# Artemarius/cuda-gaussian-splatting

Hardware: AMD Instinct MI355X
Metric: fwd+bwd Mpixels/s @1080p, 1M Gaussians, SH3 (higher is better)
Workload: dtype f32

## Files before the change

cuda-gaussian-splatting_amd/_lib.py:

```python
from __future__ import annotations

import ctypes as C
import os

_HERE = os.path.dirname(os.path.abspath(__file__))
LIB_PATH = os.environ.get("CUGS_HIP_LIBRARY") or os.path.join(_HERE, "libcugs_hip.so")

PACKED_STRIDE = 12
GRAD_STRIDE = 16
TILE = 16


class Camera(C.Structure):
    _fields_ = [("view", C.c_float * 16), ("fx", C.c_float), ("fy", C.c_float), ("cx", C.c_float),
                ("cy", C.c_float), ("width", C.c_int32), ("height", C.c_int32),
                ("cam_center", C.c_float * 3), ("reserved", C.c_float)]


class AdamGroup(C.Structure):
    _fields_ = [("param", C.c_void_p), ("grad", C.c_void_p), ("m", C.c_void_p), ("v", C.c_void_p),
                ("n", C.c_int64), ("lr", C.c_float), ("reserved", C.c_float)]


class AdamFused(C.Structure):
    _fields_ = [("m", C.c_void_p * 5), ("v", C.c_void_p * 5), ("lr", C.c_float * 5), ("beta1", C.c_float),
                ("beta2", C.c_float), ("eps", C.c_float), ("bc1", C.c_float), ("bc2", C.c_float)]


class DensifyArray(C.Structure):
    _fields_ = [("src", C.c_void_p), ("dst", C.c_void_p), ("row_floats", C.c_int32), ("mode", C.c_int32)]


DENSIFY_COPY, DENSIFY_POSITIONS, DENSIFY_SCALES, DENSIFY_STATE = 0, 1, 2, 3


class McmcFused(C.Structure):
    _fields_ = [("lambda_opacity", C.c_float), ("lambda_scale", C.c_float), ("noise_lr", C.c_float),
                ("gate_k", C.c_float), ("gate_t", C.c_float), ("step", C.c_uint32), ("seed", C.c_uint64),
                ("noise", C.c_void_p)]


KNN_AUTO, KNN_EXHAUSTIVE, KNN_TREE = 0, 1, 2
MCMC_STREAM_NOISE, MCMC_STREAM_JITTER, MCMC_STREAM_SAMPLE = 0, 1, 2


class PoseGrad(C.Structure):
    _fields_ = [("dL_dview", C.c_void_p), ("rows", C.c_void_p), ("workspace", C.c_void_p),
                ("workspace_bytes", C.c_size_t)]


class BlendForwardOpts(C.Structure):
    _fields_ = [("zero_buf", C.c_void_p), ("zero_bytes", C.c_size_t), ("tile_order", C.c_void_p),
                ("depths", C.c_void_p), ("out_depth", C.c_void_p)]


class BlendBackwardOpts(C.Structure):
    _fields_ = [("prezeroed", C.c_int), ("abs_grad", C.c_int), ("tile_order", C.c_void_p), ("depths", C.c_void_p),
                ("dL_ddepth_map", C.c_void_p), ("dL_dalpha", C.c_void_p), ("dL_ddepths", C.c_void_p),
                ("dL_dmeans_2d_abs", C.c_void_p)]


class LossOpts(C.Structure):
    _fields_ = [("exposure", C.c_void_p), ("mask", C.c_void_p), ("dL_dexposure", C.c_void_p), ("corrected", C.c_void_p)]


class DepthLossOpts(C.Structure):
    _fields_ = [("weight", C.c_void_p), ("scale_shift", C.c_void_p), ("fit", C.c_int), ("inverse", C.c_int),
                ("min_alpha", C.c_float), ("expected", C.c_void_p)]


class NormalLossOpts(C.Structure):
    _fields_ = [("weight", C.c_void_p), ("normals_out", C.c_void_p), ("cos_weight", C.c_float), ("l1_weight", C.c_float),
                ("min_alpha", C.c_float)]


class BilagridDims(C.Structure):
    _fields_ = [("l", C.c_int32), ("gy", C.c_int32), ("gx", C.c_int32)]

_P = C.c_void_p
_I = C.c_int
_L = C.c_int64
_F = C.c_float
_U32 = C.c_uint32
_U64 = C.c_uint64

SIGNATURES = {
    "cugs_version": (C.c_char_p, []),
    "cugs_error_string": (C.c_char_p, [_I]),
    "cugs_project_forward": (_I, [_L, _I, _I, _P, _P, _P, _P, _P, C.POINTER(Camera), _F,
                                  _P, _P, _P, _P, _P, _P, _P, _P, _P, _P]),
    "cugs_project_forward_keyed": (_I, [_L, _I, _I, _P, _P, _P, _P, _P, C.POINTER(Camera), _F,
                                        _P, _P, _P, _P, _P, _P, _P, _P, _P, _P, C.c_size_t, _P]),
    "cugs_project_forward_geometry": (_I, [_L, _P, _P, _P, _P, C.POINTER(Camera), _F, _P, _P, _P, _P, _P, _P, _P, _P,
                                           C.c_size_t, _P]),
    "cugs_project_forward_colour": (_I, [_L, _I, _I, _P, _P, C.POINTER(Camera), _P, _P, _P, _P]),
    "cugs_evaluate_sh": (_I, [_I, _L, _I, _P, _P, _P, _P]),
    "cugs_evaluate_sh_backward": (_I, [_I, _L, _I, _P, _P, _P, _P, _P]),
    "cugs_pack_projected": (_I, [_L, _P, _P, _P, _P, _P, _P]),
    "cugs_sort_workspace_bytes": (C.c_size_t, [_L]),
    "cugs_sort_pair_workspace_bytes": (C.c_size_t, [_L]),
    "cugs_sort_count_pairs": (_I, [_L, _P, _P, _P, _P, _I, _I, _P, C.c_size_t, C.POINTER(C.c_int64), _P]),
    "cugs_sort_count_pairs_wide": (_I, [_L, _P, _P, _P, _P, _I, _I, _P, C.c_size_t, C.POINTER(C.c_int64), _P]),
    "cugs_sort_pairs_predicted_wide": (_I, [_L, _L, _P, _P, _P, _P, _I, _I, _P, C.c_size_t, _P, C.c_size_t, _P, _P, _P,
                                            C.POINTER(C.c_int64), _P]),
    "cugs_sort_pairs": (_I, [_L, _L, _P, _P, _P, _P, _I, _I, _P, C.c_size_t, _P, C.c_size_t, _P, _P, _P, _P]),
    "cugs_sort_pairs_predicted": (_I, [_L, _L, _P, _P, _P, _P, _I, _I, _P, C.c_size_t, _P, C.c_size_t, _P, _P, _P,
                                       C.POINTER(C.c_int64), _P]),
    "cugs_sort_pairs_predicted_keyed": (_I, [_L, _L, _P, _P, _P, _P, _I, _I, _P, C.c_size_t, _P, C.c_size_t, _P, _P, _P,
                                             C.POINTER(C.c_int64), _P]),
    "cugs_sort_pairs_predicted_keyed_ordered": (_I, [_L, _L, _P, _P, _P, _P, _I, _I, _P, C.c_size_t, _P, C.c_size_t, _P, _P, _P,
                                                     C.POINTER(C.c_int64), _P, _P]),
    "cugs_tile_order": (_I, [_I, _I, _P, _P, _P]),
    "cugs_rasterize_forward": (_I, [_I, _I, C.POINTER(C.c_float), _P, _P, _P, _P, _P, _P, _P,
                                    _P, _P, _P, _P]),
    "cugs_rasterize_forward_opts": (_I, [_I, _I, C.POINTER(C.c_float), _P, _P, _P, _P, _P, _P, _P,
                                         _P, _P, _P, C.POINTER(BlendForwardOpts), _P]),
    "cugs_blend_scores": (_I, [_I, _I, _P, _P, _P, _P, _P, _P, _P, _I, _P, _P]),
    "cugs_rasterize_backward": (_I, [_I, _I, C.POINTER(C.c_float), _P, _P, _P, _P, _P, _P, _P,
                                     _P, _P, _P, _L, _P, _P, _P, _P, _P, _P]),
    "cugs_rasterize_backward_opts": (_I, [_I, _I, C.POINTER(C.c_float), _P, _P, _P, _P, _P, _P, _P,
                                          _P, _P, _P, _L, _P, _P, _P, _P, _P, C.POINTER(BlendBackwardOpts), _P]),
    "cugs_project_backward": (_I, [_L, _I, _I, _P, _P, _P, _P, _P, _P, _P, C.POINTER(Camera), _F,
                                   _P, _P, _P, _P, _P, _P, _P, _P, _P, _P, _P, _P, _P]),
    "cugs_project_backward_adam": (_I, [_L, _I, _I, _P, _P, _P, _P, _P, _P, _P, C.POINTER(Camera), _F, _P,
                                        C.POINTER(AdamFused), _P, _P]),
    "cugs_sh_backward_views": (_I, [_I, _L, _I, _P, _I, _P, C.POINTER(C.c_float), _P, _P]),
    "cugs_gated_colour_grad": (_I, [_L, _P, _P, _P, _P]),
    "cugs_adam_bias_correction": (None, [_F, _F, _I, C.POINTER(C.c_float), C.POINTER(C.c_float)]),
    "cugs_fused_adam": (_I, [_P, _P, _P, _P, _L, _F, _F, _F, _F, _F, _F, _P]),
    "cugs_fused_adam_groups": (_I, [C.POINTER(AdamGroup), _I, _F, _F, _F, _F, _F, _P]),
    "cugs_fused_adam_groups_rows": (_I, [C.POINTER(AdamGroup), _I, C.POINTER(C.c_int32), _P, _L, _F, _F, _F, _F, _F, _P]),
    "cugs_loss_workspace_bytes": (C.c_size_t, [_I, _I]),
    "cugs_combined_loss": (_I, [_I, _I, _P, _P, _F, _I, _P, C.c_size_t, _P, _P, _P, _P]),
    "cugs_loss_opts_workspace_bytes": (C.c_size_t, [_I, _I]),
    "cugs_combined_loss_opts": (_I, [_I, _I, _P, _P, _F, _I, C.POINTER(LossOpts), _P, C.c_size_t, _P, _P, _P, _P]),
    "cugs_depth_loss_workspace_bytes": (C.c_size_t, [_I, _I]),
    "cugs_depth_loss": (_I, [_I, _I, _P, _P, _P, C.POINTER(DepthLossOpts), _P, C.c_size_t, _P, _P, _P, _P]),
    "cugs_normal_loss_workspace_bytes": (C.c_size_t, [_I, _I]),
    "cugs_normal_loss": (_I, [_I, _I, _F, _F, _F, _F, _P, _P, _P, C.POINTER(NormalLossOpts), _P, C.c_size_t, _P, _P, _P, _P]),
    "cugs_bilagrid_workspace_bytes": (C.c_size_t, [_I, _I, C.POINTER(BilagridDims)]),
    "cugs_bilagrid_slice": (_I, [_I, _I, C.POINTER(BilagridDims), _P, _P, _P, _P]),
    "cugs_bilagrid_slice_backward": (_I, [_I, _I, C.POINTER(BilagridDims), _P, _P, _P, _P, C.c_size_t, _P, _P, _P]),
    "cugs_bilagrid_tv": (_I, [C.POINTER(BilagridDims), _P, _F, _P, _P, _I, _P]),
    "cugs_eval_workspace_bytes": (C.c_size_t, [_I, _I]),
    "cugs_eval_metrics": (_I, [_I, _I, _P, _P, _P, _I, _P, C.c_size_t, _P, _P]),
    "cugs_densify_accumulate": (_I, [_L, _P, _P, _P, _P, _P, _P]),
    "cugs_densify_accumulate_strided": (_I, [_L, _P, _L, _P, _P, _P, _P, _P]),
    "cugs_densify_classify": (_I, [_L, _P, _P, _P, _P, _P, _F, _F, _F, _I, _F, _F, _P, _P, _P]),
    "cugs_densify_workspace_bytes": (C.c_size_t, [_L]),
    "cugs_densify_plan": (_I, [_L, _P, _P, C.c_size_t, C.POINTER(C.c_int64), _P]),
    "cugs_densify_apply": (_I, [_L, _L, _P, C.c_size_t, _P, _P, C.POINTER(DensifyArray), _I, _P]),
    "cugs_mcmc_random_bits": (_I, [_U64, _U32, _U32, _U64, _L, _P, _P]),
    "cugs_mcmc_regularization": (_I, [_L, _P, _P, _F, _F, _P, _P, _P, _P, _P, _P, C.c_size_t, _P]),
    "cugs_mcmc_inject_noise": (_I, [_L, _P, _P, _P, _F, _F, _F, _P, _U64, _U32, _P]),
    "cugs_mcmc_relocate_workspace_bytes": (C.c_size_t, [_L]),
    "cugs_mcmc_relocate": (_I, [_L, _I, _P, _P, _P, _P, _P, _F, _F, _F, _U64, _U32, C.POINTER(_P), C.POINTER(_P), _P,
                                C.c_size_t, _P, _P, _P]),
    "cugs_project_backward_adam_mcmc": (_I, [_L, _I, _I, _P, _P, _P, _P, _P, _P, _P, C.POINTER(Camera), _F, _P,
                                             C.POINTER(AdamFused), C.POINTER(McmcFused), _P, _P]),
    "cugs_pose_grad_workspace_bytes": (C.c_size_t, [_L]),
    "cugs_project_backward_pose": (_I, [_L, _I, _I, _P, _P, _P, _P, _P, _P, _P, C.POINTER(Camera), _F,
                                        _P, _P, _P, _P, _P, _P, _P, _P, _P, _P, _P, _P, C.POINTER(PoseGrad), _P]),
    "cugs_project_backward_adam_pose": (_I, [_L, _I, _I, _P, _P, _P, _P, _P, _P, _P, C.POINTER(Camera), _F, _P,
                                             C.POINTER(AdamFused), _P, C.POINTER(PoseGrad), _P]),
    "cugs_project_backward_adam_mcmc_pose": (_I, [_L, _I, _I, _P, _P, _P, _P, _P, _P, _P, C.POINTER(Camera), _F, _P,
                                                  C.POINTER(AdamFused), C.POINTER(McmcFused), _P, C.POINTER(PoseGrad),
                                                  _P]),
    "cugs_project_backward_adam_sparse": (_I, [_L, _I, _I, _P, _P, _P, _P, _P, _P, _P, C.POINTER(Camera), _F, _P,
                                               C.POINTER(AdamFused), _P, _P]),
    "cugs_project_backward_adam_sparse_pose": (_I, [_L, _I, _I, _P, _P, _P, _P, _P, _P, _P, C.POINTER(Camera), _F, _P,
                                                    C.POINTER(AdamFused), _P, C.POINTER(PoseGrad), _P]),
    "cugs_ply_vertex_floats": (_I, [_I, _I]),
    "cugs_ply_pack": (_I, [_L, _I, C.POINTER(_P), C.POINTER(_P), C.POINTER(_P), _P, _P]),
    "cugs_ply_unpack": (_I, [_L, _I, _I, _P, _P, C.POINTER(_P), C.POINTER(_P), C.POINTER(_P), _P]),
    "cugs_image_to_float": (_I, [_I, _I, _P, _I, _I, _P, _P]),
    "cugs_knn_workspace_bytes": (C.c_size_t, [_L, _I]),
    "cugs_knn_mean_distances": (_I, [_L, _I, _P, _P, _P, C.c_size_t, _I, _P]),
    "cugs_init_from_points": (_I, [_L, _I, _P, _P, _P, _P, _P, _P, _P, _P, _P]),
    "cugs_device_count": (_I, [C.POINTER(C.c_int)]),
}


def _load() -> C.CDLL:
    if not os.path.exists(LIB_PATH):
        raise ImportError(
            f"{LIB_PATH} not found: build it with `make -C {os.path.join(_HERE, 'csrc')}` "
            "(or `python -c 'import __graft_entry__ as g; g.build()'`). "
            "There is no fallback path: the HIP library is the implementation.")
    lib = C.CDLL(LIB_PATH)
    for name, (res, args) in SIGNATURES.items():
        try:
            fn = getattr(lib, name)
        except AttributeError as e:
            raise ImportError(f"{LIB_PATH} does not export {name}") from e
        fn.restype = res
        fn.argtypes = args
    return lib


lib = _load()


class CugsError(RuntimeError):
    """Non-zero return from the C ABI (the adapter's std::runtime_error, cuda_utils.cuh:12-20)."""


# ... 9 lines not shown
```

cuda-gaussian-splatting_amd/adapter/cugs_hip_torch.cpp:

```cpp
#include "cugs_hip_torch.hpp"

#include <c10/hip/HIPFunctions.h>
#include <c10/hip/HIPStream.h>
#include <hip/hip_runtime_api.h>

#include <algorithm>
#include <chrono>
#include <cmath>
#include <cstdio>
#include <cstdlib>
#include <map>
#include <stdexcept>
#include <string>
#include <tuple>
#include <vector>

namespace cugs_hip {
namespace {

void check(int code, const char* what) {
    if (code != 0)
        throw std::runtime_error(std::string("HIP error in ") + what + " - " + cugs_error_string(code));
}
void* stream_of(const torch::Tensor& t) {
// ... 106 lines not shown
        check((wide_depth ? cugs_sort_count_pairs_wide : cugs_sort_count_pairs)(
                  n, ptr<float>(m), ptr<float>(d), ptr<int32_t>(r), ptr<int32_t>(tiles), img_w, img_h, ws.data_ptr(),
                  ws.numel(), &total, st), "cugs_sort_count_pairs");
    o.total_pairs = static_cast<int>(total);
    o.gaussian_keys_sorted = torch::empty({total}, torch::TensorOptions().dtype(torch::kInt64).device(means_2d.device()));
    o.gaussian_values_sorted = torch::empty({total}, iopt(means_2d));
    if (num_tiles > 0) {
        auto wp = workspace(means_2d.device(), cugs_sort_pair_workspace_bytes(total), 1);
        check(cugs_sort_pairs(n, total, ptr<float>(m), ptr<float>(d), ptr<int32_t>(r), ptr<int32_t>(tiles), img_w, img_h,
                              ws.data_ptr(), ws.numel(), wp.data_ptr(), wp.numel(),
                              reinterpret_cast<uint64_t*>(ptr<int64_t>(o.gaussian_keys_sorted)),
                              ptr<int32_t>(o.gaussian_values_sorted), ptr<int32_t>(o.tile_ranges), st),
              "cugs_sort_pairs");
    }
    return o;
}
}

SortingOutput sort_gaussians(const torch::Tensor& means_2d, const torch::Tensor& depths, const torch::Tensor& radii,
                             const torch::Tensor& tiles_touched, int img_w, int img_h) {
    return sort_gaussians_impl(means_2d, depths, radii, tiles_touched, img_w, img_h, false);
}

ForwardOutput rasterize_forward(const torch::Tensor& means_2d, const torch::Tensor& cov_2d_inv, const torch::Tensor& rgb,
                                const torch::Tensor& opacities, const torch::Tensor& tile_ranges,
                                const torch::Tensor& gaussian_indices, int img_w, int img_h,
                                const float background[3], const torch::Tensor& packed, const torch::Tensor& zero_buf,
                                const torch::Tensor& tile_order, const torch::Tensor& depths) {
    TORCH_CHECK(means_2d.is_cuda(), "means_2d must be on CUDA");
    ForwardOutput o;
    o.color = torch::empty({img_h, img_w, 3}, fopt(means_2d));
    o.final_T = torch::empty({img_h, img_w}, fopt(means_2d));
    o.n_contrib = torch::empty({img_h, img_w}, iopt(means_2d));
    if (depths.defined()) {
        TORCH_CHECK(depths.is_cuda() && depths.device() == means_2d.device() && depths.dim() == 1 &&
                    depths.size(0) == means_2d.size(0), "depths must be [N] on the device of means_2d");
        o.depth_map = torch::empty({img_h, img_w}, fopt(means_2d));
    }
    if (img_w == 0 || img_h == 0) {
        if (zero_buf.defined()) zero_buf.zero_();
        return o;
    }
    auto m = means_2d.contiguous(), c = cov_2d_inv.contiguous(), r = rgb.contiguous(), op = opacities.contiguous();
    auto tr = tile_ranges.contiguous(), gi = gaussian_indices.contiguous();
    if (zero_buf.defined())
        TORCH_CHECK(zero_buf.is_contiguous() && zero_buf.scalar_type() == torch::kFloat32 && zero_buf.numel() % 4 == 0,
                    "zero_buf must be a contiguous float32 tensor of a multiple of four elements");
    if (tile_order.defined())
        TORCH_CHECK(tile_order.is_contiguous() && tile_order.scalar_type() == torch::kInt32 &&
                    tile_order.numel() == 4 * tr.size(0), "tile_order must be a contiguous [tiles, 4] int32 tensor");
    const auto z = depths.defined() ? f32c(depths) : depths;
    cugs_blend_forward_opts opts{};
    if (zero_buf.defined()) {
        opts.zero_buf = zero_buf.data_ptr();
        opts.zero_bytes = static_cast<size_t>(zero_buf.numel()) * sizeof(float);
    }
    opts.tile_order = order_ptr(tile_order);
    opts.depths = ptr<float>(z);
    opts.out_depth = ptr<float>(o.depth_map);
    check(cugs_rasterize_forward_opts(img_w, img_h, background, ptr<int32_t>(tr), ptr<int32_t>(gi), ptr<float>(m),
                                      ptr<float>(c), ptr<float>(r), ptr<float>(op), ptr<float>(packed), ptr<float>(o.color),
                                      ptr<float>(o.final_T), ptr<int32_t>(o.n_contrib), &opts, stream_of(means_2d)),
          "cugs_rasterize_forward_opts");
    return o;
}

torch::Tensor tile_order_of(const torch::Tensor& tile_ranges, int img_w, int img_h) {
    auto tr = tile_ranges.contiguous();
    auto order = torch::empty({tr.size(0), 4}, iopt(tile_ranges));
    if (tr.size(0) > 0)
        check(cugs_tile_order(img_w, img_h, ptr<int32_t>(tr), reinterpret_cast<uint32_t*>(order.data_ptr<int32_t>()),
                              stream_of(tile_ranges)), "cugs_tile_order");
    return order;
}

RasterizeBackwardOutput rasterize_backward(const torch::Tensor& dL_dcolor, const torch::Tensor& means_2d,
                                           const torch::Tensor& cov_2d_inv, const torch::Tensor& rgb,
                                           const torch::Tensor& opacities, const torch::Tensor& tile_ranges,
                                           const torch::Tensor& gaussian_indices, const torch::Tensor& final_T,
                                           const torch::Tensor& n_contrib, int img_w, int img_h,
                                           const float background[3], int n_gaussians, const torch::Tensor& packed,
                                           bool unpack, const torch::Tensor& zeroed_accum, const torch::Tensor& tile_order,
                                           const torch::Tensor& depths, const torch::Tensor& dL_ddepth_map,
                                           const torch::Tensor& dL_dalpha, bool want_abs_grad) {
    TORCH_CHECK(dL_dcolor.is_cuda(), "dL_dcolor must be on CUDA");
    const int64_t n = n_gaussians;
    RasterizeBackwardOutput o;
    const bool depth_route = depths.defined() || dL_ddepth_map.defined() || dL_dalpha.defined();
    if (depth_route) {
        TORCH_CHECK(depths.defined(), "the depth / alpha map gradients need the projection's depths");
        TORCH_CHECK(depths.is_cuda() && depths.device() == dL_dcolor.device() && depths.dim() == 1 && depths.size(0) == n,
                    "depths must be [N] on the device of dL_dcolor");
        for (const torch::Tensor* t : {&dL_ddepth_map, &dL_dalpha})
            if (t->defined())
                TORCH_CHECK(t->is_cuda() && t->device() == dL_dcolor.device() && t->dim() == 2 && t->size(0) == img_h &&
                            t->size(1) == img_w, "dL_ddepth_map / dL_dalpha must be [H, W] on the device of dL_dcolor");
    }
    const bool prezeroed = zeroed_accum.defined();
    if (prezeroed)
        TORCH_CHECK(zeroed_accum.is_contiguous() && zeroed_accum.dim() == 2 && zeroed_accum.size(0) == n &&
                    zeroed_accum.size(1) == CUGS_GRAD_STRIDE, "zeroed_accum must be a contiguous [N, 16] float32 tensor");
    o.grad_accum = prezeroed ? zeroed_accum : torch::empty({n, CUGS_GRAD_STRIDE}, fopt(dL_dcolor));
    if (unpack) {
        o.dL_drgb = torch::empty({n, 3}, fopt(dL_dcolor));
        o.dL_dopacity_act = torch::empty({n}, fopt(dL_dcolor));
        o.dL_dmeans_2d = torch::empty({n, 2}, fopt(dL_dcolor));
        o.dL_dcov_2d_inv = torch::empty({n, 3}, fopt(dL_dcolor));
        if (depth_route) o.dL_ddepths = torch::empty({n}, fopt(dL_dcolor));
    }
    if (want_abs_grad)
        o.dL_dmeans_2d_abs = unpack ? torch::empty({n, 2}, fopt(dL_dcolor)) : o.grad_accum.slice(1, 10, 12);
    if (n == 0) return o;
    auto g = dL_dcolor.contiguous(), m = means_2d.contiguous(), c = cov_2d_inv.contiguous(), r = rgb.contiguous();
    auto op = opacities.contiguous(), tr = tile_ranges.contiguous(), gi = gaussian_indices.contiguous();
    auto ft = final_T.contiguous(), nc = n_contrib.contiguous();
    if (tile_order.defined())
        TORCH_CHECK(tile_order.is_contiguous() && tile_order.scalar_type() == torch::kInt32 &&
                    tile_order.numel() == 4 * tr.size(0), "tile_order must be a contiguous [tiles, 4] int32 tensor");
    auto f32 = [](const torch::Tensor& t) { return t.defined() ? f32c(t) : t; };
    const auto z = f32(depths), dd = f32(dL_ddepth_map), da = f32(dL_dalpha);
    cugs_blend_backward_opts opts{};
    opts.prezeroed = prezeroed ? 1 : 0;
    opts.abs_grad = want_abs_grad ? 1 : 0;
    opts.tile_order = order_ptr(tile_order);
    opts.depths = ptr<float>(z);
    opts.dL_ddepth_map = ptr<float>(dd);
    opts.dL_dalpha = ptr<float>(da);
    opts.dL_ddepths = ptr<float>(o.dL_ddepths);
    opts.dL_dmeans_2d_abs = unpack ? ptr<float>(o.dL_dmeans_2d_abs) : nullptr;
    check(cugs_rasterize_backward_opts(img_w, img_h, background, ptr<int32_t>(tr), ptr<int32_t>(gi), ptr<float>(m),
                                       ptr<float>(c), ptr<float>(r), ptr<float>(op), ptr<float>(packed), ptr<float>(g),
                                       ptr<float>(ft), ptr<int32_t>(nc), n, ptr<float>(o.grad_accum),
                                       ptr<float>(o.dL_drgb), ptr<float>(o.dL_dopacity_act), ptr<float>(o.dL_dmeans_2d),
                                       ptr<float>(o.dL_dcov_2d_inv), &opts, stream_of(dL_dcolor)),
          "cugs_rasterize_backward_opts");
    return o;
}

namespace {
ProjectionBackwardOutput project_backward_impl(const torch::Tensor* accum, const torch::Tensor* colour_gate,
                                               torch::Tensor* d_means_out, const torch::Tensor& gm, const torch::Tensor& gc,
                                               const torch::Tensor& gr, const torch::Tensor& go,
                                               const torch::Tensor& positions, const torch::Tensor& rotations,
                                               const torch::Tensor& scales, const torch::Tensor& opacities,
                                               const torch::Tensor& sh_coeffs, const torch::Tensor& radii,
                                               const cugs_camera& camera, int degree, float scale_modifier,
                                               const cugs_pose_grad* pose = nullptr) {
    TORCH_CHECK(positions.is_cuda(), "positions must be on CUDA");
    const int64_t n = positions.size(0);
    ProjectionBackwardOutput o;
    o.dL_dpositions = torch::empty({n, 3}, fopt(positions));
    o.dL_drotations = torch::empty({n, 4}, fopt(positions));
    o.dL_dscales = torch::empty({n, 3}, fopt(positions));
    o.dL_dopacities = torch::empty({n, 1}, fopt(positions));
    auto sh = f32c(sh_coeffs);
    o.dL_dsh_coeffs = torch::empty_like(sh);
    if (n == 0) return o;
    auto pos = f32c(positions), rot = f32c(rotations), scl = f32c(scales), opa = f32c(opacities), rad = radii.contiguous();
    auto cm = gm.defined() ? gm.contiguous() : gm, cc = gc.defined() ? gc.contiguous() : gc;
    auto cr = gr.defined() ? gr.contiguous() : gr, co = go.defined() ? go.contiguous() : go;
    if (pose) {
        check(cugs_project_backward_pose(n, static_cast<int>(sh.size(2)), degree, ptr<float>(pos), ptr<float>(rot),
                                         ptr<float>(scl), ptr<float>(opa), ptr<float>(sh), ptr<int32_t>(rad),
                                         colour_gate ? ptr<uint8_t>(*colour_gate) : nullptr, &camera, scale_modifier,
                                         accum ? ptr<float>(*accum) : nullptr, ptr<float>(cm), ptr<float>(cc),
                                         ptr<float>(cr), ptr<float>(co), ptr<float>(o.dL_dpositions),
                                         ptr<float>(o.dL_drotations), ptr<float>(o.dL_dscales),
                                         ptr<float>(o.dL_dopacities), ptr<float>(o.dL_dsh_coeffs),
                                         d_means_out ? ptr<float>(*d_means_out) : nullptr,
                                         nullptr, pose, stream_of(positions)),
              "cugs_project_backward_pose");
        return o;
    }
    check(cugs_project_backward(n, static_cast<int>(sh.size(2)), degree, ptr<float>(pos), ptr<float>(rot), ptr<float>(scl),
                                ptr<float>(opa), ptr<float>(sh), ptr<int32_t>(rad),
                                colour_gate ? ptr<uint8_t>(*colour_gate) : nullptr, &camera, scale_modifier,
                                accum ? ptr<float>(*accum) : nullptr, ptr<float>(cm), ptr<float>(cc), ptr<float>(cr),
                                ptr<float>(co), ptr<float>(o.dL_dpositions), ptr<float>(o.dL_drotations),
                                ptr<float>(o.dL_dscales), ptr<float>(o.dL_dopacities), ptr<float>(o.dL_dsh_coeffs),
                                d_means_out ? ptr<float>(*d_means_out) : nullptr, nullptr,
                                stream_of(positions)),
          "cugs_project_backward");
    return o;
}
}

ProjectionBackwardOutput project_backward(const torch::Tensor& dL_dmeans_2d, const torch::Tensor& dL_dcov_2d_inv,
                                          const torch::Tensor& dL_drgb, const torch::Tensor& dL_dopacity_act,
                                          const torch::Tensor& positions, const torch::Tensor& rotations,
                                          const torch::Tensor& scales, const torch::Tensor& opacities,
                                          const torch::Tensor& sh_coeffs, const torch::Tensor& radii,
                                          const cugs_camera& camera, int active_sh_degree, float scale_modifier) {
    return project_backward_impl(nullptr, nullptr, nullptr, dL_dmeans_2d, dL_dcov_2d_inv, dL_drgb, dL_dopacity_act,
                                 positions, rotations, scales, opacities, sh_coeffs, radii, camera, active_sh_degree,
                                 scale_modifier);
}

torch::Tensor evaluate_sh_cuda(int degree, const torch::Tensor& sh_coeffs, const torch::Tensor& directions) {
    TORCH_CHECK(degree >= 0 && degree <= 3, "SH degree must be 0..3, got ", degree);
    TORCH_CHECK(sh_coeffs.is_cuda(), "sh_coeffs must be on CUDA device");
    TORCH_CHECK(directions.is_cuda(), "directions must be on CUDA device");
    TORCH_CHECK(sh_coeffs.dim() == 3 && sh_coeffs.size(1) == 3, "sh_coeffs must be [N, 3, C]");
    TORCH_CHECK(directions.dim() == 2 && directions.size(1) == 3, "directions must be [N, 3]");
    TORCH_CHECK(sh_coeffs.size(0) == directions.size(0), "Batch size mismatch");
    TORCH_CHECK(sh_coeffs.size(2) >= (degree + 1) * (degree + 1), "Need at least ", (degree + 1) * (degree + 1),
                " coefficients for degree ", degree);
    auto c = f32c(sh_coeffs), d = f32c(directions);
    auto out = torch::empty({c.size(0), 3}, fopt(c));
    if (c.size(0) == 0) return out;
    check(cugs_evaluate_sh(degree, c.size(0), static_cast<int>(c.size(2)), ptr<float>(c), ptr<float>(d), ptr<float>(out),
                           stream_of(c)), "cugs_evaluate_sh");
    return out;
}

torch::Tensor evaluate_sh_backward_cuda(int degree, const torch::Tensor& sh_coeffs, const torch::Tensor& directions,
                                        const torch::Tensor& dL_dcolor) {
    TORCH_CHECK(degree >= 0 && degree <= 3, "SH degree must be 0..3, got ", degree);
    TORCH_CHECK(sh_coeffs.is_cuda() && directions.is_cuda() && dL_dcolor.is_cuda(), "inputs must be on CUDA device");
    TORCH_CHECK(sh_coeffs.dim() == 3 && sh_coeffs.size(1) == 3, "sh_coeffs must be [N, 3, C]");
    TORCH_CHECK(directions.dim() == 2 && directions.size(1) == 3, "directions must be [N, 3]");
    TORCH_CHECK(dL_dcolor.dim() == 2 && dL_dcolor.size(1) == 3, "dL_dcolor must be [N, 3]");
    auto c = f32c(sh_coeffs), d = f32c(directions), g = f32c(dL_dcolor);
    auto out = torch::empty_like(c);
    if (c.size(0) == 0) return out;
    check(cugs_evaluate_sh_backward(degree, c.size(0), static_cast<int>(c.size(2)), ptr<float>(c), ptr<float>(d),
                                    ptr<float>(g), ptr<float>(out), stream_of(c)), "cugs_evaluate_sh_backward");
    return out;
}

static int max_sh_degree(const torch::Tensor& sh) {
    return sh.defined() ? static_cast<int>(std::sqrt(static_cast<float>(sh.size(2)))) - 1 : 0;
}

RenderOutput render(const ModelTensors& model, const cugs_camera& camera, const RenderSettings& settings,
                    bool for_backward, bool want_depth_map) {
    TORCH_CHECK(model.positions.defined() && model.positions.is_cuda(), "GaussianModel must be on CUDA device");
    const int64_t n = model.positions.size(0);
    const int w = camera.width, h = camera.height;
    RenderOutput o;
    if (n == 0) {
        o.color = torch::empty({h, w, 3}, fopt(model.positions));
        for (int ch = 0; ch < 3; ++ch) o.color.select(2, ch).fill_(settings.background[ch]);
        o.final_T = torch::ones({h, w}, fopt(model.positions));
        o.n_contrib = torch::zeros({h, w}, iopt(model.positions));
        o.means_2d = torch::empty({0, 2}, fopt(model.positions)); o.depths = torch::empty({0}, fopt(model.positions));
        o.cov_2d_inv = torch::empty({0, 3}, fopt(model.positions)); o.radii = torch::empty({0}, iopt(model.positions));
        o.rgb = torch::empty({0, 3}, fopt(model.positions)); o.opacities_act = torch::empty({0}, fopt(model.positions));
        o.gaussian_indices = torch::empty({0}, iopt(model.positions)); o.tile_ranges = torch::empty({0, 2}, iopt(model.positions));
        if (want_depth_map) o.depth_map = torch::zeros({h, w}, fopt(model.positions));
        return o;
    }
    const int degree = std::min(settings.active_sh_degree, max_sh_degree(model.sh_coeffs));
    SortState& state = sort_state(model.positions.device());
    const int num_tiles = ((w + CUGS_TILE - 1) / CUGS_TILE) * ((h + CUGS_TILE - 1) / CUGS_TILE);
    const bool predicted = state.last_pairs >= 0 && num_tiles > 0;
    const bool wide = state.wide_left > 0;
    if (wide) --state.wide_left;
    const bool keyed = predicted && !wide;
    auto proj = project_impl(model.positions, model.rotations, model.scales, model.opacities, model.sh_coeffs, camera,
                             degree, settings.scale_modifier, keyed);
    torch::Tensor accum = for_backward ? torch::empty({n, CUGS_GRAD_STRIDE}, fopt(model.positions)) : torch::Tensor();
    auto blend = [&](const SortingOutput& s) {
        return rasterize_forward(proj.means_2d, proj.cov_2d_inv, proj.rgb, proj.opacities_act, s.tile_ranges,
                                 s.gaussian_values_sorted, w, h, settings.background, proj.packed, accum, s.tile_order,
                                 want_depth_map ? proj.depths : torch::Tensor());
// ... 29 lines not shown
            check(cugs_sort_pairs_predicted_keyed(
                      n, cap, ptr<float>(proj.means_2d), ptr<float>(proj.depths), ptr<int32_t>(proj.radii), ptr<int32_t>(tiles), w, h,
                      ws.data_ptr(), ws.numel(), wp.data_ptr(), wp.numel(), nullptr, ptr<int32_t>(srt.gaussian_values_sorted),
                      ptr<int32_t>(srt.tile_ranges), total.data_ptr<int64_t>(), st), "cugs_sort_pairs_predicted_keyed");
        } else {
            srt.tile_order = torch::empty({num_tiles, 4}, iopt(proj.means_2d));
            check(cugs_sort_pairs_predicted_keyed_ordered(
                      n, cap, ptr<float>(proj.means_2d), ptr<float>(proj.depths), ptr<int32_t>(proj.radii), ptr<int32_t>(tiles), w, h,
                      ws.data_ptr(), ws.numel(), wp.data_ptr(), wp.numel(), nullptr, ptr<int32_t>(srt.gaussian_values_sorted),
                      ptr<int32_t>(srt.tile_ranges), total.data_ptr<int64_t>(),
                      reinterpret_cast<uint32_t*>(srt.tile_order.data_ptr<int32_t>()), st), "cugs_sort_pairs_predicted_keyed_ordered");
        }
        hipEvent_t ev;
        TORCH_CHECK(hipEventCreateWithFlags(&ev, hipEventDisableTiming) == hipSuccess, "hipEventCreate failed");
        TORCH_CHECK(hipEventRecord(ev, static_cast<hipStream_t>(st)) == hipSuccess, "hipEventRecord failed");
        fwd = blend(srt);
        const bool ok = hipEventSynchronize(ev) == hipSuccess;
        (void)hipEventDestroy(ev);
        TORCH_CHECK(ok, "hipEventSynchronize failed");
        const int64_t p = total.data_ptr<int64_t>()[0];
        TORCH_CHECK(p >= -1 && p <= 2147483647ll, "pair count exceeds the reference's int indexing");
        if (p >= 0 && p <= cap) {
            srt.total_pairs = static_cast<int>(p);
            srt.gaussian_values_sorted = srt.gaussian_values_sorted.slice(0, 0, p);
        } else {
            if (p == -1) state.wide_left = kWideDepthHold;
            srt = sort_gaussians_impl(proj.means_2d, proj.depths, proj.radii, proj.tiles_touched, w, h,
                                      p == -1 || state.wide_left > 0);
            if (ordered) srt.tile_order = tile_order_of(srt.tile_ranges, w, h);
            fwd = blend(srt);
        }
    }
    state.last_pairs = std::max<int64_t>(srt.total_pairs, prev - prev / 32);
    o.color = fwd.color; o.final_T = fwd.final_T; o.n_contrib = fwd.n_contrib; o.depth_map = fwd.depth_map;
    o.means_2d = proj.means_2d; o.depths = proj.depths; o.cov_2d_inv = proj.cov_2d_inv; o.radii = proj.radii;
    o.rgb = proj.rgb; o.opacities_act = proj.opacities_act;
    o.gaussian_indices = srt.gaussian_values_sorted; o.tile_ranges = srt.tile_ranges; o.packed = proj.packed;
    o.tile_order = srt.tile_order;
    o.colour_gate = proj.colour_gate;
    o.zeroed_accum = accum;
    if (accum.defined()) o.accum_used = std::make_shared<std::atomic<bool>>(false);
    return o;
}

BackwardOutput render_backward(const torch::Tensor& dL_dcolor, const RenderOutput& ro, const ModelTensors& model,
                               const cugs_camera& camera, const RenderSettings& settings, FusedAdam* fused,
                               const MCMCController* mcmc, int step, const torch::Tensor& dL_ddepth_map,
                               const torch::Tensor& dL_dalpha, bool want_camera_grad, bool want_abs_grad,
                               bool sparse_adam) {
    TORCH_CHECK(!mcmc || fused, "the fused MCMC route needs the FusedAdam (otherwise: compute_regularization, step, "
                "inject_noise)");
    TORCH_CHECK(!sparse_adam || fused, "sparse_adam needs the FusedAdam (otherwise: render_backward, apply_gradients, "
                "step(radii))");
    TORCH_CHECK(!sparse_adam || !mcmc, "sparse_adam cannot be combined with the fused MCMC route: its regulariser and "
                "noise act on every Gaussian");
    TORCH_CHECK(dL_dcolor.is_cuda(), "dL_dcolor must be on CUDA device");
    TORCH_CHECK(dL_dcolor.dim() == 3 && dL_dcolor.size(2) == 3, "dL_dcolor must be [H, W, 3]");
    TORCH_CHECK(!dL_ddepth_map.defined() || ro.depth_map.defined(),
                "dL_ddepth_map needs a render with the depth map (render(..., want_depth_map = true))");
    const bool depth_grads = dL_ddepth_map.defined() || dL_dalpha.defined();
    const int64_t n = model.positions.size(0);
    BackwardOutput o;
    if (n == 0) {
        o.dL_dpositions = torch::zeros({0, 3}, fopt(dL_dcolor)); o.dL_drotations = torch::zeros({0, 4}, fopt(dL_dcolor));
        o.dL_dscales = torch::zeros({0, 3}, fopt(dL_dcolor)); o.dL_dopacities = torch::zeros({0, 1}, fopt(dL_dcolor));
        o.dL_dsh_coeffs = torch::zeros_like(model.sh_coeffs); o.dL_dmeans_2d = torch::zeros({0, 2}, fopt(dL_dcolor));
        if (want_camera_grad) o.dL_dviewmat = torch::zeros({4, 4}, fopt(dL_dcolor));
        if (want_abs_grad) o.dL_dmeans_2d_abs = torch::zeros({0, 2}, fopt(dL_dcolor));
        return o;
    }
    const int degree = std::min(settings.active_sh_degree, max_sh_degree(model.sh_coeffs));
    torch::Tensor packed = ro.packed;
    if (!packed.defined() || packed.size(0) != n) {
        packed = torch::empty({n, CUGS_PACKED_STRIDE}, fopt(dL_dcolor));
        auto m = ro.means_2d.contiguous(), c = ro.cov_2d_inv.contiguous(), r = ro.rgb.contiguous(),
             op = ro.opacities_act.contiguous();
        check(cugs_pack_projected(n, ptr<float>(m), ptr<float>(c), ptr<float>(r), ptr<float>(op), ptr<float>(packed),
                                  stream_of(dL_dcolor)), "cugs_pack_projected");
    }
    torch::Tensor zeroed = ro.zeroed_accum;
    ro.zeroed_accum = torch::Tensor();
    if (zeroed.defined() && ro.accum_used && ro.accum_used->exchange(true)) zeroed = torch::Tensor();
    if (zeroed.defined() && (zeroed.dim() != 2 || zeroed.size(0) != n)) zeroed = torch::Tensor();
    auto rb = rasterize_backward(dL_dcolor, ro.means_2d, ro.cov_2d_inv, ro.rgb, ro.opacities_act, ro.tile_ranges,
                                 ro.gaussian_indices, ro.final_T, ro.n_contrib, camera.width, camera.height,
                                 settings.background, static_cast<int>(n), packed, false, zeroed, ro.tile_order,
                                 depth_grads ? ro.depths : torch::Tensor(), dL_ddepth_map, dL_dalpha, want_abs_grad);
    o.dL_dmeans_2d_abs = rb.dL_dmeans_2d_abs;
    o.dL_dmeans_2d = torch::empty({n, 2}, fopt(dL_dcolor));
    cugs_pose_grad pose{};
    torch::Tensor pose_ws;
    if (want_camera_grad) {
        o.dL_dviewmat = torch::empty({4, 4}, fopt(dL_dcolor));
        const size_t bytes = cugs_pose_grad_workspace_bytes(n);
        pose_ws = torch::empty({static_cast<int64_t>(bytes)}, dL_dcolor.options().dtype(torch::kUInt8));
        pose = cugs_pose_grad{ptr<float>(o.dL_dviewmat), nullptr, pose_ws.data_ptr(), bytes};
    }
    if (fused) {
        const auto& pr = fused->params();
        TORCH_CHECK(pr[0].data_ptr() == model.positions.data_ptr() && pr[1].data_ptr() == model.sh_coeffs.data_ptr(),
                    "the fused optimizer step needs the FusedAdam that was built on this model");
        TORCH_CHECK(ro.colour_gate.defined() && ro.colour_gate.size(0) == n,
                    "the fused optimizer step needs the colour_gate of cugs_hip::render");
        const cugs_adam_fused adam = fused->begin_fused_step();
        auto radii = ro.radii.contiguous(), gate = ro.colour_gate.contiguous();
        if (mcmc) {
            const cugs_mcmc_fused mc = mcmc->fused_args(step);
            if (want_camera_grad) {
                check(cugs_project_backward_adam_mcmc_pose(n, static_cast<int>(model.sh_coeffs.size(2)), degree,
                                                           ptr<float>(model.positions), ptr<float>(model.rotations),
                                                           ptr<float>(model.scales), ptr<float>(model.opacities),
                                                           ptr<float>(model.sh_coeffs), ptr<int32_t>(radii),
                                                           ptr<uint8_t>(gate), &camera, settings.scale_modifier,
                                                           ptr<float>(rb.grad_accum), &adam, &mc,
                                                           ptr<float>(o.dL_dmeans_2d), &pose, stream_of(dL_dcolor)),
                      "cugs_project_backward_adam_mcmc_pose");
                return o;
            }
            check(cugs_project_backward_adam_mcmc(n, static_cast<int>(model.sh_coeffs.size(2)), degree,
                                                  ptr<float>(model.positions), ptr<float>(model.rotations),
                                                  ptr<float>(model.scales), ptr<float>(model.opacities),
                                                  ptr<float>(model.sh_coeffs), ptr<int32_t>(radii), ptr<uint8_t>(gate),
                                                  &camera, settings.scale_modifier, ptr<float>(rb.grad_accum), &adam, &mc,
                                                  ptr<float>(o.dL_dmeans_2d), stream_of(dL_dcolor)),
                  "cugs_project_backward_adam_mcmc");
            return o;
        }
        if (sparse_adam) {
            if (want_camera_grad) {
                check(cugs_project_backward_adam_sparse_pose(n, static_cast<int>(model.sh_coeffs.size(2)), degree,
                                                             ptr<float>(model.positions), ptr<float>(model.rotations),
                                                             ptr<float>(model.scales), ptr<float>(model.opacities),
                                                             ptr<float>(model.sh_coeffs), ptr<int32_t>(radii),
                                                             ptr<uint8_t>(gate), &camera, settings.scale_modifier,
                                                             ptr<float>(rb.grad_accum), &adam, ptr<float>(o.dL_dmeans_2d),
                                                             &pose, stream_of(dL_dcolor)),
                      "cugs_project_backward_adam_sparse_pose");
                return o;
            }
            check(cugs_project_backward_adam_sparse(n, static_cast<int>(model.sh_coeffs.size(2)), degree,
                                                    ptr<float>(model.positions), ptr<float>(model.rotations),
                                                    ptr<float>(model.scales), ptr<float>(model.opacities),
                                                    ptr<float>(model.sh_coeffs), ptr<int32_t>(radii), ptr<uint8_t>(gate),
                                                    &camera, settings.scale_modifier, ptr<float>(rb.grad_accum), &adam,
                                                    ptr<float>(o.dL_dmeans_2d), stream_of(dL_dcolor)),
                  "cugs_project_backward_adam_sparse");
            return o;
        }
        if (want_camera_grad) {
            check(cugs_project_backward_adam_pose(n, static_cast<int>(model.sh_coeffs.size(2)), degree,
                                                  ptr<float>(model.positions), ptr<float>(model.rotations),
                                                  ptr<float>(model.scales), ptr<float>(model.opacities),
                                                  ptr<float>(model.sh_coeffs), ptr<int32_t>(radii), ptr<uint8_t>(gate),
                                                  &camera, settings.scale_modifier, ptr<float>(rb.grad_accum), &adam,
                                                  ptr<float>(o.dL_dmeans_2d), &pose, stream_of(dL_dcolor)),
                  "cugs_project_backward_adam_pose");
            return o;
        }
        check(cugs_project_backward_adam(n, static_cast<int>(model.sh_coeffs.size(2)), degree, ptr<float>(model.positions),
                                         ptr<float>(model.rotations), ptr<float>(model.scales), ptr<float>(model.opacities),
                                         ptr<float>(model.sh_coeffs), ptr<int32_t>(radii), ptr<uint8_t>(gate), &camera,
                                         settings.scale_modifier, ptr<float>(rb.grad_accum), &adam,
                                         ptr<float>(o.dL_dmeans_2d), stream_of(dL_dcolor)),
              "cugs_project_backward_adam");
        return o;
    }
    const bool have_gate = ro.colour_gate.defined() && ro.colour_gate.dim() == 1 && ro.colour_gate.size(0) == n;
    auto pb = project_backward_impl(&rb.grad_accum, have_gate ? &ro.colour_gate : nullptr, &o.dL_dmeans_2d, {}, {}, {}, {}, model.positions,
                                    model.rotations, model.scales, model.opacities, model.sh_coeffs, ro.radii, camera, degree,
                                    settings.scale_modifier, want_camera_grad ? &pose : nullptr);
    o.dL_dpositions = pb.dL_dpositions; o.dL_drotations = pb.dL_drotations; o.dL_dscales = pb.dL_dscales;
    o.dL_dopacities = pb.dL_dopacities; o.dL_dsh_coeffs = pb.dL_dsh_coeffs;
    return o;
}

namespace {
void validate_pair(const torch::Tensor& rendered, const torch::Tensor& target) {
    for (const torch::Tensor* img : {&rendered, &target}) {
        TORCH_CHECK(img->dim() == 3, "image must be 3-dimensional [H, W, 3], got ", img->dim(), " dims");
        TORCH_CHECK(img->size(2) == 3, "image must have 3 channels, got ", img->size(2));
        TORCH_CHECK(img->dtype() == torch::kFloat32, "image must be float32, got ", img->dtype());
        TORCH_CHECK(img->is_cuda(), "image must be on a CUDA device");
    }
    TORCH_CHECK(rendered.sizes() == target.sizes(), "rendered and target must have the same shape, got ",
                rendered.sizes(), " vs ", target.sizes());
}
torch::Tensor run_loss(const torch::Tensor& rendered, const torch::Tensor& target, float lambda_, int window_size,
                       torch::Tensor* ssim_map, torch::Tensor* grad) {
    validate_pair(rendered, target);
    TORCH_CHECK(window_size % 2 == 1, "window_size must be odd, got ", window_size);
    TORCH_CHECK(window_size >= 3, "window_size must be >= 3, got ", window_size);
    const int h = static_cast<int>(rendered.size(0)), w = static_cast<int>(rendered.size(1));
    auto r = rendered.contiguous(), t = target.contiguous();
    auto out = torch::empty({4}, fopt(rendered));
    if (ssim_map) *ssim_map = torch::empty({h, w}, fopt(rendered));
    if (grad) *grad = torch::empty({h, w, 3}, fopt(rendered));
    auto ws = workspace(rendered.device(), cugs_loss_workspace_bytes(w, h), 2);
    check(cugs_combined_loss(w, h, ptr<float>(r), ptr<float>(t), lambda_, window_size, ws.data_ptr(), ws.numel(),
                             ptr<float>(out), ssim_map ? ptr<float>(*ssim_map) : nullptr,
                             grad ? ptr<float>(*grad) : nullptr, stream_of(rendered)), "cugs_combined_loss");
    return out;
}
}

LossAndGrad combined_loss_and_grad(const torch::Tensor& rendered, const torch::Tensor& target, float lambda_, bool want_grad) {
    LossAndGrad o;
    auto out = run_loss(rendered, target, lambda_, 11, nullptr, want_grad ? &o.dL_dcolor : nullptr);
    o.loss = out[0]; o.l1 = out[1]; o.ssim_mean = out[2];
    return o;
}
torch::Tensor combined_loss(const torch::Tensor& rendered, const torch::Tensor& target, float lambda_) {
    return run_loss(rendered, target, lambda_, 11, nullptr, nullptr)[0];
}
torch::Tensor ssim(const torch::Tensor& rendered, const torch::Tensor& target, int window_size) {
    torch::Tensor map;
    run_loss(rendered, target, 0.2f, window_size, &map, nullptr);
    return map;
}

ExposureLoss combined_loss_exposure(const torch::Tensor& rendered, const torch::Tensor& target, float lambda_,
                                    const torch::Tensor& exposure, const torch::Tensor& mask, bool want_grad,
                                    bool want_corrected, int window_size) {
    validate_pair(rendered, target);
    TORCH_CHECK(window_size % 2 == 1, "window_size must be odd, got ", window_size);
    TORCH_CHECK(window_size >= 3, "window_size must be >= 3, got ", window_size);
    const int h = static_cast<int>(rendered.size(0)), w = static_cast<int>(rendered.size(1));
    if (exposure.defined()) {
        TORCH_CHECK(exposure.dim() == 2 && exposure.size(0) == 3 && exposure.size(1) == 4, "exposure must be [3, 4], got ", exposure.sizes());
        TORCH_CHECK(exposure.dtype() == torch::kFloat32, "exposure must be float32, got ", exposure.dtype());
        TORCH_CHECK(exposure.is_cuda() && exposure.device() == rendered.device(), "exposure must be on the images' CUDA device");
        TORCH_CHECK(exposure.is_contiguous(), "exposure must be contiguous");
    }
    torch::Tensor m;
    if (mask.defined()) {
        TORCH_CHECK(mask.dim() == 2 && mask.size(0) == h && mask.size(1) == w, "mask must be [H, W], got ", mask.sizes());
        TORCH_CHECK(mask.dtype() == torch::kFloat32, "mask must be float32, got ", mask.dtype());
        TORCH_CHECK(mask.is_cuda() && mask.device() == rendered.device(), "mask must be on the images' CUDA device");
        m = mask.contiguous();
    }
    auto r = rendered.contiguous(), t = target.contiguous();
    auto out = torch::empty({4}, fopt(rendered));
    ExposureLoss o;
    if (want_grad) o.dL_dcolor = torch::empty({h, w, 3}, fopt(rendered));
    if (want_grad && exposure.defined()) o.dL_dexposure = torch::empty({3, 4}, fopt(rendered));
    if (want_corrected) o.corrected = torch::empty({h, w, 3}, fopt(rendered));
    cugs_loss_opts opts{};
    opts.exposure = exposure.defined() ? exposure.data_ptr<float>() : nullptr;
    opts.mask = m.defined() ? m.data_ptr<float>() : nullptr;
    opts.dL_dexposure = o.dL_dexposure.defined() ? o.dL_dexposure.data_ptr<float>() : nullptr;
    opts.corrected = o.corrected.defined() ? o.corrected.data_ptr<float>() : nullptr;
    auto ws = workspace(rendered.device(), cugs_loss_opts_workspace_bytes(w, h), 2);
    check(cugs_combined_loss_opts(w, h, ptr<float>(r), ptr<float>(t), lambda_, window_size, &opts, ws.data_ptr(), ws.numel(),
                                  ptr<float>(out), nullptr, want_grad ? o.dL_dcolor.data_ptr<float>() : nullptr,
// ... 864 lines not shown
```

cuda-gaussian-splatting_amd/adapter/cugs_hip_torch.hpp:

```cpp
#pragma once

#include <torch/torch.h>

#include <atomic>
#include <memory>

#include <array>
#include <string>
#include <vector>

#include "../../include/cugs_hip.h"
#include "eval_results.hpp"

namespace cugs_hip {

struct ProjectionOutput {
    torch::Tensor means_2d, depths, cov_2d_inv, radii, tiles_touched, rgb, opacities_act;
    torch::Tensor packed;
    torch::Tensor colour_gate;
};
struct SortingOutput {
    torch::Tensor gaussian_keys_sorted, gaussian_values_sorted, tile_ranges;
    int total_pairs = 0;
    torch::Tensor tile_order;
};
struct ForwardOutput {
    torch::Tensor color, final_T, n_contrib;
    torch::Tensor depth_map;
};
struct RasterizeBackwardOutput {
    torch::Tensor dL_drgb, dL_dopacity_act, dL_dmeans_2d, dL_dcov_2d_inv;
    torch::Tensor grad_accum;
    torch::Tensor dL_ddepths;
    torch::Tensor dL_dmeans_2d_abs;
};
struct ProjectionBackwardOutput { torch::Tensor dL_dpositions, dL_drotations, dL_dscales, dL_dopacities, dL_dsh_coeffs; };

struct ModelTensors {
    torch::Tensor positions, sh_coeffs, opacities, rotations, scales;
};
struct RenderSettings { float background[3] = {0.f, 0.f, 0.f}; int active_sh_degree = 3; float scale_modifier = 1.f; };
struct RenderOutput {
    torch::Tensor color, final_T, n_contrib, means_2d, depths, cov_2d_inv, radii, rgb, opacities_act,
        gaussian_indices, tile_ranges;
    torch::Tensor packed;
    torch::Tensor colour_gate;
    mutable torch::Tensor zeroed_accum;
    std::shared_ptr<std::atomic<bool>> accum_used;
    torch::Tensor tile_order;
    torch::Tensor depth_map;
};
struct BackwardOutput {
    torch::Tensor dL_dpositions, dL_drotations, dL_dscales, dL_dopacities, dL_dsh_coeffs, dL_dmeans_2d;
    torch::Tensor dL_dviewmat;
    torch::Tensor dL_dmeans_2d_abs;
};

ProjectionOutput project_gaussians(const torch::Tensor& positions, const torch::Tensor& rotations,
                                   const torch::Tensor& scales, const torch::Tensor& opacities,
                                   const torch::Tensor& sh_coeffs, const cugs_camera& camera,
                                   int active_sh_degree, float scale_modifier = 1.0f);
SortingOutput sort_gaussians(const torch::Tensor& means_2d, const torch::Tensor& depths, const torch::Tensor& radii,
                             const torch::Tensor& tiles_touched, int img_w, int img_h);
ForwardOutput rasterize_forward(const torch::Tensor& means_2d, const torch::Tensor& cov_2d_inv,
                                const torch::Tensor& rgb, const torch::Tensor& opacities,
                                const torch::Tensor& tile_ranges, const torch::Tensor& gaussian_indices,
                                int img_w, int img_h, const float background[3],
                                const torch::Tensor& packed = {}, const torch::Tensor& zero_buf = {},
                                const torch::Tensor& tile_order = {}, const torch::Tensor& depths = {});
torch::Tensor tile_order_of(const torch::Tensor& tile_ranges, int img_w, int img_h);
RasterizeBackwardOutput rasterize_backward(const torch::Tensor& dL_dcolor, const torch::Tensor& means_2d,
                                           const torch::Tensor& cov_2d_inv, const torch::Tensor& rgb,
                                           const torch::Tensor& opacities, const torch::Tensor& tile_ranges,
                                           const torch::Tensor& gaussian_indices, const torch::Tensor& final_T,
                                           const torch::Tensor& n_contrib, int img_w, int img_h,
                                           const float background[3], int n_gaussians,
                                           const torch::Tensor& packed = {}, bool unpack = true,
                                           const torch::Tensor& zeroed_accum = {}, const torch::Tensor& tile_order = {},
                                           const torch::Tensor& depths = {}, const torch::Tensor& dL_ddepth_map = {},
                                           const torch::Tensor& dL_dalpha = {}, bool want_abs_grad = false);
ProjectionBackwardOutput project_backward(const torch::Tensor& dL_dmeans_2d, const torch::Tensor& dL_dcov_2d_inv,
                                          const torch::Tensor& dL_drgb, const torch::Tensor& dL_dopacity_act,
                                          const torch::Tensor& positions, const torch::Tensor& rotations,
                                          const torch::Tensor& scales, const torch::Tensor& opacities,
                                          const torch::Tensor& sh_coeffs, const torch::Tensor& radii,
                                          const cugs_camera& camera, int active_sh_degree,
                                          float scale_modifier = 1.0f);
torch::Tensor evaluate_sh_cuda(int degree, const torch::Tensor& sh_coeffs, const torch::Tensor& directions);
torch::Tensor evaluate_sh_backward_cuda(int degree, const torch::Tensor& sh_coeffs, const torch::Tensor& directions,
                                        const torch::Tensor& dL_dcolor);

RenderOutput render(const ModelTensors& model, const cugs_camera& camera, const RenderSettings& settings,
                    bool for_backward = true, bool want_depth_map = false);
class FusedAdam;
class MCMCController;
BackwardOutput render_backward(const torch::Tensor& dL_dcolor, const RenderOutput& render_out,
                               const ModelTensors& model, const cugs_camera& camera, const RenderSettings& settings,
                               FusedAdam* fused = nullptr, const MCMCController* mcmc = nullptr, int step = 0,
                               const torch::Tensor& dL_ddepth_map = {}, const torch::Tensor& dL_dalpha = {},
                               bool want_camera_grad = false, bool want_abs_grad = false, bool sparse_adam = false);

struct LossAndGrad { torch::Tensor loss, l1, ssim_mean, dL_dcolor; };
LossAndGrad combined_loss_and_grad(const torch::Tensor& rendered, const torch::Tensor& target, float lambda_ = 0.2f,
                                   bool want_grad = true);
torch::Tensor combined_loss(const torch::Tensor& rendered, const torch::Tensor& target, float lambda_ = 0.2f);
torch::Tensor ssim(const torch::Tensor& rendered, const torch::Tensor& target, int window_size = 11);

struct ExposureLoss { torch::Tensor loss, dL_dcolor, dL_dexposure, l1, ssim_mean, corrected; };
ExposureLoss combined_loss_exposure(const torch::Tensor& rendered, const torch::Tensor& target, float lambda_ = 0.2f,
                                    const torch::Tensor& exposure = {}, const torch::Tensor& mask = {},
                                    bool want_grad = true, bool want_corrected = false, int window_size = 11);

struct DepthLoss { torch::Tensor loss, dL_ddepth_map, dL_dalpha, scale_shift, valid_weight, valid_count, fit_ok, expected; };
DepthLoss depth_loss(const torch::Tensor& depth_map, const torch::Tensor& alpha, const torch::Tensor& target,
                     const torch::Tensor& weight = {}, bool inverse = false, const torch::Tensor& align = {},
                     bool fit = false, float min_alpha = 1e-3f, bool want_grad = true, bool want_expected = false);

struct NormalLoss { torch::Tensor loss, dL_ddepth_map, dL_dalpha, valid_weight, valid_count, normals; };
NormalLoss normal_loss(const torch::Tensor& depth_map, const torch::Tensor& alpha, float fx, float fy, float cx, float cy,
                       const torch::Tensor& target = {}, const torch::Tensor& weight = {}, float cos_weight = 1.0f,
                       float l1_weight = 0.0f, float min_alpha = 1e-3f, bool want_grad = true, bool want_normals = false);
torch::Tensor depth_to_normals(const torch::Tensor& depth_map, const torch::Tensor& alpha, float fx, float fy, float cx,
                               float cy, float min_alpha = 1e-3f);

struct BilagridGrad { torch::Tensor dL_drendered, dL_dgrid; };
struct BilagridTV { torch::Tensor tv, dL_dgrid; };
torch::Tensor bilagrid_slice(const torch::Tensor& grid, const torch::Tensor& rendered);
BilagridGrad bilagrid_slice_backward(const torch::Tensor& grid, const torch::Tensor& rendered,
                                     const torch::Tensor& dL_dcorrected, bool want_grid_grad = true,
                                     bool want_image_grad = true);
BilagridTV bilagrid_tv(const torch::Tensor& grid, float weight = 1.0f, const torch::Tensor& dL_dgrid = {});

struct AdamHyper { float beta1 = 0.9f, beta2 = 0.999f, eps = 1e-15f; };
class FusedAdam {
public:
    FusedAdam(std::array<torch::Tensor, 5> params, std::array<float, 5> lrs, AdamHyper h = {});
    void apply_gradients(const BackwardOutput& grads);
    void zero_grad();
    void set_lr(int group, float lr) { lrs_[group] = lr; }
    float get_lr(int group) const { return lrs_[group]; }
    void step();
    void step(const torch::Tensor& visible);
    cugs_adam_fused begin_fused_step();
    const std::array<torch::Tensor, 5>& params() const { return params_; }
    const std::array<torch::Tensor, 5>& exp_avg() const { return m_; }
    const std::array<torch::Tensor, 5>& exp_avg_sq() const { return v_; }
private:
    friend class DensificationController;
    friend class MCMCController;
    friend int64_t prune_gaussians(ModelTensors&, const torch::Tensor&, FusedAdam*);
    friend bool write_gaussian_ply(const std::string&, const ModelTensors&, const FusedAdam*);
    friend ModelTensors read_gaussian_ply(const std::string&, const torch::Device&, FusedAdam*);
    void step_groups(const torch::Tensor* rows);
    std::array<torch::Tensor, 5> params_, m_, v_, grads_;
    std::array<float, 5> lrs_;
    AdamHyper h_;
    int step_count_ = 0;
};

struct DensificationConfig {
    int densify_from = 500, densify_until = 15000, densify_every = 100, opacity_reset_every = 3000;
    float grad_threshold = 0.0002f, opacity_threshold = 0.005f, percent_dense = 0.01f;
    int max_screen_size = 20, max_gaussians = 0;
// ... 87 lines not shown
```

cuda-gaussian-splatting_amd/csrc/project_backward.hip:

```cpp
#include "project_backward_kernels.h"

namespace {

template <int C>
int launch_shv(int64_t n, int degree, const float* pos, const float* gated, const ViewCenters& vc, float* out,
               bool aligned, hipStream_t st) {
    if (aligned)
        hipLaunchKernelGGL((k_sh_backward_views<C, true>), dim3(grid_for(n)), dim3(CUGS_BLOCK), 0, st, n, degree, pos, gated, vc, out);
    else
        hipLaunchKernelGGL((k_sh_backward_views<C, false>), dim3(grid_for(n)), dim3(CUGS_BLOCK), 0, st, n, degree, pos, gated, vc, out);
    CUGS_LAUNCH_CHECK();
    return 0;
}


template <int C>
int launch_pb(int64_t n, int degree, const CamArgs& cam, const PBPtrs& p, bool aligned, hipStream_t st,
              const AdamFusedArgs* adam = nullptr) {
    const AdamFusedArgs none{};
    if (adam) {
        if constexpr (C == 16) {
            if (aligned && p.colour_gate) {
                hipLaunchKernelGGL((k_project_backward<C, true, true, true>), dim3(grid_for(n)), dim3(CUGS_BLOCK), 0, st, n, degree, cam, p, *adam, McmcFusedArgs{}, PoseArgs{});
                CUGS_LAUNCH_CHECK();
                return 0;
            }
        }
        if (aligned)
            hipLaunchKernelGGL((k_project_backward<C, true, true>), dim3(grid_for(n)), dim3(CUGS_BLOCK), 0, st, n, degree, cam, p, *adam, McmcFusedArgs{}, PoseArgs{});
        else
            hipLaunchKernelGGL((k_project_backward<C, false, true>), dim3(grid_for(n)), dim3(CUGS_BLOCK), 0, st, n, degree, cam, p, *adam, McmcFusedArgs{}, PoseArgs{});
    } else if (aligned) {
        if constexpr (C == 16) {
            if (p.colour_gate) {
                hipLaunchKernelGGL((k_project_backward<C, true, false, true>), dim3(grid_for(n)), dim3(CUGS_BLOCK), 0, st, n, degree, cam, p, none, McmcFusedArgs{}, PoseArgs{});
                CUGS_LAUNCH_CHECK();
                return 0;
            }
        }
        hipLaunchKernelGGL((k_project_backward<C, true, false>), dim3(grid_for(n)), dim3(CUGS_BLOCK), 0, st, n, degree, cam, p, none, McmcFusedArgs{}, PoseArgs{});
    } else {
        hipLaunchKernelGGL((k_project_backward<C, false, false>), dim3(grid_for(n)), dim3(CUGS_BLOCK), 0, st, n, degree, cam, p, none, McmcFusedArgs{}, PoseArgs{});
    }
    CUGS_LAUNCH_CHECK();
    return 0;
}


template <int C>
int launch_shb(int64_t n, int degree, const float* sh, const float* dirs, const float* g, float* out,
               bool aligned, hipStream_t st) {
    if (aligned)
        hipLaunchKernelGGL((k_sh_backward<C, true>), dim3(grid_for(n)), dim3(CUGS_BLOCK), 0, st, n, degree, sh, dirs, g, out);
    else
        hipLaunchKernelGGL((k_sh_backward<C, false>), dim3(grid_for(n)), dim3(CUGS_BLOCK), 0, st, n, degree, sh, dirs, g, out);
    CUGS_LAUNCH_CHECK();
    return 0;
}


}

extern "C" int cugs_project_backward(int64_t n, int num_coeffs, int active_degree, const float* positions,
                                     const float* rotations, const float* scales, const float* opacities,
                                     const float* sh_coeffs, const int32_t* radii, const uint8_t* colour_gate,
                                     const cugs_camera* camera_host, float scale_modifier,
                                     const float* grad_accum, const float* dL_dmeans_2d,
                                     const float* dL_dcov_2d_inv, const float* dL_drgb,
                                     const float* dL_dopacity_act, float* dL_dpositions, float* dL_drotations,
                                     float* dL_dscales, float* dL_dopacities, float* dL_dsh_coeffs,
                                     float* dL_dmeans_2d_out, float* dL_drgb_gated_out, void* stream) {
    CamArgs cam;
    PBPtrs p;
    bool aligned;
    const int r = prepare_plain(n, num_coeffs, active_degree, positions, rotations, scales, opacities, sh_coeffs, radii,
                                colour_gate, camera_host, scale_modifier, grad_accum, dL_dmeans_2d, dL_dcov_2d_inv, dL_drgb,
                                dL_dopacity_act, dL_dpositions, dL_drotations, dL_dscales, dL_dopacities, dL_dsh_coeffs,
                                dL_dmeans_2d_out, dL_drgb_gated_out, cam, p, aligned);
    if (r != 0) return r == 1 ? 0 : r;
    hipStream_t st = static_cast<hipStream_t>(stream);
    switch (num_coeffs) {
        case 1: return launch_pb<1>(n, active_degree, cam, p, aligned, st);
        case 4: return launch_pb<4>(n, active_degree, cam, p, aligned, st);
        case 9: return launch_pb<9>(n, active_degree, cam, p, aligned, st);
        default: return launch_pb<16>(n, active_degree, cam, p, aligned, st);
    }
}


extern "C" int cugs_project_backward_adam(int64_t n, int num_coeffs, int active_degree, float* positions,
                                          float* rotations, float* scales, float* opacities, float* sh_coeffs,
                                          const int32_t* radii, const uint8_t* colour_gate,
                                          const cugs_camera* camera_host, float scale_modifier,
                                          const float* grad_accum, const cugs_adam_fused* adam_host,
                                          float* dL_dmeans_2d_out, void* stream) {
    CamArgs cam;
    PBPtrs p;
    AdamFusedArgs a;
    bool aligned;
    const int r = prepare_adam(n, num_coeffs, active_degree, positions, rotations, scales, opacities, sh_coeffs, radii,
                               colour_gate, camera_host, scale_modifier, grad_accum, adam_host, dL_dmeans_2d_out, cam, p,
                               a, aligned);
    if (r != 0) return r == 1 ? 0 : r;
    hipStream_t st = static_cast<hipStream_t>(stream);
    switch (num_coeffs) {
        case 1: return launch_pb<1>(n, active_degree, cam, p, aligned, st, &a);
        case 4: return launch_pb<4>(n, active_degree, cam, p, aligned, st, &a);
        case 9: return launch_pb<9>(n, active_degree, cam, p, aligned, st, &a);
        default: return launch_pb<16>(n, active_degree, cam, p, aligned, st, &a);
    }
}

extern "C" int cugs_evaluate_sh_backward(int degree, int64_t n, int num_coeffs, const float* sh_coeffs,
                                         const float* directions, const float* dL_dcolor, float* dL_dsh,
                                         void* stream) {
    if (degree < 0 || degree > 3 || n < 0) return CUGS_EINVAL;
    if ((degree + 1) * (degree + 1) > num_coeffs) return CUGS_EINVAL;
    if (n == 0) return 0;
    if (!sh_coeffs || !directions || !dL_dcolor || !dL_dsh) return CUGS_EINVAL;
    hipStream_t st = static_cast<hipStream_t>(stream);
    const bool aligned = cugs_aligned16(sh_coeffs) && cugs_aligned16(dL_dsh);
    switch (num_coeffs) {
        case 1: return launch_shb<1>(n, degree, sh_coeffs, directions, dL_dcolor, dL_dsh, aligned, st);
        case 4: return launch_shb<4>(n, degree, sh_coeffs, directions, dL_dcolor, dL_dsh, aligned, st);
        case 9: return launch_shb<9>(n, degree, sh_coeffs, directions, dL_dcolor, dL_dsh, aligned, st);
        case 16: return launch_shb<16>(n, degree, sh_coeffs, directions, dL_dcolor, dL_dsh, aligned, st);
        default:
            hipLaunchKernelGGL(k_sh_backward_generic, dim3(grid_for(n)), dim3(CUGS_BLOCK), 0, st, n, degree,
                               num_coeffs, sh_coeffs, directions, dL_dcolor, dL_dsh);
            CUGS_LAUNCH_CHECK();
            return 0;
    }
}

extern "C" int cugs_sh_backward_views(int degree, int64_t n, int num_coeffs, const float* positions,
                                      int num_views, const float* gated_rgb_views,
                                      const float* cam_centers_host, float* dL_dsh, void* stream) {
    if (degree < 0 || degree > 3 || n < 0 || num_views < 1 || num_views > MAX_VIEWS) return CUGS_EINVAL;
    if ((degree + 1) * (degree + 1) > num_coeffs) return CUGS_EINVAL;
    if (num_coeffs != 1 && num_coeffs != 4 && num_coeffs != 9 && num_coeffs != 16) return CUGS_EINVAL;
    if (n == 0) return 0;
    if (!positions || !gated_rgb_views || !cam_centers_host || !dL_dsh) return CUGS_EINVAL;
    ViewCenters vc;
    vc.count = num_views;
    for (int v = 0; v < MAX_VIEWS; ++v)
        for (int k = 0; k < 3; ++k) vc.c[v][k] = v < num_views ? cam_centers_host[v * 3 + k] : 0.0f;
    hipStream_t st = static_cast<hipStream_t>(stream);
    const bool aligned = cugs_aligned16(dL_dsh);
    switch (num_coeffs) {
        case 1: return launch_shv<1>(n, degree, positions, gated_rgb_views, vc, dL_dsh, aligned, st);
        case 4: return launch_shv<4>(n, degree, positions, gated_rgb_views, vc, dL_dsh, aligned, st);
        case 9: return launch_shv<9>(n, degree, positions, gated_rgb_views, vc, dL_dsh, aligned, st);
        default: return launch_shv<16>(n, degree, positions, gated_rgb_views, vc, dL_dsh, aligned, st);
    }
}

extern "C" int cugs_gated_colour_grad(int64_t n, const float* grad_accum, const uint8_t* colour_gate,
                                      float* dL_drgb_gated_out, void* stream) {
    if (n < 0) return CUGS_EINVAL;
    if (n == 0) return 0;
    if (!grad_accum || !colour_gate || !dL_drgb_gated_out) return CUGS_EINVAL;
    if (!cugs_aligned16(grad_accum)) return CUGS_EALIGN;
    hipLaunchKernelGGL(k_gated_colour_grad, dim3(grid_for(n)), dim3(CUGS_BLOCK), 0, static_cast<hipStream_t>(stream), n,
                       grad_accum, colour_gate, dL_drgb_gated_out);
    CUGS_LAUNCH_CHECK();
    return 0;
}
```

cuda-gaussian-splatting_amd/csrc/project_backward_kernels.h:

```cpp
#pragma once
#include "cugs_raster_common.h"
#include "cugs_mcmc.h"

namespace {

template <int C>
struct ShTile {
    static constexpr int ROW = 3 * C;
    static constexpr int LROW = (ROW % 2 == 0) ? ROW + 1 : ROW;
};

template <int C, bool ALIGNED>
__device__ __forceinline__ void load_sh_rows(const float* __restrict__ sh, int64_t base, int count, float* s_sh) {
    constexpr int ROW = ShTile<C>::ROW, LROW = ShTile<C>::LROW;
    const float* src = sh + base * ROW;
    const int total = count * ROW;
    const int tid = threadIdx.x;
    if (ALIGNED && count == CUGS_BLOCK) {
        constexpr int TOTAL4 = CUGS_BLOCK * ROW / 4, PER = (TOTAL4 + CUGS_BLOCK - 1) / CUGS_BLOCK;
        const float4* src4 = reinterpret_cast<const float4*>(src);
        float4 v[PER];
#pragma unroll
        for (int i = 0; i < PER; ++i) {
            const int e4 = tid + i * CUGS_BLOCK;
            v[i] = (e4 < TOTAL4) ? src4[e4] : make_float4(0.f, 0.f, 0.f, 0.f);
        }
#pragma unroll
        for (int i = 0; i < PER; ++i) {
            const int e4 = tid + i * CUGS_BLOCK;
            if (e4 < TOTAL4) {
                int e = e4 * 4;
                int row = e / ROW, col = e - row * ROW;
                const float vals[4] = {v[i].x, v[i].y, v[i].z, v[i].w};
#pragma unroll
                for (int k = 0; k < 4; ++k) {
                    s_sh[row * LROW + col] = vals[k];
                    if (++col == ROW) { col = 0; ++row; }
                }
            }
        }
    } else if (ALIGNED) {
        const int total4 = total >> 2;
        const float4* src4 = reinterpret_cast<const float4*>(src);
        for (int e4 = threadIdx.x; e4 < total4; e4 += CUGS_BLOCK) {
            const float4 v = src4[e4];
            int e = e4 * 4, row = e / ROW, col = e - row * ROW;
            const float vals[4] = {v.x, v.y, v.z, v.w};
#pragma unroll
            for (int k = 0; k < 4; ++k) {
                s_sh[row * LROW + col] = vals[k];
                if (++col == ROW) { col = 0; ++row; }
            }
        }
        for (int e = (total4 << 2) + threadIdx.x; e < total; e += CUGS_BLOCK) {
            int row = e / ROW, col = e - row * ROW;
            s_sh[row * LROW + col] = src[e];
        }
    } else {
        for (int e = threadIdx.x; e < total; e += CUGS_BLOCK) {
            int row = e / ROW, col = e - row * ROW;
            s_sh[row * LROW + col] = src[e];
        }
    }
}

constexpr int SH_FACTOR_ROW = 20;
__device__ __forceinline__ void store_sh_rows_from_factors(float* __restrict__ dst_base, int64_t base, int count, int num_active,
                                                           const float* s_fac) {
    constexpr int C = 16, ROW4 = 3 * C / 4;
    float4* dst4 = reinterpret_cast<float4*>(dst_base + base * (3 * C));
    const int total4 = count * ROW4;
#pragma unroll
    for (int i = 0; i < ROW4; ++i) {
        const int e4 = (int)threadIdx.x + i * CUGS_BLOCK;
        if (e4 < total4) {
            const int r = e4 / ROW4, j = e4 - r * ROW4, ch = j >> 2, k = (j & 3) * 4;
            const float4 y = *reinterpret_cast<const float4*>(s_fac + r * SH_FACTOR_ROW + k);
            const float g = s_fac[r * SH_FACTOR_ROW + 16 + ch];
            cugs_stnt(dst4 + e4, make_float4(k + 0 < num_active ? g * y.x : 0.0f, k + 1 < num_active ? g * y.y : 0.0f,
                                             k + 2 < num_active ? g * y.z : 0.0f, k + 3 < num_active ? g * y.w : 0.0f));
        }
    }
}

template <int C, bool ALIGNED>
__device__ __forceinline__ void store_sh_rows(float* __restrict__ dst_base, int64_t base, int count,
                                              const float* s_sh) {
    constexpr int ROW = ShTile<C>::ROW, LROW = ShTile<C>::LROW;
    float* dst = dst_base + base * ROW;
    const int total = count * ROW;
    if (ALIGNED) {
        const int total4 = total >> 2;
        float4* dst4 = reinterpret_cast<float4*>(dst);
        for (int e4 = threadIdx.x; e4 < total4; e4 += CUGS_BLOCK) {
            int e = e4 * 4, row = e / ROW, col = e - row * ROW;
            float vals[4];
#pragma unroll
            for (int k = 0; k < 4; ++k) {
                vals[k] = s_sh[row * LROW + col];
                if (++col == ROW) { col = 0; ++row; }
            }
            cugs_stnt(dst4 + e4, make_float4(vals[0], vals[1], vals[2], vals[3]));
        }
        for (int e = (total4 << 2) + threadIdx.x; e < total; e += CUGS_BLOCK) {
            int row = e / ROW, col = e - row * ROW;
            dst[e] = s_sh[row * LROW + col];
        }
    } else {
        for (int e = threadIdx.x; e < total; e += CUGS_BLOCK) {
            int row = e / ROW, col = e - row * ROW;
            dst[e] = s_sh[row * LROW + col];
        }
    }
}

struct AdamFusedArgs {
    float* m[5]; float* v[5];
    float lr[5];
    float beta1, beta2, eps, bc1, bc2;
};
__device__ __forceinline__ void adam_update(float& p, float g, float& m, float& v, float lr, const AdamFusedArgs& h) {
    const float mi = h.beta1 * m + (1.0f - h.beta1) * g;
    m = mi;
    const float vi = h.beta2 * v + (1.0f - h.beta2) * g * g;
    v = vi;
    const float m_hat = mi * h.bc1;
    const float v_hat = vi * h.bc2;
    p -= lr * m_hat / (sqrtf(v_hat) + h.eps);
}
template <int C, bool ALIGNED, bool SPARSE = false>
__device__ __forceinline__ void adam_sh_rows(float* __restrict__ param, float* __restrict__ mom, float* __restrict__ var,
                                             int64_t base, int count, const float* s_sh, float lr, const AdamFusedArgs& h,
                                             const float* s_vis = nullptr) {
    constexpr int ROW = ShTile<C>::ROW, LROW = ShTile<C>::LROW;
    float* P = param + base * ROW; float* M = mom + base * ROW; float* V = var + base * ROW;
    const int total = count * ROW;
    int done = 0;
    if constexpr (SPARSE) {
        if (ALIGNED) {
            const int total4 = total >> 2;
            for (int e4 = threadIdx.x; e4 < total4; e4 += CUGS_BLOCK) {
                int e = e4 * 4, row = e / ROW, col = e - row * ROW;
                float g[4];
                bool vis[4];
#pragma unroll
                for (int k = 0; k < 4; ++k) {
                    g[k] = s_sh[row * LROW + col];
                    vis[k] = s_vis[row] != 0.0f;
                    if (++col == ROW) { col = 0; ++row; }
                }
                if (!(vis[0] || vis[1] || vis[2] || vis[3])) continue;
                float4 pp = cugs_ldnt(reinterpret_cast<float4*>(P) + e4), mm = cugs_ldnt(reinterpret_cast<float4*>(M) + e4),
                       vv = cugs_ldnt(reinterpret_cast<float4*>(V) + e4);
                if (vis[0]) adam_update(pp.x, g[0], mm.x, vv.x, lr, h);
                if (vis[1]) adam_update(pp.y, g[1], mm.y, vv.y, lr, h);
                if (vis[2]) adam_update(pp.z, g[2], mm.z, vv.z, lr, h);
                if (vis[3]) adam_update(pp.w, g[3], mm.w, vv.w, lr, h);
                cugs_stnt(reinterpret_cast<float4*>(P) + e4, pp); cugs_stnt(reinterpret_cast<float4*>(M) + e4, mm);
                cugs_stnt(reinterpret_cast<float4*>(V) + e4, vv);
            }
            done = total4 << 2;
        }
        for (int e = done + threadIdx.x; e < total; e += CUGS_BLOCK) {
// ... 90 lines not shown
    }
}

__device__ __forceinline__ int active_count(int degree) { return (degree + 1) * (degree + 1); }


__device__ __forceinline__ Sym2 grad_cov_from_inv(const Sym2& inv, const Sym2& g_inv) {
    const float a = inv.a, b = inv.b, c = inv.c;
    const float da = g_inv.a, db = g_inv.b * 0.5f, dc = g_inv.c;
    const float t00 = a * da + b * db, t01 = a * db + b * dc;
    const float t10 = b * da + c * db, t11 = b * db + c * dc;
    return Sym2{-(t00 * a + t01 * b), -(t00 * b + t01 * c), -(t10 * b + t11 * c)};
}

__device__ __forceinline__ Sym3 grad_cov3d(const M23& T, const Sym2& g) {
    const float e0 = T.r0x * g.a + T.r1x * g.b, e1 = T.r0x * g.b + T.r1x * g.c;
    const float e2 = T.r0y * g.a + T.r1y * g.b, e3 = T.r0y * g.b + T.r1y * g.c;
    const float e4 = T.r0z * g.a + T.r1z * g.b, e5 = T.r0z * g.b + T.r1z * g.c;
    Sym3 d;
    d.xx = e0 * T.r0x + e1 * T.r1x;
    d.xy = e0 * T.r0y + e1 * T.r1y;
    d.xz = e0 * T.r0z + e1 * T.r1z;
    d.yy = e2 * T.r0y + e3 * T.r1y;
    d.yz = e2 * T.r0z + e3 * T.r1z;
    d.zz = e4 * T.r0z + e5 * T.r1z;
    return d;
}

__device__ __forceinline__ M3 grad_M(const Sym3& d, const M3& M) {
    M3 o;
    o.m00 = 2.0f * (d.xx * M.m00 + d.xy * M.m10 + d.xz * M.m20);
    o.m01 = 2.0f * (d.xx * M.m01 + d.xy * M.m11 + d.xz * M.m21);
    o.m02 = 2.0f * (d.xx * M.m02 + d.xy * M.m12 + d.xz * M.m22);
    o.m10 = 2.0f * (d.xy * M.m00 + d.yy * M.m10 + d.yz * M.m20);
    o.m11 = 2.0f * (d.xy * M.m01 + d.yy * M.m11 + d.yz * M.m21);
    o.m12 = 2.0f * (d.xy * M.m02 + d.yy * M.m12 + d.yz * M.m22);
    o.m20 = 2.0f * (d.xz * M.m00 + d.yz * M.m10 + d.zz * M.m20);
    o.m21 = 2.0f * (d.xz * M.m01 + d.yz * M.m11 + d.zz * M.m21);
    o.m22 = 2.0f * (d.xz * M.m02 + d.yz * M.m12 + d.zz * M.m22);
    return o;
}

__device__ __forceinline__ float4 grad_quat(const QuatRot& q, const M3& g) {
    const float w = q.w, x = q.x, y = q.y, z = q.z;
    const float dw = 2.0f * (-z * g.m01 + y * g.m02 + z * g.m10 - x * g.m12 + -y * g.m20 + x * g.m21);
    const float dx = 2.0f * (y * g.m01 + z * g.m02 + y * g.m10 - 2.0f * x * g.m11 - w * g.m12 +
                             z * g.m20 + w * g.m21 - 2.0f * x * g.m22);
    const float dy = 2.0f * (-2.0f * y * g.m00 + x * g.m01 + w * g.m02 + x * g.m10 + z * g.m12 +
                             -w * g.m20 + z * g.m21 - 2.0f * y * g.m22);
    const float dz = 2.0f * (-2.0f * z * g.m00 - w * g.m01 + x * g.m02 + w * g.m10 -
                             2.0f * z * g.m11 + y * g.m12 + x * g.m20 + y * g.m21);
    const float dot = dw * w + dx * x + dy * y + dz * z;
    return make_float4(q.inv_norm * (dw - w * dot), q.inv_norm * (dx - x * dot),
                       q.inv_norm * (dy - y * dot), q.inv_norm * (dz - z * dot));
}

__device__ __forceinline__ void add_grad_t_from_cov(const Sym2& g, const Sym3& S, const M3& W, V3 t,
                                                    float fx, float fy, const Jac& J, const M23& T, V3& dt,
                                                    float (&K)[6]) {
    const M23 TS = times_sym3(T, S);
    const float k0 = 2.0f * (g.a * TS.r0x + g.b * TS.r1x), k1 = 2.0f * (g.a * TS.r0y + g.b * TS.r1y);
    const float k2 = 2.0f * (g.a * TS.r0z + g.b * TS.r1z), k3 = 2.0f * (g.b * TS.r0x + g.c * TS.r1x);
    const float k4 = 2.0f * (g.b * TS.r0y + g.c * TS.r1y), k5 = 2.0f * (g.b * TS.r0z + g.c * TS.r1z);
    K[0] = k0; K[1] = k1; K[2] = k2; K[3] = k3; K[4] = k4; K[5] = k5;
    const float j0 = k0 * W.m00 + k1 * W.m01 + k2 * W.m02;
    const float j2 = k0 * W.m20 + k1 * W.m21 + k2 * W.m22;
    const float j4 = k3 * W.m10 + k4 * W.m11 + k5 * W.m12;
    const float j5 = k3 * W.m20 + k4 * W.m21 + k5 * W.m22;
    const float tz_inv3 = J.tz_inv2 * J.tz_inv;
    dt.x += j2 * (-fx * J.tz_inv2);
    dt.y += j5 * (-fy * J.tz_inv2);
    dt.z += j0 * (-fx * J.tz_inv2) + j2 * (2.0f * fx * t.x * tz_inv3) + j4 * (-fy * J.tz_inv2) +
            j5 * (2.0f * fy * t.y * tz_inv3);
}

struct PBPtrs {
    const float* positions; const float* rotations; const float* scales; const float* opacities;
    const float* sh; const int32_t* radii; const uint8_t* colour_gate;
    const float* grad_accum;
    const float* g_means; const float* g_cov; const float* g_rgb; const float* g_opa;
    float* d_pos; float* d_rot; float* d_scl; float* d_opa; float* d_sh; float* d_means_out;
    float* d_rgb_gated_out;
    float* w_pos; float* w_rot; float* w_scl; float* w_opa; float* w_sh;
};

struct PoseArgs {
    float* partial;
    float* rows;
};
constexpr int POSE_TERMS = 12;

__device__ __forceinline__ void pose_block_partial(const float (&v)[POSE_TERMS], float* s_red, float* __restrict__ out) {
    const int lane = (int)threadIdx.x & (CUGS_WAVE - 1), wave = (int)threadIdx.x / CUGS_WAVE;
    float r = reduce12r16(v, lane);
    r += __shfl_xor(r, 16);
    r += __shfl_xor(r, 32);
    __syncthreads();
    const int slot = reduce12r16_slot(lane);
    if (lane < 16 && slot >= 0) s_red[wave * POSE_TERMS + slot] = r;
    __syncthreads();
    if (threadIdx.x < POSE_TERMS) {
        float acc = s_red[threadIdx.x];
#pragma unroll
        for (int w = 1; w < CUGS_BLOCK / CUGS_WAVE; ++w) acc += s_red[w * POSE_TERMS + threadIdx.x];
        out[threadIdx.x] = acc;
    }
}

template <int C, bool ALIGNED, bool ADAM, bool FACTORS = false, bool MCMC = false, bool POSE = false, bool SPARSE = false>
__global__ __launch_bounds__(CUGS_BLOCK) void k_project_backward(int64_t n, int degree, CamArgs cam, PBPtrs p,
                                                                AdamFusedArgs adam, McmcFusedArgs mc, PoseArgs pose) {
    static_assert(!MCMC || ADAM, "the MCMC route is the fused optimizer step's");
    static_assert(!FACTORS || (C == 16 && ALIGNED), "factor tile: degree-3 storage, 16-byte rows");
    static_assert(!SPARSE || (ADAM && !MCMC), "the sparse route is the fused optimizer step's, and not MCMC's");
    constexpr int LROW = FACTORS ? SH_FACTOR_ROW : ShTile<C>::LROW;
    constexpr int VIS_WORDS = (SPARSE && !FACTORS) ? CUGS_BLOCK : 0;
    __shared__ __attribute__((aligned(16))) float s_sh[CUGS_BLOCK * LROW + VIS_WORDS];
    const int64_t base = (int64_t)blockIdx.x * CUGS_BLOCK;
    const int count = (int)min((int64_t)CUGS_BLOCK, n - base);
    const int64_t idx = base + threadIdx.x;
    const bool live = idx < n;
    const int num_active = active_count(degree);
    auto ldp = [](const float* q_) { return ADAM ? *q_ : cugs_ldnt(q_); };

    const bool gate_from_sh = !FACTORS && (p.colour_gate == nullptr);
    if (gate_from_sh) {
        load_sh_rows<C, ALIGNED>(p.sh, base, count, s_sh);
        __syncthreads();
    }

    float Y[16] = {0.0f, 0.0f, 0.0f, 0.0f, 0.0f, 0.0f, 0.0f, 0.0f, 0.0f, 0.0f, 0.0f, 0.0f, 0.0f, 0.0f, 0.0f, 0.0f};
    float gated[3] = {0.0f, 0.0f, 0.0f};
    V3 pos{0.0f, 0.0f, 0.0f};
    float g_mx = 0.0f, g_my = 0.0f, g_opa = 0.0f;
    Sym2 g_inv{0.0f, 0.0f, 0.0f};
    GradMoments mom{0.0f, 0.0f, 0.0f, 0.0f, 0.0f};
    float g_z = 0.0f;
    const bool from_rows = (p.grad_accum != nullptr);
    float in_scl[3] = {0.0f, 0.0f, 0.0f}, in_opa = 0.0f;
    float4 in_q = make_float4(0.0f, 0.0f, 0.0f, 0.0f);
    int in_radius = 0;
    if (FACTORS && live) {
        in_radius = p.radii[idx];
        if (!SPARSE || in_radius > 0) {
            in_scl[0] = ldp(p.scales + idx * 3 + 0); in_scl[1] = ldp(p.scales + idx * 3 + 1); in_scl[2] = ldp(p.scales + idx * 3 + 2);
            in_q = ADAM ? reinterpret_cast<const float4*>(p.rotations)[idx] : cugs_ldnt(reinterpret_cast<const float4*>(p.rotations) + idx);
            in_opa = ldp(p.opacities + idx);
        }
    }
    if constexpr (SPARSE && !FACTORS) {
        if (live) in_radius = p.radii[idx];
    }
    const bool work = SPARSE ? (live && in_radius > 0) : live;
    if (work) {
        pos = V3{ldp(p.positions + idx * 3 + 0), ldp(p.positions + idx * 3 + 1), ldp(p.positions + idx * 3 + 2)};
        float g_rgb[3];
        if (from_rows) {
            const float4* row = reinterpret_cast<const float4*>(p.grad_accum + idx * CUGS_GRAD_STRIDE);
            const float4 r0 = row[0], r1 = row[1];
            g_rgb[0] = r0.x; g_rgb[1] = r0.y; g_rgb[2] = r0.z; g_opa = r0.w;
            const float2 r2 = *reinterpret_cast<const float2*>(p.grad_accum + idx * CUGS_GRAD_STRIDE + 8);
            mom = GradMoments{r1.x, r1.y, r1.z, r1.w, r2.x};
            g_z = r2.y;
        } else {
            g_rgb[0] = p.g_rgb[idx * 3 + 0]; g_rgb[1] = p.g_rgb[idx * 3 + 1]; g_rgb[2] = p.g_rgb[idx * 3 + 2];
            g_opa = p.g_opa[idx];
            g_mx = p.g_means[idx * 2 + 0]; g_my = p.g_means[idx * 2 + 1];
            g_inv = Sym2{p.g_cov[idx * 3 + 0], p.g_cov[idx * 3 + 1], p.g_cov[idx * 3 + 2]};
        }
        sh_basis(degree, view_direction(pos, cam), Y);
#pragma unroll
        for (int ch = 0; ch < 3; ++ch) {
            bool open;
            if (gate_from_sh) open = raw_colour_backward(s_sh + threadIdx.x * LROW + ch * C, Y, num_active) > 0.0f;
            else open = ((p.colour_gate[idx] >> ch) & 1u) != 0u;
            gated[ch] = g_rgb[ch] * (open ? 1.0f : 0.0f);
            if (p.d_rgb_gated_out) p.d_rgb_gated_out[idx * 3 + ch] = gated[ch];
        }
    }
    if (gate_from_sh) __syncthreads();

    if (FACTORS) {
        if (ADAM || p.d_sh) {
            if (work) {
                float4* row = reinterpret_cast<float4*>(s_sh + threadIdx.x * SH_FACTOR_ROW);
                row[0] = make_float4(Y[0], Y[1], Y[2], Y[3]);
                row[1] = make_float4(Y[4], Y[5], Y[6], Y[7]);
                row[2] = make_float4(Y[8], Y[9], Y[10], Y[11]);
                row[3] = make_float4(Y[12], Y[13], Y[14], Y[15]);
                row[4] = make_float4(gated[0], gated[1], gated[2], SPARSE ? 1.0f : 0.0f);
            } else if constexpr (SPARSE) {
                if (live) reinterpret_cast<float4*>(s_sh + threadIdx.x * SH_FACTOR_ROW)[4] = make_float4(0.0f, 0.0f, 0.0f, 0.0f);
            }
            __syncthreads();
            if (ADAM) adam_sh_rows_from_factors<SPARSE>(p.w_sh, adam.m[1], adam.v[1], base, count, num_active, s_sh, adam.lr[1], adam);
            else store_sh_rows_from_factors(p.d_sh, base, count, num_active, s_sh);
        }
    } else if (ADAM || p.d_sh) {
        if constexpr (SPARSE) {
            if (live) s_sh[CUGS_BLOCK * LROW + threadIdx.x] = work ? 1.0f : 0.0f;
        }
        if (work) {
            float* row = s_sh + threadIdx.x * LROW;
#pragma unroll
            for (int ch = 0; ch < 3; ++ch)
#pragma unroll
                for (int k = 0; k < C; ++k) row[ch * C + k] = (k < num_active) ? gated[ch] * Y[k] : 0.0f;
        }
        __syncthreads();
        if (ADAM) adam_sh_rows<C, ALIGNED, SPARSE>(p.w_sh, adam.m[1], adam.v[1], base, count, s_sh, adam.lr[1], adam,
                                                   s_sh + CUGS_BLOCK * LROW);
        else store_sh_rows<C, ALIGNED>(p.d_sh, base, count, s_sh);
    }
    if (!POSE && !live) return;
    float pg[POSE_TERMS];
#pragma unroll
    for (int k = 0; k < POSE_TERMS; ++k) pg[k] = 0.0f;

    if (work) {
        V3 d_pos{0.0f, 0.0f, 0.0f}, d_log{0.0f, 0.0f, 0.0f};
        float4 d_q = make_float4(0.0f, 0.0f, 0.0f, 0.0f);
        float d_logit = 0.0f;
        if (((FACTORS || SPARSE) ? in_radius : p.radii[idx]) > 0) {
            const M3 W = view_rotation(cam);
            const V3 t = to_camera(cam, W, pos);
            if (!FACTORS) {
                in_scl[0] = ldp(p.scales + idx * 3 + 0); in_scl[1] = ldp(p.scales + idx * 3 + 1); in_scl[2] = ldp(p.scales + idx * 3 + 2);
            }
            const V3 s{cugs_expf(in_scl[0] + cam.log_mod), cugs_expf(in_scl[1] + cam.log_mod), cugs_expf(in_scl[2] + cam.log_mod)};
            const float4 q = FACTORS ? in_q
                           : ALIGNED ? (ADAM ? reinterpret_cast<const float4*>(p.rotations)[idx]
                                             : cugs_ldnt(reinterpret_cast<const float4*>(p.rotations) + idx))
                                     : make_float4(p.rotations[idx * 4 + 0], p.rotations[idx * 4 + 1],
                                                   p.rotations[idx * 4 + 2], p.rotations[idx * 4 + 3]);
            const QuatRot qr = rotation_of(q.x, q.y, q.z, q.w);
            const M3 M = scale_columns(qr.R, s);
            const Sym3 S = gram(M);
            const Jac J = jacobian(t, cam.fx, cam.fy);
            const Sym2 cov = screen_covariance(project_matrix_full(J, W), S);
            Sym2 inv;
            if (invert_sym2(cov, inv) > 0.0f) {
                if (from_rows) {
                    const Grad2D g2 = grads_from_moments(mom, inv.a, inv.b, inv.c);
                    g_mx = g2.mx; g_my = g2.my;
                    g_inv = Sym2{g2.a, g2.b, g2.c};
                }
                const M23 T = project_matrix_sparse(J, W);
                const Sym2 g_cov = grad_cov_from_inv(inv, g_inv);
                const Sym3 g_S = grad_cov3d(T, g_cov);
                const M3 g_M = grad_M(g_S, M);
                const M3 g_R{g_M.m00 * s.x, g_M.m01 * s.y, g_M.m02 * s.z, g_M.m10 * s.x, g_M.m11 * s.y,
                             g_M.m12 * s.z, g_M.m20 * s.x, g_M.m21 * s.y, g_M.m22 * s.z};
                const M3& R = qr.R;
                d_log.x = (g_M.m00 * R.m00 + g_M.m10 * R.m10 + g_M.m20 * R.m20) * s.x;
                d_log.y = (g_M.m01 * R.m01 + g_M.m11 * R.m11 + g_M.m21 * R.m21) * s.y;
                d_log.z = (g_M.m02 * R.m02 + g_M.m12 * R.m12 + g_M.m22 * R.m22) * s.z;
                d_q = grad_quat(qr, g_R);

                V3 dt{0.0f, 0.0f, 0.0f};
                dt.x += g_mx * cam.fx * J.tz_inv;
                dt.y += g_my * cam.fy * J.tz_inv;
                dt.z += g_mx * (-cam.fx * t.x * J.tz_inv2) + g_my * (-cam.fy * t.y * J.tz_inv2);
                float K[6];
                add_grad_t_from_cov(g_cov, S, W, t, cam.fx, cam.fy, J, T, dt, K);
                dt.z = (g_z != 0.0f) ? dt.z + g_z : dt.z;
                if (POSE) {
                    pg[0] = dt.x * pos.x + J.j00 * K[0]; pg[1] = dt.x * pos.y + J.j00 * K[1]; pg[2] = dt.x * pos.z + J.j00 * K[2];
                    pg[3] = dt.y * pos.x + J.j11 * K[3]; pg[4] = dt.y * pos.y + J.j11 * K[4]; pg[5] = dt.y * pos.z + J.j11 * K[5];
                    pg[6] = dt.z * pos.x + (J.j02 * K[0] + J.j12 * K[3]);
                    pg[7] = dt.z * pos.y + (J.j02 * K[1] + J.j12 * K[4]);
                    pg[8] = dt.z * pos.z + (J.j02 * K[2] + J.j12 * K[5]);
                    pg[9] = dt.x; pg[10] = dt.y; pg[11] = dt.z;
                }
                d_pos.x = W.m00 * dt.x + W.m10 * dt.y + W.m20 * dt.z;
                d_pos.y = W.m01 * dt.x + W.m11 * dt.y + W.m21 * dt.z;
                d_pos.z = W.m02 * dt.x + W.m12 * dt.y + W.m22 * dt.z;

                const float sig = cugs_sigmoidf(FACTORS ? in_opa : ldp(p.opacities + idx));
                d_logit = g_opa * sig * (1.0f - sig);
// ... 270 lines not shown
```

cuda-gaussian-splatting_amd/csrc/raster_backward.hip:

```cpp
#include "cugs_raster_common.h"

#include <cstdlib>

#ifdef CUGS_DEV
bool cugs_dev_backward_stats();
#endif

namespace {

#define CUGS_BWD_HITS 4
static_assert(CUGS_BWD_HITS == CUGS_HIT_GROUP, "a hit group is one flush");
#ifndef CUGS_BWD_ABS_WAVES
#define CUGS_BWD_ABS_WAVES 7
#endif
#ifndef CUGS_BWD_HSTRIDE
#define CUGS_BWD_HSTRIDE 64
#endif

template <bool PACKED, bool WIDE, bool STATS, bool DEPTH = false, bool ABS = false>
__global__ __launch_bounds__(CUGS_BLOCK) __attribute__((amdgpu_waves_per_eu(ABS ? CUGS_BWD_ABS_WAVES : (DEPTH ? 7 : 8))))
void k_raster_backward(RasterGeom geo, RasterSrc src,
                                                                const float* __restrict__ dL_dcolor,
                                                                const float* __restrict__ final_T,
                                                                const int32_t* __restrict__ n_contrib,
                                                                float* __restrict__ grad_accum, int64_t stats_row,
                                                                const float* __restrict__ depths,
                                                                const float* __restrict__ dL_ddepth_map,
                                                                const float* __restrict__ dL_dalpha) {
    __shared__ float4 s_rec[CUGS_BLOCK * CUGS_REC_F4];
    __shared__ float2 s_contrib[4][CUGS_BWD_HITS][CUGS_BWD_HSTRIDE];

#ifdef CUGS_DEV
    const bool no_atomics = stats_row == -2;
#else
    constexpr bool no_atomics = false;
#endif
    unsigned tile;
    int range_start, range_end;
    if (src.tile_order) {
        const uint4 rec = src.tile_order[blockIdx.x];
        tile = rec.x; range_start = (int)rec.y; range_end = (int)rec.z;
    } else {
        tile = cugs_blend_tile(blockIdx.x, (unsigned)geo.ntx, (unsigned)(geo.ntiles / geo.ntx));
        range_start = src.tile_ranges[tile * 2 + 0];
        range_end = src.tile_ranges[tile * 2 + 1];
    }
    const int tile_x = (int)(tile % (unsigned)geo.ntx), tile_y = (int)(tile / (unsigned)geo.ntx);
    const int tid = threadIdx.x, wave = tid >> 6, lane = tid & 63;
    const int quad_x = tile_x * CUGS_TILE + (wave & 1) * 8, quad_y = tile_y * CUGS_TILE + (wave >> 1) * 8;
    const int px = quad_x + (lane & 7), py = quad_y + (lane >> 3);
    const bool inside = (px < geo.width) && (py < geo.height);
    const float pxf = (float)px + 0.5f, pyf = (float)py + 0.5f;
    const float qx0 = (float)quad_x + 0.5f, qy0 = (float)quad_y + 0.5f;

    const int num_in_range = range_end - range_start;
    const int num_batches = (num_in_range + CUGS_BLOCK - 1) / CUGS_BLOCK;

    const int pix = py * geo.width + px;
    float T = inside ? final_T[pix] : 0.0f;
    const int max_contrib = inside ? n_contrib[pix] : 0;
    float dC0 = 0.0f, dC1 = 0.0f, dC2 = 0.0f;
    if (inside) {
        dC0 = dL_dcolor[pix * 3 + 0];
        dC1 = dL_dcolor[pix * 3 + 1];
        dC2 = dL_dcolor[pix * 3 + 2];
    }
    float dDp = 0.0f;
    if (DEPTH && inside && dL_ddepth_map) dDp = dL_ddepth_map[pix];
    const int h2 = lane >> 4, g2i = lane & 15;
    const int gx0 = quad_x + (g2i & 1) * 4, gy = quad_y + (g2i >> 1);
    const float px2 = (float)gx0 + 0.5f, py2 = (float)gy + 0.5f;
    const bool side = (lane & 8) != 0;
    float eA[4], eB[4], e2[4], eZ[4];
#pragma unroll
    for (int i = 0; i < 4; ++i) {
        float r = 0.0f, gg = 0.0f, bb = 0.0f, zz = 0.0f;
        if (gx0 + i < geo.width && gy < geo.height) {
            const int pq = gy * geo.width + gx0 + i, q = pq * 3;
            r = dL_dcolor[q + 0]; gg = dL_dcolor[q + 1]; bb = dL_dcolor[q + 2];
            if (DEPTH && dL_ddepth_map) zz = dL_ddepth_map[pq];
        }
        eA[i] = side ? gg : r; eB[i] = side ? r : gg; e2[i] = bb; eZ[i] = zz;
    }
    const int slot2 = ABS ? reduce12ar16_slot(lane, DEPTH) : DEPTH ? reduce10r16_slot(lane) : reduce9r16_slot(lane);
    const unsigned slot_off = (unsigned)(slot2 < 0 ? 0 : slot2) * 4u;
    unsigned long long hitrecs = 0ull;

    float D = fmaf(dC2, T * geo.bg2, fmaf(dC1, T * geo.bg1, dC0 * (T * geo.bg0)));
    if (DEPTH && inside && dL_dalpha) D = fmaf(-T, dL_dalpha[pix], D);
    float rem = (inside && max_contrib > 0) ? (float)max_contrib : -1.0f;
    bool wave_done = (__ballot(rem >= 0.0f) == 0ull);
    int pending = 0;
    unsigned st_steps = 0, st_contrib = 0, st_lanes = 0, st_batches = 0, st_tested = 0, st_open = 0;

    auto flush = [&](int cnt) {
        const int rec = (int)((hitrecs >> (16 * h2)) & 0xFFFFull);
        const float4* c4 = reinterpret_cast<const float4*>(&s_contrib[wave][h2][g2i * 4]);
        const float4 p01 = c4[0], p23 = c4[1];
        float4 head;
        if (ABS) {
            head = s_rec[rec];
        } else {
            const float2 m = *reinterpret_cast<const float2*>(&s_rec[rec]);
            head = make_float4(m.x, m.y, 0.0f, 0.0f);
        }
        const float2 mean = make_float2(head.x, head.y);
        const float4 tail = s_rec[rec + 1];
        const float dy = py2 - mean.y;
        const float dx0 = px2 - mean.x, dx1 = dx0 + 1.0f, dx2 = dx0 + 2.0f, dx3 = dx0 + 3.0f;
        float t = p01.y * dx0;
        float A = p01.y, M1 = t, Mxx = t * dx0;
        float RA = p01.x * eA[0], RB = p01.x * eB[0], R2 = p01.x * e2[0];
        t = p01.w * dx1; A += p01.w; M1 += t; Mxx = fmaf(t, dx1, Mxx);
        RA = fmaf(p01.z, eA[1], RA); RB = fmaf(p01.z, eB[1], RB); R2 = fmaf(p01.z, e2[1], R2);
        t = p23.y * dx2; A += p23.y; M1 += t; Mxx = fmaf(t, dx2, Mxx);
        RA = fmaf(p23.x, eA[2], RA); RB = fmaf(p23.x, eB[2], RB); R2 = fmaf(p23.x, e2[2], R2);
        t = p23.w * dx3; A += p23.w; M1 += t; Mxx = fmaf(t, dx3, Mxx);
        RA = fmaf(p23.z, eA[3], RA); RB = fmaf(p23.z, eB[3], RB); R2 = fmaf(p23.z, e2[3], R2);
        const float oA = tail.y * A;
        M1 *= tail.y; Mxx *= tail.y;
        const float M1y = dy * oA, Myy = dy * M1y, Mxy = dy * M1;
        float total;
        if (ABS) {
            const float bdy = head.w * dy, cdy = tail.x * dy;
            float SX = fabsf(p01.y) * fabsf(fmaf(head.z, dx0, bdy));
            float SY = fabsf(p01.y) * fabsf(fmaf(head.w, dx0, cdy));
            SX = fmaf(fabsf(p01.w), fabsf(fmaf(head.z, dx1, bdy)), SX);
            SY = fmaf(fabsf(p01.w), fabsf(fmaf(head.w, dx1, cdy)), SY);
            SX = fmaf(fabsf(p23.y), fabsf(fmaf(head.z, dx2, bdy)), SX);
            SY = fmaf(fabsf(p23.y), fabsf(fmaf(head.w, dx2, cdy)), SY);
            SX = fmaf(fabsf(p23.w), fabsf(fmaf(head.z, dx3, bdy)), SX);
// ... 22 lines not shown
                atomicAdd(reinterpret_cast<float*>(reinterpret_cast<char*>(grad_accum) + off), total);
            }
        }
    };

    auto step = [&](const int rec, const int slot) __attribute__((always_inline)) {
        if (STATS) ++st_steps;
        const float4 g0 = s_rec[rec], g1 = s_rec[rec + 1], col = s_rec[rec + 2];
        const float o = g1.y;

        PixelEval e;
        const float alpha = pixel_alpha_raw(pxf, pyf, g0.x, g0.y, g0.z, g0.w, g1.x, o, 1.0f, e);
        const float passf = passes_alpha_min(alpha);
        const float k = sat_mul(passf, rem);
        rem -= passf;
        const float al = alpha * k;
        const float gk = k * below_alpha_cap(alpha);

        const float rcp = __builtin_amdgcn_rcpf(1.0f - al);
        T *= rcp;
        const float weight = al * T;
        float G = fmaf(dC2, col.w, fmaf(dC1, col.z, dC0 * col.x));
        if (DEPTH) G = fmaf(dDp, col.y, G);
        const float gate = fmaf(T, G, -(rcp * D)) * gk;
        D = fmaf(weight, G, D);
        if (STATS) {
            const unsigned long long lm = __ballot(k != 0.0f);
            if (lm) { ++st_contrib; st_lanes += __popcll(lm); st_open += __popcll(__ballot(rem >= 0.0f)); }
        }
        s_contrib[wave][slot][lane] = make_float2(weight, gate * e.e);
    };

    for (int batch = num_batches - 1; batch >= 0; --batch) {
        if (lane == 0) s_contrib[wave][0][0].x = wave_done ? 1.0f : 0.0f;
        __syncthreads();
        if (s_contrib[0][0][0].x * s_contrib[1][0][0].x * s_contrib[2][0][0].x * s_contrib[3][0][0].x != 0.0f) break;

        stage_record<PACKED, DEPTH>(src, range_start + batch * CUGS_BLOCK + tid, range_end, s_rec, depths);
        __syncthreads();

        if (STATS && !wave_done) ++st_batches;
        if (!wave_done) {
            const int batch_count = min(CUGS_BLOCK, num_in_range - batch * CUGS_BLOCK);
            const int nsub = (batch_count + CUGS_WAVE - 1) / CUGS_WAVE;
            for (int sub = nsub - 1; sub >= 0 && !wave_done; --sub) {
                const int j = sub * CUGS_WAVE + lane;
                const ActiveRect ar = active_rect(__ballot(rem >= 0.0f), qx0, qy0);
                bool hit = false;
                if (j < batch_count)
                    hit = may_touch_quad(s_rec[j * CUGS_REC_F4 + 0], s_rec[j * CUGS_REC_F4 + 1], ar.x0, ar.y0, ar.wx,
                                         ar.wy);
                unsigned long long mask = __ballot(hit);
                if (STATS) st_tested += min(CUGS_WAVE, batch_count - sub * CUGS_WAVE);
                const unsigned rec_sub = (unsigned)(sub * CUGS_WAVE * CUGS_REC_F4);
                while (pending + __popcll(mask) >= CUGS_BWD_HITS) {
                    if (pending == 0) {
                        hitrecs = cugs_pop_hits4_desc(mask, rec_sub);
                    } else {
                        do hitrecs = cugs_set_hit(hitrecs, pending, rec_sub + cugs_pop_hit_desc(mask) * CUGS_REC_F4);
                        while (++pending < CUGS_BWD_HITS);
                        pending = 0;
                    }
                    step(cugs_hit(hitrecs, 0), 0);
                    step(cugs_hit(hitrecs, 1), 1);
                    step(cugs_hit(hitrecs, 2), 2);
                    step(cugs_hit(hitrecs, 3), 3);
                    const bool closed = (__ballot(rem >= 0.0f) == 0ull);
                    flush(CUGS_BWD_HITS);
                    if (closed) { wave_done = true; mask = 0ull; break; }
                }
                while (mask != 0ull) {
                    hitrecs = cugs_set_hit(hitrecs, pending, rec_sub + cugs_pop_hit_desc(mask) * CUGS_REC_F4);
                    ++pending;
                }
            }
            if (pending) {
                for (int p = 0; p < pending; ++p) step(cugs_hit(hitrecs, p), p);
                if (__ballot(rem >= 0.0f) == 0ull) wave_done = true;
                flush(pending);
                pending = 0;
            }
        }
    }
    if (STATS && lane == 0) {
        float* st = grad_accum + (int64_t)stats_row * CUGS_GRAD_STRIDE;
        atomicAdd(&st[0], (float)st_steps); atomicAdd(&st[1], (float)st_contrib); atomicAdd(&st[2], (float)st_lanes);
        atomicAdd(&st[3], (float)st_batches); atomicAdd(&st[4], (float)st_tested); atomicAdd(&st[5], (float)num_batches);
        atomicAdd(&st[7], (float)st_open);
    }
}

template <bool PACKED, bool DEPTH = false, bool ABS = false>
__global__ __launch_bounds__(CUGS_BLOCK) void k_unpack_grads(int64_t n, const float* __restrict__ acc,
                                                             const float* __restrict__ packed,
                                                             const float* __restrict__ cov_2d_inv,
                                                             float* __restrict__ dL_drgb,
                                                             float* __restrict__ dL_dopa,
                                                             float* __restrict__ dL_dmeans,
                                                             float* __restrict__ dL_dcov,
                                                             float* __restrict__ dL_ddepths,
                                                             float* __restrict__ dL_dmeans_abs) {
    const int64_t i = (int64_t)blockIdx.x * CUGS_BLOCK + threadIdx.x;
    if (i >= n) return;
    const float4* row = reinterpret_cast<const float4*>(acc + i * CUGS_GRAD_STRIDE);
    const float4 r0 = row[0], r1 = row[1];
    float r2;
    if (ABS) {
        const float4 w = row[2];
        r2 = w.x;
        if (DEPTH) dL_ddepths[i] = w.y;
        *reinterpret_cast<float2*>(dL_dmeans_abs + i * 2) = make_float2(w.z, w.w);
    } else if (DEPTH) {
        const float2 w89 = *reinterpret_cast<const float2*>(acc + i * CUGS_GRAD_STRIDE + 8);
        r2 = w89.x;
        dL_ddepths[i] = w89.y;
    } else {
        r2 = acc[i * CUGS_GRAD_STRIDE + 8];
    }
    float a, b, c;
    if (PACKED) {
        const float4* rec = reinterpret_cast<const float4*>(packed + i * CUGS_PACKED_STRIDE);
        const float4 p0 = rec[0];
        a = p0.z; b = p0.w; c = rec[1].x;
    } else {
        a = cov_2d_inv[i * 3 + 0]; b = cov_2d_inv[i * 3 + 1]; c = cov_2d_inv[i * 3 + 2];
    }
    dL_drgb[i * 3 + 0] = r0.x; dL_drgb[i * 3 + 1] = r0.y; dL_drgb[i * 3 + 2] = r0.z;
    dL_dopa[i] = r0.w;
    const GradMoments m{r1.x, r1.y, r1.z, r1.w, r2};
    const Grad2D g = grads_from_moments(m, a, b, c);
    dL_dmeans[i * 2 + 0] = g.mx; dL_dmeans[i * 2 + 1] = g.my;
    dL_dcov[i * 3 + 0] = g.a; dL_dcov[i * 3 + 1] = g.b; dL_dcov[i * 3 + 2] = g.c;
}

}

extern "C" int cugs_rasterize_backward_opts(int width, int height, const float background_host[3],
                                            const int32_t* tile_ranges, const int32_t* gaussian_indices,
                                            const float* means_2d, const float* cov_2d_inv, const float* rgb,
                                            const float* opacities_act, const float* packed,
                                            const float* dL_dcolor, const float* final_T,
                                            const int32_t* n_contrib, int64_t n, float* grad_accum,
                                            float* dL_drgb, float* dL_dopacity_act, float* dL_dmeans_2d,
                                            float* dL_dcov_2d_inv, const cugs_blend_backward_opts* opts, void* stream) {
    const cugs_blend_backward_opts o = opts ? *opts : cugs_blend_backward_opts{};
    const bool depth_map = o.depths || o.dL_ddepth_map || o.dL_dalpha;
    const bool abs_grad = o.abs_grad != 0;
    if (width < 0 || height < 0 || n < 0 || !background_host) return CUGS_EINVAL;
    if (n == 0) return 0;
    if (!grad_accum) return CUGS_EINVAL;
    if ((reinterpret_cast<uintptr_t>(grad_accum) & 63u) != 0) return CUGS_EALIGN;
    const int n_soa = (dL_drgb != nullptr) + (dL_dopacity_act != nullptr) + (dL_dmeans_2d != nullptr) +
                      (dL_dcov_2d_inv != nullptr);
    if (n_soa != 0 && n_soa != 4) return CUGS_EINVAL;
    if (depth_map && (n_soa == 4) != (o.dL_ddepths != nullptr)) return CUGS_EINVAL;
    if (!depth_map && o.dL_ddepths) return CUGS_EINVAL;
    if (abs_grad && (n_soa == 4) != (o.dL_dmeans_2d_abs != nullptr)) return CUGS_EINVAL;
    if (n_soa == 4 && !packed && !cov_2d_inv) return CUGS_EINVAL;
    if (packed && !cugs_aligned16(packed)) return CUGS_EALIGN;
    if (o.tile_order && !cugs_aligned16(o.tile_order)) return CUGS_EALIGN;
    hipStream_t st = static_cast<hipStream_t>(stream);
    int64_t rows = n;
#ifdef CUGS_DEV
    const bool stats = cugs_dev_backward_stats();
    if (stats) rows = n + 1;
#endif
    if (!o.prezeroed || rows != n)
        CUGS_RETURN_IF_HIP(hipMemsetAsync(grad_accum, 0, sizeof(float) * CUGS_GRAD_STRIDE * (size_t)rows, st));

    const int ntx = (width + CUGS_TILE - 1) / CUGS_TILE, nty = (height + CUGS_TILE - 1) / CUGS_TILE;
    if (ntx > 0 && nty > 0 && gaussian_indices) {
        if (!tile_ranges || !dL_dcolor || !final_T || !n_contrib) return CUGS_EINVAL;
        if (!packed && (!means_2d || !cov_2d_inv || !rgb || !opacities_act)) return CUGS_EINVAL;
        if (depth_map && !o.depths) return CUGS_EINVAL;
        if ((int64_t)width * height > 2147483647ll / 3) return CUGS_EOVERFLOW;
        RasterGeom geo{width, height, ntx, ntx * nty, background_host[0], background_host[1], background_host[2]};
        RasterSrc src{tile_ranges, gaussian_indices, packed, means_2d, cov_2d_inv, rgb, opacities_act, reinterpret_cast<const uint4*>(o.tile_order)};
        const bool wide = rows > (int64_t(1) << 26);
        int64_t stats_arg = n;
#ifdef CUGS_DEV
        if (const char* e = std::getenv("CUGS_BWD_NO_ATOMICS")) if (e[0] == '1') stats_arg = -2;
#endif
        const auto launch = [&](auto* kernel) {
            hipLaunchKernelGGL(kernel, dim3(geo.ntiles), dim3(CUGS_BLOCK), 0, st, geo, src, dL_dcolor, final_T, n_contrib,
                               grad_accum, stats_arg, o.depths, o.dL_ddepth_map, o.dL_dalpha);
        };
#ifdef CUGS_DEV
        if (stats && !depth_map && !abs_grad)
            cugs_with_bool(packed != nullptr, [&](auto P) { launch(k_raster_backward<P(), true, true>); });
        else
#endif
        cugs_with_bool(packed != nullptr, [&](auto P) { cugs_with_bool(wide, [&](auto W) {
            cugs_with_bool(depth_map, [&](auto D) { cugs_with_bool(abs_grad, [&](auto A) {
                launch(k_raster_backward<P(), W(), false, D(), A()>);
            }); });
        }); });
        CUGS_LAUNCH_CHECK();
    }
    if (n_soa == 4) {
        const dim3 grid((unsigned)((n + CUGS_BLOCK - 1) / CUGS_BLOCK));
        cugs_with_bool(packed != nullptr, [&](auto P) { cugs_with_bool(depth_map, [&](auto D) {
            cugs_with_bool(abs_grad, [&](auto A) {
                hipLaunchKernelGGL((k_unpack_grads<P(), D(), A()>), grid, dim3(CUGS_BLOCK), 0, st, n, grad_accum, packed,
                                   cov_2d_inv, dL_drgb, dL_dopacity_act, dL_dmeans_2d, dL_dcov_2d_inv, o.dL_ddepths,
                                   o.dL_dmeans_2d_abs);
            });
        }); });
        CUGS_LAUNCH_CHECK();
    }
    return 0;
}

extern "C" int cugs_rasterize_backward(int width, int height, const float background_host[3],
                                       const int32_t* tile_ranges, const int32_t* gaussian_indices,
                                       const float* means_2d, const float* cov_2d_inv, const float* rgb,
                                       const float* opacities_act, const float* packed,
                                       const float* dL_dcolor, const float* final_T,
                                       const int32_t* n_contrib, int64_t n, float* grad_accum,
                                       float* dL_drgb, float* dL_dopacity_act, float* dL_dmeans_2d,
                                       float* dL_dcov_2d_inv, void* stream) {
    return cugs_rasterize_backward_opts(width, height, background_host, tile_ranges, gaussian_indices, means_2d, cov_2d_inv,
                                        rgb, opacities_act, packed, dL_dcolor, final_T, n_contrib, n, grad_accum, dL_drgb,
                                        dL_dopacity_act, dL_dmeans_2d, dL_dcov_2d_inv, nullptr, stream);
}

#ifdef CUGS_DEV
namespace {
__global__ void k_dbg_reduce9(const float* __restrict__ in, float* __restrict__ out, int* __restrict__ slots) {
    const int l = threadIdx.x;
    const bool side = (l & 8) != 0;
    const float v0 = in[0 * 64 + l], v1 = in[1 * 64 + l];
    out[l] = reduce9t(side ? v1 : v0, side ? v0 : v1, in[2 * 64 + l], in[3 * 64 + l], in[4 * 64 + l], in[5 * 64 + l],
                      in[6 * 64 + l], in[8 * 64 + l], in[7 * 64 + l]);
    slots[l] = reduce9t_slot(l);
}
__global__ void k_dbg_reduce9r16(const float* __restrict__ in, float* __restrict__ out, int* __restrict__ slots) {
    const int l = threadIdx.x;
    const bool side = (l & 8) != 0;
    const float v0 = in[0 * 64 + l], v1 = in[1 * 64 + l];
    out[l] = reduce9r16(side ? v1 : v0, side ? v0 : v1, in[2 * 64 + l], in[3 * 64 + l], in[4 * 64 + l], in[5 * 64 + l],
                        in[6 * 64 + l], in[8 * 64 + l], in[7 * 64 + l], l);
    slots[l] = reduce9r16_slot(l);
}
__global__ void k_dbg_reduce10r16(const float* __restrict__ in, float* __restrict__ out, int* __restrict__ slots) {
    const int l = threadIdx.x;
    const bool side = (l & 8) != 0;
    const float v0 = in[0 * 64 + l], v1 = in[1 * 64 + l];
    out[l] = reduce10r16(side ? v1 : v0, side ? v0 : v1, in[2 * 64 + l], in[3 * 64 + l], in[4 * 64 + l], in[5 * 64 + l],
                         in[6 * 64 + l], in[8 * 64 + l], in[7 * 64 + l], in[9 * 64 + l], l);
    slots[l] = reduce10r16_slot(l);
}
__global__ void k_dbg_reduce12ar16(const float* __restrict__ in, float* __restrict__ out, int* __restrict__ slots,
                                   int* __restrict__ slots_nodepth) {
    const int l = threadIdx.x;
    const bool side = (l & 8) != 0;
    const float v0 = in[0 * 64 + l], v1 = in[1 * 64 + l];
    out[l] = reduce12ar16(side ? v1 : v0, side ? v0 : v1, in[2 * 64 + l], in[3 * 64 + l], in[4 * 64 + l], in[5 * 64 + l],
                          in[6 * 64 + l], in[8 * 64 + l], in[7 * 64 + l], in[9 * 64 + l], in[10 * 64 + l], in[11 * 64 + l],
                          l);
    slots[l] = reduce12ar16_slot(l, true);
    slots_nodepth[l] = reduce12ar16_slot(l, false);
}
__global__ void k_dbg_rcp(const float* __restrict__ in, float* __restrict__ out, int n) {
    const int i = blockIdx.x * blockDim.x + threadIdx.x;
    if (i < n) out[i] = __builtin_amdgcn_rcpf(in[i]);
}
__global__ void k_dbg_blend_exp(const float* __restrict__ q, float* __restrict__ out, int n) {
    const int i = blockIdx.x * blockDim.x + threadIdx.x;
// ... 73 lines not shown
```

cuda-gaussian-splatting_amd/rasterizer.py:

```python
from __future__ import annotations

import ctypes as C
from typing import Dict, Optional, Sequence

import torch

from . import _lib
from ._lib import lib, check
from .types import (BackwardOutput, CameraInfo, ForwardOutput, GaussianModel, ProjectionBackwardOutput,
                    ProjectionOutput, RasterizeBackwardOutput, RenderOutput, RenderSettings,
                    SortingOutput, K_TILE_SIZE)


def _torch_check(cond: bool, msg: str) -> None:
    if not cond:
        raise RuntimeError(msg)


def _ptr(t: Optional[torch.Tensor]) -> C.c_void_p:
    return C.c_void_p(0 if t is None or t.numel() == 0 else t.data_ptr())


def _stream(device: torch.device) -> C.c_void_p:
    return C.c_void_p(torch.cuda.current_stream(device).cuda_stream)


def _f32c(t: torch.Tensor) -> torch.Tensor:
    return t.contiguous().to(torch.float32)


_workspaces: Dict[tuple, torch.Tensor] = {}
SORT_CONTROL_BYTES = 256


def _skey(device: torch.device) -> tuple:
    return (device, int(torch.cuda.current_stream(device).cuda_stream))


_pinned = {}


class _PinnedSlot:

    def __init__(self, tensor, pool):
        self.tensor, self._pool = tensor, pool

    def release(self):
        if self._pool is not None:
            pool, self._pool = self._pool, None
            pool.append(self.tensor)

    def __del__(self):
        try:
            self.release()
        except Exception:
            pass


def _pinned_total(device: torch.device) -> "_PinnedSlot":
    pool = _pinned.setdefault(device, [])
    return _PinnedSlot(pool.pop() if pool else torch.zeros(1, dtype=torch.int64).pin_memory(), pool)


def _workspace(device: torch.device, nbytes: int, kind: str = "n") -> torch.Tensor:
    key = (_skey(device), kind)
    ws = _workspaces.get(key)
    if ws is None or ws.numel() < nbytes:
        ws = torch.empty(int(nbytes * 1.25) + 4096, dtype=torch.uint8, device=device)
        ws[:SORT_CONTROL_BYTES].zero_()
        _workspaces[key] = ws
    return ws


_side_streams = {}


def _side_stream(device: torch.device) -> torch.cuda.Stream:
    key = _skey(device)
    st = _side_streams.get(key)
    if st is None:
        try:
            least, _greatest = torch.cuda.Stream.priority_range()
        except Exception:
            least = 0
        st = torch.cuda.Stream(device=device, priority=least)
        _side_streams[key] = st
    return st


def project_gaussians(positions: torch.Tensor, rotations: torch.Tensor, scales: torch.Tensor,
                      opacities: torch.Tensor, sh_coeffs: torch.Tensor, camera: CameraInfo,
                      active_sh_degree: int, scale_modifier: float = 1.0,
                      want_colour_gate: bool = True, key_sort: bool = False,
                      colour_on_side_stream: bool = False) -> ProjectionOutput:
    _torch_check(positions.is_cuda, "positions must be on CUDA")
    _torch_check(positions.dim() == 2 and positions.shape[1] == 3, "positions must be [N, 3]")
    n = int(positions.shape[0])
    dev = positions.device
    f = dict(dtype=torch.float32, device=dev)
    i = dict(dtype=torch.int32, device=dev)
    means_2d = torch.empty((n, 2), **f)
    depths = torch.empty((n,), **f)
    cov_2d_inv = torch.empty((n, 3), **f)
    radii = torch.empty((n,), **i)
    tiles_touched = torch.empty((n,), **i)
    opacities_act = torch.empty((n,), **f)
    rgb = torch.empty((n, 3), **f)
    packed = torch.empty((n, _lib.PACKED_STRIDE), **f)
    colour_gate = torch.empty((n,), dtype=torch.uint8, device=dev) if want_colour_gate else None
    if n == 0:
        return ProjectionOutput(means_2d, depths, cov_2d_inv, radii, tiles_touched, rgb, opacities_act, packed,
                                colour_gate)
    _torch_check(sh_coeffs.dim() == 3 and sh_coeffs.shape[1] == 3 and sh_coeffs.shape[0] == n,
                 "sh_coeffs must be [N, 3, C]")
    num_coeffs = int(sh_coeffs.shape[2])
    _torch_check(0 <= active_sh_degree <= 3, f"SH degree must be 0..3, got {active_sh_degree}")
    _torch_check((active_sh_degree + 1) ** 2 <= num_coeffs,
                 f"Need at least {(active_sh_degree + 1) ** 2} coefficients for degree {active_sh_degree}")
    pos_c, rot_c, scl_c, opa_c, sh_c = map(_f32c, (positions, rotations, scales, opacities, sh_coeffs))
    cam = camera.to_abi()
    outs = (_ptr(means_2d), _ptr(depths), _ptr(cov_2d_inv), _ptr(radii), _ptr(tiles_touched), _ptr(opacities_act),
            _ptr(rgb), _ptr(packed), _ptr(colour_gate))
    if colour_on_side_stream:
        ws = _workspace(dev, lib.cugs_sort_workspace_bytes(n), "n") if key_sort else None
        main = torch.cuda.current_stream(dev)
        side = _side_stream(dev)
        start = torch.cuda.Event()
        start.record(main)
        check(lib.cugs_project_forward_geometry(n, _ptr(pos_c), _ptr(rot_c), _ptr(scl_c), _ptr(opa_c), C.byref(cam),
                                                float(scale_modifier), _ptr(means_2d), _ptr(depths), _ptr(cov_2d_inv),
                                                _ptr(radii), _ptr(tiles_touched), _ptr(opacities_act), _ptr(packed),
                                                _ptr(ws), ws.numel() if ws is not None else 0, _stream(dev)),
              "cugs_project_forward_geometry")
        side.wait_event(start)
        check(lib.cugs_project_forward_colour(n, num_coeffs, int(active_sh_degree), _ptr(pos_c), _ptr(sh_c), C.byref(cam),
                                              _ptr(rgb), _ptr(packed), _ptr(colour_gate),
                                              C.c_void_p(side.cuda_stream)), "cugs_project_forward_colour")
        done = torch.cuda.Event()
        done.record(side)
        return ProjectionOutput(means_2d, depths, cov_2d_inv, radii, tiles_touched, rgb, opacities_act, packed,
                                colour_gate, sort_workspace=ws, colour_ready=done)
    if key_sort:
        ws = _workspace(dev, lib.cugs_sort_workspace_bytes(n), "n")
        check(lib.cugs_project_forward_keyed(n, num_coeffs, int(active_sh_degree), _ptr(pos_c), _ptr(rot_c),
                                             _ptr(scl_c), _ptr(opa_c), _ptr(sh_c), C.byref(cam), float(scale_modifier),
                                             *outs, _ptr(ws), ws.numel(), _stream(dev)), "cugs_project_forward_keyed")
        return ProjectionOutput(means_2d, depths, cov_2d_inv, radii, tiles_touched, rgb, opacities_act, packed,
                                colour_gate, sort_workspace=ws)
    check(lib.cugs_project_forward(n, num_coeffs, int(active_sh_degree), _ptr(pos_c), _ptr(rot_c), _ptr(scl_c),
                                   _ptr(opa_c), _ptr(sh_c), C.byref(cam), float(scale_modifier),
                                   *outs, _stream(dev)), "cugs_project_forward")
    return ProjectionOutput(means_2d, depths, cov_2d_inv, radii, tiles_touched, rgb, opacities_act, packed,
                            colour_gate)


def evaluate_sh_cuda(degree: int, sh_coeffs: torch.Tensor, directions: torch.Tensor) -> torch.Tensor:
    _torch_check(0 <= degree <= 3, f"SH degree must be 0..3, got {degree}")
    _torch_check(sh_coeffs.is_cuda, "sh_coeffs must be on CUDA device")
    _torch_check(directions.is_cuda, "directions must be on CUDA device")
    _torch_check(sh_coeffs.dim() == 3 and sh_coeffs.shape[1] == 3, "sh_coeffs must be [N, 3, C]")
    _torch_check(directions.dim() == 2 and directions.shape[1] == 3, "directions must be [N, 3]")
    _torch_check(sh_coeffs.shape[0] == directions.shape[0], "Batch size mismatch")
    num_coeffs = int(sh_coeffs.shape[2])
    _torch_check(num_coeffs >= (degree + 1) ** 2,
                 f"Need at least {(degree + 1) ** 2} coefficients for degree {degree}")
    n = int(sh_coeffs.shape[0])
    coeffs, dirs = _f32c(sh_coeffs), _f32c(directions)
    out = torch.empty((n, 3), dtype=torch.float32, device=sh_coeffs.device)
    if n == 0:
        return out
    check(lib.cugs_evaluate_sh(int(degree), n, num_coeffs, _ptr(coeffs), _ptr(dirs), _ptr(out),
                               _stream(out.device)), "cugs_evaluate_sh")
    return out


def evaluate_sh_backward_cuda(degree: int, sh_coeffs: torch.Tensor, directions: torch.Tensor,
                              dL_dcolor: torch.Tensor) -> torch.Tensor:
    _torch_check(0 <= degree <= 3, f"SH degree must be 0..3, got {degree}")
    _torch_check(sh_coeffs.is_cuda, "sh_coeffs must be on CUDA device")
    _torch_check(directions.is_cuda, "directions must be on CUDA device")
    _torch_check(dL_dcolor.is_cuda, "dL_dcolor must be on CUDA device")
    _torch_check(sh_coeffs.dim() == 3 and sh_coeffs.shape[1] == 3, "sh_coeffs must be [N, 3, C]")
    _torch_check(directions.dim() == 2 and directions.shape[1] == 3, "directions must be [N, 3]")
    _torch_check(dL_dcolor.dim() == 2 and dL_dcolor.shape[1] == 3, "dL_dcolor must be [N, 3]")
    n, num_coeffs = int(sh_coeffs.shape[0]), int(sh_coeffs.shape[2])
    _torch_check(num_coeffs >= (degree + 1) ** 2, "not enough SH coefficients for the degree")
    coeffs, dirs, g = _f32c(sh_coeffs), _f32c(directions), _f32c(dL_dcolor)
    out = torch.empty_like(coeffs)
    if n == 0:
        return out
    check(lib.cugs_evaluate_sh_backward(int(degree), n, num_coeffs, _ptr(coeffs), _ptr(dirs), _ptr(g),
                                        _ptr(out), _stream(out.device)), "cugs_evaluate_sh_backward")
    return out


TILE_ORDER = True
TILE_ORDER_MIN_PAIRS = 2_000_000


def wants_tile_order(dev) -> bool:
    return bool(TILE_ORDER) and _last_pairs.get(_skey(dev), 0) >= TILE_ORDER_MIN_PAIRS

# ... 110 lines not shown
        out = sort_gaussians(means_2d, depths, radii, tiles_touched, img_w, img_h, want_keys, wide_depth=wide,
                             want_tile_order=want_tile_order)
        _last_pairs[key] = out.total_pairs
        return out
    cap = _capacity_for(dev, last)
    i32 = dict(dtype=torch.int32, device=dev)
    tile_ranges = torch.empty((ntx * nty, 2), **i32)
    keys = torch.empty((cap if want_keys else 0,), dtype=torch.int64, device=dev)
    vals = torch.empty((cap,), **i32)
    tiles_c = tiles_touched.contiguous().to(torch.int32)
    means_c, depths_c, radii_c = means_2d.contiguous(), depths.contiguous(), radii.contiguous()
    ws = keyed_workspace if keyed_workspace is not None else _workspace(dev, lib.cugs_sort_workspace_bytes(n), "n")
    wp = _workspace(dev, lib.cugs_sort_pair_workspace_bytes(cap), "p")
    slot = _pinned_total(dev)
    total = slot.tensor
    entry = lib.cugs_sort_pairs_predicted_keyed if keyed_workspace is not None else lib.cugs_sort_pairs_predicted
    if wide:
        entry = lib.cugs_sort_pairs_predicted_wide
    common = (n, cap, _ptr(means_c), _ptr(depths_c), _ptr(radii_c), _ptr(tiles_c), int(img_w), int(img_h), _ptr(ws),
              ws.numel(), _ptr(wp), wp.numel(), _ptr(keys) if want_keys else C.c_void_p(0), _ptr(vals),
              _ptr(tile_ranges), C.cast(total.data_ptr(), C.POINTER(C.c_int64)))
    tile_order = None
    if want_tile_order and keyed_workspace is not None and not wide:
        tile_order = torch.empty((ntx * nty, 4), **i32)
        check(lib.cugs_sort_pairs_predicted_keyed_ordered(*common, _ptr(tile_order), _stream(dev)),
              "cugs_sort_pairs_predicted_keyed_ordered")
    else:
        check(entry(*common, _stream(dev)), "cugs_sort_pairs_predicted")
        if want_tile_order:
            tile_order = tile_order_of(tile_ranges, img_w, img_h)
    ev = torch.cuda.Event()
    ev.record()
    return PendingSort((means_c, depths_c, radii_c, tiles_c, img_w, img_h, want_keys), keys, vals, tile_ranges, cap, slot, ev,
                       key, tile_order=tile_order)


def rasterize_forward(means_2d: torch.Tensor, cov_2d_inv: torch.Tensor, rgb: torch.Tensor,
                      opacities: torch.Tensor, tile_ranges: torch.Tensor, gaussian_indices: torch.Tensor,
                      img_w: int, img_h: int, background: Sequence[float],
                      packed: Optional[torch.Tensor] = None, zero_buf: Optional[torch.Tensor] = None,
                      tile_order: Optional[torch.Tensor] = None,
                      depths: Optional[torch.Tensor] = None) -> ForwardOutput:
    _torch_check(means_2d.is_cuda, "means_2d must be on CUDA")
    dev = means_2d.device
    color = torch.empty((img_h, img_w, 3), dtype=torch.float32, device=dev)
    final_T = torch.empty((img_h, img_w), dtype=torch.float32, device=dev)
    n_contrib = torch.empty((img_h, img_w), dtype=torch.int32, device=dev)
    depth_map = None
    if depths is not None:
        _torch_check(depths.is_cuda and depths.device == dev, "depths must be on the device of means_2d")
        _torch_check(depths.dim() == 1 and depths.shape[0] == means_2d.shape[0], "depths must be [N]")
        depth_map = torch.empty((img_h, img_w), dtype=torch.float32, device=dev)
    if img_w == 0 or img_h == 0:
        if zero_buf is not None:
            zero_buf.zero_()
        return ForwardOutput(color, final_T, n_contrib, depth_map)
    bg = (C.c_float * 3)(*[float(b) for b in background])
    if zero_buf is not None:
        _torch_check(zero_buf.is_contiguous() and zero_buf.dtype == torch.float32 and zero_buf.numel() % 4 == 0,
                     "zero_buf must be a contiguous float32 tensor of a multiple of four elements")
    if tile_order is not None:
        _torch_check(tile_order.is_contiguous() and tile_order.dtype == torch.int32 and
                     tile_order.numel() == 4 * tile_ranges.shape[0], "tile_order must be a contiguous [tiles, 4] int32 tensor")
    z = None if depths is None else _f32c(depths)
    opts = _lib.BlendForwardOpts(_ptr(zero_buf), zero_buf.numel() * 4 if zero_buf is not None else 0, _ptr(tile_order),
                                 _ptr(z), _ptr(depth_map))
    check(lib.cugs_rasterize_forward_opts(int(img_w), int(img_h), bg, _ptr(tile_ranges.contiguous()),
                                          _ptr(gaussian_indices.contiguous()), _ptr(means_2d.contiguous()),
                                          _ptr(cov_2d_inv.contiguous()), _ptr(rgb.contiguous()),
                                          _ptr(opacities.contiguous()), _ptr(packed), _ptr(color), _ptr(final_T),
                                          _ptr(n_contrib), C.byref(opts), _stream(dev)), "cugs_rasterize_forward_opts")
    return ForwardOutput(color, final_T, n_contrib, depth_map)


def rasterize_backward(dL_dcolor: torch.Tensor, means_2d: torch.Tensor, cov_2d_inv: torch.Tensor,
                       rgb: torch.Tensor, opacities: torch.Tensor, tile_ranges: torch.Tensor,
                       gaussian_indices: torch.Tensor, final_T: torch.Tensor, n_contrib: torch.Tensor,
                       img_w: int, img_h: int, background: Sequence[float], n_gaussians: int,
                       packed: Optional[torch.Tensor] = None, unpack: bool = True,
                       zeroed_accum: Optional[torch.Tensor] = None,
                       tile_order: Optional[torch.Tensor] = None, depths: Optional[torch.Tensor] = None,
                       dL_ddepth_map: Optional[torch.Tensor] = None,
                       dL_dalpha: Optional[torch.Tensor] = None,
                       want_abs_grad: bool = False) -> RasterizeBackwardOutput:
    _torch_check(dL_dcolor.is_cuda, "dL_dcolor must be on CUDA")
    dev = dL_dcolor.device
    n = int(n_gaussians)
    f = dict(dtype=torch.float32, device=dev)
    depth_route = depths is not None or dL_ddepth_map is not None or dL_dalpha is not None
    if depth_route:
        _torch_check(depths is not None, "the depth / alpha map gradients need the projection's depths")
        _torch_check(depths.is_cuda and depths.device == dev and depths.dim() == 1 and depths.shape[0] == n,
                     "depths must be [N] on the device of dL_dcolor")
        for name, g in (("dL_ddepth_map", dL_ddepth_map), ("dL_dalpha", dL_dalpha)):
            if g is not None:
                _torch_check(g.is_cuda and g.device == dev, f"{name} must be on the device of dL_dcolor")
                _torch_check(tuple(g.shape) == (int(img_h), int(img_w)), f"{name} must be [H, W] = [{img_h}, {img_w}]")
    if zeroed_accum is not None:
        _torch_check(tuple(zeroed_accum.shape) == (n, _lib.GRAD_STRIDE) and zeroed_accum.is_contiguous(),
                     "zeroed_accum must be a contiguous [N, 16] float32 tensor")
    accum = zeroed_accum if zeroed_accum is not None else torch.empty((n, _lib.GRAD_STRIDE), **f)
    if unpack:
        d_rgb, d_opa = torch.empty((n, 3), **f), torch.empty((n,), **f)
        d_means, d_cov = torch.empty((n, 2), **f), torch.empty((n, 3), **f)
    else:
        d_rgb = d_opa = d_means = d_cov = None
    d_z = torch.empty((n,), **f) if unpack and depth_route else None
    d_abs = None
    if want_abs_grad:
        d_abs = torch.empty((n, 2), **f) if unpack else accum[:, 10:12]
    if n > 0 and tile_order is not None:
        _torch_check(tile_order.is_contiguous() and tile_order.dtype == torch.int32 and
                     tile_order.numel() == 4 * tile_ranges.shape[0], "tile_order must be a contiguous [tiles, 4] int32 tensor")
    if n > 0:
        bg = (C.c_float * 3)(*[float(b) for b in background])
        z, g_depth, g_alpha = (None if t is None else _f32c(t) for t in (depths, dL_ddepth_map, dL_dalpha))
        opts = _lib.BlendBackwardOpts(1 if zeroed_accum is not None else 0, 1 if want_abs_grad else 0, _ptr(tile_order),
                                      _ptr(z), _ptr(g_depth), _ptr(g_alpha), _ptr(d_z),
                                      _ptr(d_abs) if unpack else None)
        check(lib.cugs_rasterize_backward_opts(int(img_w), int(img_h), bg, _ptr(tile_ranges.contiguous()),
                                               _ptr(gaussian_indices.contiguous()), _ptr(means_2d.contiguous()),
                                               _ptr(cov_2d_inv.contiguous()), _ptr(rgb.contiguous()),
                                               _ptr(opacities.contiguous()), _ptr(packed),
                                               _ptr(dL_dcolor.contiguous()), _ptr(final_T.contiguous()),
                                               _ptr(n_contrib.contiguous()), n, _ptr(accum), _ptr(d_rgb), _ptr(d_opa),
                                               _ptr(d_means), _ptr(d_cov), C.byref(opts), _stream(dev)),
              "cugs_rasterize_backward_opts")
    return RasterizeBackwardOutput(d_rgb, d_opa, d_means, d_cov, accum, dL_ddepths=d_z, dL_dmeans_2d_abs=d_abs)


def project_backward(dL_dmeans_2d: Optional[torch.Tensor], dL_dcov_2d_inv: Optional[torch.Tensor],
                     dL_drgb: Optional[torch.Tensor], dL_dopacity_act: Optional[torch.Tensor],
                     positions: torch.Tensor, rotations: torch.Tensor, scales: torch.Tensor,
                     opacities: torch.Tensor, sh_coeffs: torch.Tensor, radii: torch.Tensor,
                     camera: CameraInfo, active_sh_degree: int, scale_modifier: float = 1.0,
                     grad_accum: Optional[torch.Tensor] = None, colour_gate: Optional[torch.Tensor] = None,
                     dL_dmeans_2d_out: Optional[torch.Tensor] = None,
                     dL_drgb_gated_out: Optional[torch.Tensor] = None,
                     skip_sh_grad: bool = False,
                     geom_flat: Optional[torch.Tensor] = None, want_camera_grad: bool = False,
                     dL_dview_rows: Optional[torch.Tensor] = None) -> ProjectionBackwardOutput:
    _torch_check(positions.is_cuda, "positions must be on CUDA")
    n = int(positions.shape[0])
    dev = positions.device
    f = dict(dtype=torch.float32, device=dev)
    _torch_check(dL_dview_rows is None or want_camera_grad, "dL_dview_rows needs want_camera_grad=True")
    _check_pose_rows(dL_dview_rows, n, dev)
    d_view = torch.empty((4, 4), **f) if want_camera_grad else None
    if geom_flat is not None:
        d_rot, d_pos, d_scl, d_opa = geometry_views(geom_flat, n)
    else:
        d_pos, d_rot = torch.empty((n, 3), **f), torch.empty((n, 4), **f)
        d_scl, d_opa = torch.empty((n, 3), **f), torch.empty((n, 1), **f)
    sh_c = _f32c(sh_coeffs)
    d_sh = None if skip_sh_grad else torch.empty_like(sh_c)
    if n == 0:
        if d_view is not None:
            d_view.zero_()
        return ProjectionBackwardOutput(d_pos, d_rot, d_scl, d_opa, d_sh, dL_dviewmat=d_view)
    pos_c, rot_c, scl_c, opa_c = map(_f32c, (positions, rotations, scales, opacities))
    cam = camera.to_abi()
    cont = lambda t: None if t is None else t.contiguous()
    args = (n, int(sh_c.shape[2]), int(active_sh_degree), _ptr(pos_c), _ptr(rot_c), _ptr(scl_c), _ptr(opa_c), _ptr(sh_c),
            _ptr(radii.contiguous()), _ptr(cont(colour_gate)), C.byref(cam), float(scale_modifier),
            _ptr(cont(grad_accum)), _ptr(cont(dL_dmeans_2d)), _ptr(cont(dL_dcov_2d_inv)), _ptr(cont(dL_drgb)),
            _ptr(cont(dL_dopacity_act)), _ptr(d_pos), _ptr(d_rot), _ptr(d_scl), _ptr(d_opa), _ptr(d_sh),
            _ptr(dL_dmeans_2d_out), _ptr(dL_drgb_gated_out))
    if want_camera_grad:
        pg = _pose_grad(d_view, dL_dview_rows, n, dev)
        check(lib.cugs_project_backward_pose(*args, C.byref(pg), _stream(dev)), "cugs_project_backward_pose")
    else:
        check(lib.cugs_project_backward(*args, _stream(dev)), "cugs_project_backward")
    return ProjectionBackwardOutput(d_pos, d_rot, d_scl, d_opa, d_sh, dL_dviewmat=d_view)


def _check_pose_rows(rows: Optional[torch.Tensor], n: int, dev) -> None:
    _torch_check(rows is None or (tuple(rows.shape) == (n, 12) and rows.dtype == torch.float32 and rows.is_contiguous()
                                  and rows.device == dev), "dL_dview_rows must be a contiguous [N, 12] float32 tensor")


def _pose_grad(d_view: torch.Tensor, rows: Optional[torch.Tensor], n: int, dev) -> "_lib.PoseGrad":
    nbytes = int(lib.cugs_pose_grad_workspace_bytes(n))
    ws = _workspace(dev, nbytes, kind="pose")
    return _lib.PoseGrad(d_view.data_ptr(), None if rows is None else rows.data_ptr(), ws.data_ptr(), ws.numel())


def geometry_views(flat: torch.Tensor, n: int):
    _torch_check(flat.numel() == 11 * n and flat.is_contiguous(), "geom_flat must be a contiguous [11*N] tensor")
    return (flat[0:4 * n].view(n, 4), flat[4 * n:7 * n].view(n, 3), flat[7 * n:10 * n].view(n, 3),
            flat[10 * n:11 * n].view(n, 1))


def sh_backward_views(degree: int, positions: torch.Tensor, gated_rgb_views: torch.Tensor,
                      cam_centers, num_coeffs: int) -> torch.Tensor:
    _torch_check(positions.is_cuda and gated_rgb_views.is_cuda, "inputs must be on CUDA")
    v, n = int(gated_rgb_views.shape[0]), int(positions.shape[0])
    _torch_check(gated_rgb_views.shape == (v, n, 3), "gated_rgb_views must be [V, N, 3]")
    pos_c, g_c = _f32c(positions), _f32c(gated_rgb_views)
    out = torch.empty((n, 3, num_coeffs), dtype=torch.float32, device=positions.device)
    if n == 0:
        return out
    cc = (C.c_float * (3 * v))(*[float(x) for c in cam_centers for x in c])
    check(lib.cugs_sh_backward_views(int(degree), n, int(num_coeffs), _ptr(pos_c), v, _ptr(g_c), cc, _ptr(out),
                                     _stream(positions.device)), "cugs_sh_backward_views")
    return out


def gated_colour_grad(grad_accum: torch.Tensor, colour_gate: torch.Tensor,
                      out: Optional[torch.Tensor] = None) -> torch.Tensor:
    _torch_check(grad_accum.is_cuda and grad_accum.dim() == 2 and grad_accum.shape[1] == _lib.GRAD_STRIDE
                 and grad_accum.is_contiguous() and grad_accum.dtype == torch.float32,
                 "grad_accum must be a contiguous [N, 16] float32 CUDA tensor")
    n = int(grad_accum.shape[0])
    _torch_check(colour_gate is not None and colour_gate.dtype == torch.uint8 and colour_gate.numel() == n,
                 "colour_gate must be the [N] uint8 gate bits of project_gaussians")
    if out is None:
        out = torch.empty((n, 3), dtype=torch.float32, device=grad_accum.device)
    _torch_check(tuple(out.shape) == (n, 3) and out.is_contiguous() and out.dtype == torch.float32,
                 "out must be a contiguous [N, 3] float32 tensor")
    if n > 0:
        check(lib.cugs_gated_colour_grad(n, _ptr(grad_accum), _ptr(colour_gate.contiguous()), _ptr(out),
                                         _stream(grad_accum.device)), "cugs_gated_colour_grad")
    return out


OVERLAP_COLOUR = False


def render(model: GaussianModel, camera: CameraInfo, settings: RenderSettings, for_backward: bool = True,
           defer_count: bool = False, want_depth_map: bool = False) -> RenderOutput:
    _torch_check(model.is_valid(), "GaussianModel is not valid")
    _torch_check(model.positions.is_cuda, "GaussianModel must be on CUDA device")
    n = model.num_gaussians()
    dev = model.positions.device
    f = dict(dtype=torch.float32, device=dev)
    i = dict(dtype=torch.int32, device=dev)
    if n == 0:
        color = torch.empty((camera.height, camera.width, 3), **f)
        for ch in range(3):
            color[..., ch] = float(settings.background[ch])
        return RenderOutput(color, torch.ones((camera.height, camera.width), **f),
                            torch.zeros((camera.height, camera.width), **i), torch.empty((0, 2), **f),
                            torch.empty((0,), **f), torch.empty((0, 3), **f), torch.empty((0,), **i),
                            torch.empty((0, 3), **f), torch.empty((0,), **f), torch.empty((0,), **i),
                            torch.empty((0, 2), **i),
                            depth_map=torch.zeros((camera.height, camera.width), **f) if want_depth_map else None)
    active_degree = min(int(settings.active_sh_degree), model.max_sh_degree())
    wide = _wide_depth.get(_skey(dev), 0) > 0
    proj = project_gaussians(model.positions, model.rotations, model.scales, model.opacities, model.sh_coeffs,
                             camera, active_degree, settings.scale_modifier, want_colour_gate=for_backward,
                             key_sort=not wide,
                             colour_on_side_stream=OVERLAP_COLOUR)
    accum = torch.empty((n, _lib.GRAD_STRIDE), **f) if for_backward else None
    blend = lambda s: rasterize_forward(proj.means_2d, proj.cov_2d_inv, proj.rgb, proj.opacities_act, s.tile_ranges,
                                        s.gaussian_values_sorted, camera.width, camera.height, settings.background,
                                        packed=proj.packed, zero_buf=accum, tile_order=s.tile_order,
                                        depths=proj.depths if want_depth_map else None)
    srt = sort_gaussians_predicted(proj.means_2d, proj.depths, proj.radii, proj.tiles_touched, camera.width,
                                   camera.height, want_keys=False, keyed_workspace=proj.sort_workspace,
                                   want_tile_order=wants_tile_order(dev))
    proj.wait_colour()
    fwd = blend(srt)
    if defer_count and isinstance(srt, PendingSort):
        return RenderOutput(fwd.color, fwd.final_T, fwd.n_contrib, proj.means_2d, proj.depths, proj.cov_2d_inv,
                            proj.radii, proj.rgb, proj.opacities_act, srt.gaussian_values_sorted, srt.tile_ranges,
                            packed=proj.packed, colour_gate=proj.colour_gate, total_pairs=-1, zeroed_accum=accum,
                            pending=srt, tile_order=srt.tile_order, depth_map=fwd.depth_map)
    if isinstance(srt, PendingSort):
        srt, valid = srt.finish()
        if not valid:
            fwd = blend(srt)
    return RenderOutput(fwd.color, fwd.final_T, fwd.n_contrib, proj.means_2d, proj.depths, proj.cov_2d_inv,
                        proj.radii, proj.rgb, proj.opacities_act, srt.gaussian_values_sorted, srt.tile_ranges,
                        packed=proj.packed, colour_gate=proj.colour_gate, total_pairs=srt.total_pairs,
                        zeroed_accum=accum, tile_order=srt.tile_order, depth_map=fwd.depth_map)


def render_backward(dL_dcolor: torch.Tensor, render_out: RenderOutput, model: GaussianModel,
                    camera: CameraInfo, settings: RenderSettings,
                    dL_drgb_gated_out: Optional[torch.Tensor] = None,
                    geom_flat: Optional[torch.Tensor] = None, fused_adam=None, on_gated_ready=None,
                    mcmc=None, mcmc_step: int = 0, mcmc_noise: Optional[torch.Tensor] = None,
                    dL_ddepth_map: Optional[torch.Tensor] = None,
                    dL_dalpha: Optional[torch.Tensor] = None, want_camera_grad: bool = False,
                    want_abs_grad: bool = False, sparse_adam: bool = False) -> BackwardOutput:
    _torch_check(not sparse_adam or fused_adam is not None,
                 "sparse_adam needs fused_adam (otherwise: render_backward, apply_gradients, step(visible=radii))")
    _torch_check(not sparse_adam or mcmc is None,
                 "sparse_adam cannot be combined with the fused MCMC route: its regulariser and noise act on every "
                 "Gaussian")
    _torch_check(dL_dcolor.is_cuda, "dL_dcolor must be on CUDA device")
    _torch_check(dL_dcolor.dim() == 3 and dL_dcolor.shape[2] == 3, "dL_dcolor must be [H, W, 3]")
    depth_grads = dL_ddepth_map is not None or dL_dalpha is not None
    if depth_grads:
        _torch_check(dL_ddepth_map is None or render_out.depth_map is not None,
                     "dL_ddepth_map needs a render with the depth map (render(..., want_depth_map=True))")
        hw = (int(dL_dcolor.shape[0]), int(dL_dcolor.shape[1]))
        for name, g in (("dL_ddepth_map", dL_ddepth_map), ("dL_dalpha", dL_dalpha)):
            if g is not None:
                _torch_check(g.is_cuda and g.device == dL_dcolor.device, f"{name} must be on the device of dL_dcolor")
                _torch_check(tuple(g.shape) == hw, f"{name} must be [H, W] = [{hw[0]}, {hw[1]}]")
        _torch_check(dL_drgb_gated_out is None and geom_flat is None and on_gated_ready is None,
                     "the depth / alpha map gradients are not supported with the data-parallel gradient exchange "
                     "(dL_drgb_gated_out, geom_flat, on_gated_ready)")
    if want_camera_grad:
        _torch_check(dL_drgb_gated_out is None and geom_flat is None and on_gated_ready is None,
                     "the camera gradient is not supported with the data-parallel gradient exchange "
                     "(dL_drgb_gated_out, geom_flat, on_gated_ready)")
    n = model.num_gaussians()
    dev = dL_dcolor.device
    f = dict(dtype=torch.float32, device=dev)
    if n == 0:
        return BackwardOutput(torch.zeros((0, 3), **f), torch.zeros((0, 4), **f), torch.zeros((0, 3), **f),
                              torch.zeros((0, 1), **f), torch.zeros_like(model.sh_coeffs),
                              torch.zeros((0, 2), **f),
                              dL_dviewmat=torch.zeros((4, 4), **f) if want_camera_grad else None,
                              dL_dmeans_2d_abs=torch.zeros((0, 2), **f) if want_abs_grad else None)
    active_degree = min(int(settings.active_sh_degree), model.max_sh_degree())
    render_out.wait()
    zeroed, render_out.zeroed_accum = getattr(render_out, "zeroed_accum", None), None
    if zeroed is not None and getattr(zeroed, "_cugs_consumed", False):
        zeroed = None
    if zeroed is not None:
        zeroed._cugs_consumed = True
    rb = rasterize_backward(dL_dcolor, render_out.means_2d, render_out.cov_2d_inv, render_out.rgb,
                            render_out.opacities_act, render_out.tile_ranges, render_out.gaussian_indices,
                            render_out.final_T, render_out.n_contrib, camera.width, camera.height,
                            settings.background, n, packed=render_out.packed, unpack=False, zeroed_accum=zeroed,
                            tile_order=getattr(render_out, "tile_order", None),
                            depths=render_out.depths if depth_grads else None, dL_ddepth_map=dL_ddepth_map,
                            dL_dalpha=dL_dalpha, want_abs_grad=want_abs_grad)
    d_means_2d = torch.empty((n, 2), **f)
    if fused_adam is not None:
        _torch_check(fused_adam.model_ is model, "fused_adam must have been built on this model")
        _torch_check(dL_drgb_gated_out is None and geom_flat is None,
                     "the fused optimizer step is for single-GPU training (no gradient exchange)")
        _torch_check(render_out.colour_gate is not None, "the fused optimizer step needs render()'s colour_gate")
        if mcmc_noise is not None:
            _torch_check(mcmc is not None, "mcmc_noise needs mcmc")
            _torch_check(tuple(mcmc_noise.shape) == (n, 3) and mcmc_noise.is_cuda, "mcmc_noise must be [N, 3] on CUDA")
            mcmc_noise = mcmc_noise.contiguous().to(torch.float32)
        adam = fused_adam.begin_fused_step()
        cam = camera.to_abi()
        args = (n, int(model.sh_coeffs.shape[2]), active_degree, _ptr(model.positions), _ptr(model.rotations),
                _ptr(model.scales), _ptr(model.opacities), _ptr(model.sh_coeffs), _ptr(render_out.radii.contiguous()),
                _ptr(render_out.colour_gate.contiguous()), C.byref(cam), float(settings.scale_modifier),
                _ptr(rb.grad_accum), C.byref(adam))
        d_view = torch.empty((4, 4), **f) if want_camera_grad else None
        pg = _pose_grad(d_view, None, n, dev) if want_camera_grad else None
        if mcmc is not None:
            mc = mcmc.fused_args(mcmc_step, mcmc_noise)
            if pg is not None:
                check(lib.cugs_project_backward_adam_mcmc_pose(*args, C.byref(mc), _ptr(d_means_2d), C.byref(pg),
                                                               _stream(dev)), "cugs_project_backward_adam_mcmc_pose")
            else:
                check(lib.cugs_project_backward_adam_mcmc(*args, C.byref(mc), _ptr(d_means_2d), _stream(dev)),
                      "cugs_project_backward_adam_mcmc")
        elif sparse_adam and pg is not None:
            check(lib.cugs_project_backward_adam_sparse_pose(*args, _ptr(d_means_2d), C.byref(pg), _stream(dev)),
                  "cugs_project_backward_adam_sparse_pose")
        elif sparse_adam:
            check(lib.cugs_project_backward_adam_sparse(*args, _ptr(d_means_2d), _stream(dev)),
                  "cugs_project_backward_adam_sparse")
        elif pg is not None:
            check(lib.cugs_project_backward_adam_pose(*args, _ptr(d_means_2d), C.byref(pg), _stream(dev)),
                  "cugs_project_backward_adam_pose")
        else:
            check(lib.cugs_project_backward_adam(*args, _ptr(d_means_2d), _stream(dev)), "cugs_project_backward_adam")
        return BackwardOutput(None, None, None, None, None, d_means_2d, dL_dviewmat=d_view,
                              dL_dmeans_2d_abs=rb.dL_dmeans_2d_abs)
    _torch_check(mcmc is None, "the fused MCMC route needs fused_adam (otherwise: compute_regularization, "
                 "step, inject_noise)")
    gated_by_projection = dL_drgb_gated_out
    if on_gated_ready is not None:
        _torch_check(dL_drgb_gated_out is not None, "on_gated_ready needs dL_drgb_gated_out")
        _torch_check(render_out.colour_gate is not None, "on_gated_ready needs render()'s colour_gate")
        on_gated_ready(gated_colour_grad(rb.grad_accum, render_out.colour_gate, out=dL_drgb_gated_out))
        gated_by_projection = None
    pb = project_backward(None, None, None, None, model.positions, model.rotations, model.scales,
                          model.opacities, model.sh_coeffs, render_out.radii, camera, active_degree,
                          settings.scale_modifier, grad_accum=rb.grad_accum, colour_gate=render_out.colour_gate,
                          dL_dmeans_2d_out=d_means_2d, dL_drgb_gated_out=gated_by_projection,
                          skip_sh_grad=dL_drgb_gated_out is not None, geom_flat=geom_flat,
                          want_camera_grad=want_camera_grad)
    return BackwardOutput(pb.dL_dpositions, pb.dL_drotations, pb.dL_dscales, pb.dL_dopacities,
                          pb.dL_dsh_coeffs, d_means_2d, geom_flat=geom_flat, dL_dviewmat=pb.dL_dviewmat,
                          dL_dmeans_2d_abs=rb.dL_dmeans_2d_abs)
```

include/cugs_hip.h:

```cpp
#ifndef CUGS_HIP_H
#define CUGS_HIP_H

#include <stddef.h>
#include <stdint.h>

#ifdef __cplusplus
extern "C" {
#endif

#define CUGS_TILE 16
#define CUGS_PACKED_STRIDE 12
#define CUGS_GRAD_STRIDE 16

#define CUGS_EINVAL (-1)
#define CUGS_EALIGN (-2)
#define CUGS_EOVERFLOW (-3)
#define CUGS_EWORKSPACE (-4)

typedef struct cugs_camera {
    float view[16];
    float fx, fy, cx, cy;
    int32_t width, height;
    float cam_center[3];
    float reserved;
// ... 48 lines not shown
                          void* stream);

int cugs_sort_pairs(int64_t n, int64_t total_pairs, const float* means_2d, const float* depths,
                    const int32_t* radii, const int32_t* tiles_touched, int width, int height,
                    void* workspace, size_t workspace_bytes, void* pair_workspace,
                    size_t pair_workspace_bytes, uint64_t* keys_sorted, int32_t* values_sorted,
                    int32_t* tile_ranges, void* stream);

int cugs_sort_pairs_predicted(int64_t n, int64_t capacity, const float* means_2d, const float* depths,
                              const int32_t* radii, const int32_t* tiles_touched, int width, int height,
                              void* workspace, size_t workspace_bytes, void* pair_workspace,
                              size_t pair_workspace_bytes, uint64_t* keys_sorted, int32_t* values_sorted,
                              int32_t* tile_ranges, int64_t* total_pairs_host, void* stream);

int cugs_sort_pairs_predicted_keyed(int64_t n, int64_t capacity, const float* means_2d, const float* depths,
                                    const int32_t* radii, const int32_t* tiles_touched, int width, int height,
                                    void* workspace, size_t workspace_bytes, void* pair_workspace,
                                    size_t pair_workspace_bytes, uint64_t* keys_sorted, int32_t* values_sorted,
                                    int32_t* tile_ranges, int64_t* total_pairs_host, void* stream);

int cugs_sort_pairs_predicted_keyed_ordered(int64_t n, int64_t capacity, const float* means_2d, const float* depths,
                                            const int32_t* radii, const int32_t* tiles_touched, int width, int height,
                                            void* workspace, size_t workspace_bytes, void* pair_workspace,
                                            size_t pair_workspace_bytes, uint64_t* keys_sorted, int32_t* values_sorted,
                                            int32_t* tile_ranges, int64_t* total_pairs_host, uint32_t* tile_order,
                                            void* stream);

int cugs_tile_order(int width, int height, const int32_t* tile_ranges, uint32_t* tile_order, void* stream);

int cugs_sort_count_pairs_wide(int64_t n, const float* means_2d, const float* depths,
                               const int32_t* radii, const int32_t* tiles_touched, int width, int height,
                               void* workspace, size_t workspace_bytes, int64_t* total_pairs_host,
                               void* stream);
int cugs_sort_pairs_predicted_wide(int64_t n, int64_t capacity, const float* means_2d, const float* depths,
                                   const int32_t* radii, const int32_t* tiles_touched, int width, int height,
                                   void* workspace, size_t workspace_bytes, void* pair_workspace,
                                   size_t pair_workspace_bytes, uint64_t* keys_sorted, int32_t* values_sorted,
                                   int32_t* tile_ranges, int64_t* total_pairs_host, void* stream);

int cugs_rasterize_forward(int width, int height, const float background_host[3],
                           const int32_t* tile_ranges, const int32_t* gaussian_indices,
                           const float* means_2d, const float* cov_2d_inv, const float* rgb,
                           const float* opacities_act, const float* packed,
                           float* out_color, float* out_final_T, int32_t* out_n_contrib,
                           void* stream);

typedef struct cugs_blend_forward_opts {
    void* zero_buf;
    size_t zero_bytes;
    const uint32_t* tile_order;
    const float* depths;
    float* out_depth;
} cugs_blend_forward_opts;

int cugs_rasterize_forward_opts(int width, int height, const float background_host[3],
                                const int32_t* tile_ranges, const int32_t* gaussian_indices,
                                const float* means_2d, const float* cov_2d_inv, const float* rgb,
                                const float* opacities_act, const float* packed,
                                float* out_color, float* out_final_T, int32_t* out_n_contrib,
                                const cugs_blend_forward_opts* opts, void* stream);

int cugs_blend_scores(int width, int height, const int32_t* tile_ranges, const int32_t* gaussian_indices,
                      const float* means_2d, const float* cov_2d_inv, const float* opacities_act,
                      const float* packed, const void* tile_order, int n, void* scores, void* stream);

int cugs_rasterize_backward(int width, int height, const float background_host[3],
                            const int32_t* tile_ranges, const int32_t* gaussian_indices,
                            const float* means_2d, const float* cov_2d_inv, const float* rgb,
                            const float* opacities_act, const float* packed,
                            const float* dL_dcolor, const float* final_T,
                            const int32_t* n_contrib, int64_t n, float* grad_accum,
                            float* dL_drgb, float* dL_dopacity_act, float* dL_dmeans_2d,
                            float* dL_dcov_2d_inv, void* stream);

typedef struct cugs_blend_backward_opts {
    int prezeroed;
    int abs_grad;
    const uint32_t* tile_order;
    const float* depths;
    const float* dL_ddepth_map;
    const float* dL_dalpha;
    float* dL_ddepths;
    float* dL_dmeans_2d_abs;
} cugs_blend_backward_opts;

int cugs_rasterize_backward_opts(int width, int height, const float background_host[3],
                                 const int32_t* tile_ranges, const int32_t* gaussian_indices,
                                 const float* means_2d, const float* cov_2d_inv, const float* rgb,
                                 const float* opacities_act, const float* packed,
                                 const float* dL_dcolor, const float* final_T,
                                 const int32_t* n_contrib, int64_t n, float* grad_accum,
                                 float* dL_drgb, float* dL_dopacity_act, float* dL_dmeans_2d,
                                 float* dL_dcov_2d_inv, const cugs_blend_backward_opts* opts, void* stream);

int cugs_project_backward(int64_t n, int num_coeffs, int active_degree,
                          const float* positions, const float* rotations, const float* scales,
                          const float* opacities, const float* sh_coeffs, const int32_t* radii,
                          const uint8_t* colour_gate, const cugs_camera* camera_host,
                          float scale_modifier, const float* grad_accum,
                          const float* dL_dmeans_2d, const float* dL_dcov_2d_inv,
                          const float* dL_drgb, const float* dL_dopacity_act,
                          float* dL_dpositions, float* dL_drotations, float* dL_dscales,
                          float* dL_dopacities, float* dL_dsh_coeffs, float* dL_dmeans_2d_out,
                          float* dL_drgb_gated_out, void* stream);

typedef struct cugs_adam_fused {
    float* m[5];
    float* v[5];
    float lr[5];
    float beta1, beta2, eps, bc1, bc2;
} cugs_adam_fused;
int cugs_project_backward_adam(int64_t n, int num_coeffs, int active_degree, float* positions,
                               float* rotations, float* scales, float* opacities, float* sh_coeffs,
                               const int32_t* radii, const uint8_t* colour_gate,
                               const cugs_camera* camera_host, float scale_modifier,
                               const float* grad_accum, const cugs_adam_fused* adam_host,
                               float* dL_dmeans_2d_out, void* stream);

int cugs_sh_backward_views(int degree, int64_t n, int num_coeffs, const float* positions,
                           int num_views, const float* gated_rgb_views,
                           const float* cam_centers_host, float* dL_dsh, void* stream);

int cugs_gated_colour_grad(int64_t n, const float* grad_accum, const uint8_t* colour_gate,
                           float* dL_drgb_gated_out, void* stream);

void cugs_adam_bias_correction(float beta1, float beta2, int step, float* bc1_host,
                               float* bc2_host);

int cugs_fused_adam(float* param, const float* grad, float* m, float* v, int64_t n, float lr,
                    float beta1, float beta2, float eps, float bc1, float bc2, void* stream);

typedef struct cugs_adam_group {
    float* param;
    const float* grad;
    float* m;
    float* v;
    int64_t n;
    float lr;
    float reserved;
} cugs_adam_group;

int cugs_fused_adam_groups(const cugs_adam_group* groups_host, int ngroups, float beta1,
                           float beta2, float eps, float bc1, float bc2, void* stream);

int cugs_fused_adam_groups_rows(const cugs_adam_group* groups_host, int ngroups, const int32_t* row_elems_host,
                                const int32_t* radii, int64_t n_rows, float beta1, float beta2, float eps,
                                float bc1, float bc2, void* stream);

size_t cugs_loss_workspace_bytes(int width, int height);
int cugs_combined_loss(int width, int height, const float* rendered, const float* target, float lambda,
                       int window_size, void* workspace, size_t workspace_bytes, float* loss_out,
                       float* ssim_map, float* dL_dcolor, void* stream);

typedef struct cugs_loss_opts {
    const float* exposure;
    const float* mask;
    float*       dL_dexposure;
    float*       corrected;
} cugs_loss_opts;
size_t cugs_loss_opts_workspace_bytes(int width, int height);
int cugs_combined_loss_opts(int width, int height, const float* rendered, const float* target, float lambda,
                            int window_size, const cugs_loss_opts* opts, void* workspace, size_t workspace_bytes,
                            float* loss_out, float* ssim_map, float* dL_dcolor, void* stream);

typedef struct cugs_depth_loss_opts {
    const float* weight;
    const float* scale_shift;
    int          fit;
    int          inverse;
    float        min_alpha;
    float*       expected;
} cugs_depth_loss_opts;
size_t cugs_depth_loss_workspace_bytes(int width, int height);
int cugs_depth_loss(int width, int height, const float* depth_map, const float* alpha, const float* target,
                    const cugs_depth_loss_opts* opts, void* workspace, size_t workspace_bytes,
                    float* loss_out , float* dL_ddepth_map, float* dL_dalpha, void* stream);

typedef struct cugs_normal_loss_opts {
    const float* weight;
    float*       normals_out;
    float        cos_weight;
    float        l1_weight;
    float        min_alpha;
} cugs_normal_loss_opts;
size_t cugs_normal_loss_workspace_bytes(int width, int height);
int cugs_normal_loss(int width, int height, float fx, float fy, float cx, float cy, const float* depth_map,
                     const float* alpha, const float* target , const cugs_normal_loss_opts* opts,
// ... 144 lines not shown
```

Measured before the change: 2725.

## Pre-zero SH gradient buffer during blend backward, skip zero stores in projection

The SH-coefficient gradient buffer is now zeroed as a side task of the rasterize-backward kernel through a new zero_buf option. Projection backward then uses a new entry point that knows the buffer is already zero and can skip writing zeros for culled or gated Gaussians. The aim is to cut the SH gradient write traffic (1M x 48 floats) in projection backward by overlapping the zeroing with the tile-bound blend kernel. It adds a Python handover mechanism between calls and new API surface, and correctness depends on the buffer being zeroed before the projection kernel runs.

```diff
diff --git a/cuda-gaussian-splatting_amd/_lib.py b/cuda-gaussian-splatting_amd/_lib.py
--- a/cuda-gaussian-splatting_amd/_lib.py
+++ b/cuda-gaussian-splatting_amd/_lib.py
@@ -57,7 +57,7 @@
 class BlendBackwardOpts(C.Structure):
     _fields_ = [("prezeroed", C.c_int), ("abs_grad", C.c_int), ("tile_order", C.c_void_p), ("depths", C.c_void_p),
                 ("dL_ddepth_map", C.c_void_p), ("dL_dalpha", C.c_void_p), ("dL_ddepths", C.c_void_p),
-                ("dL_dmeans_2d_abs", C.c_void_p)]
+                ("dL_dmeans_2d_abs", C.c_void_p), ("zero_buf", C.c_void_p), ("zero_bytes", C.c_size_t)]
 
 
 class LossOpts(C.Structure):
@@ -122,6 +122,8 @@
                                           _P, _P, _P, _L, _P, _P, _P, _P, _P, C.POINTER(BlendBackwardOpts), _P]),
     "cugs_project_backward": (_I, [_L, _I, _I, _P, _P, _P, _P, _P, _P, _P, C.POINTER(Camera), _F,
                                    _P, _P, _P, _P, _P, _P, _P, _P, _P, _P, _P, _P, _P]),
+    "cugs_project_backward_zeroed_sh": (_I, [_L, _I, _I, _P, _P, _P, _P, _P, _P, _P, C.POINTER(Camera), _F,
+                                             _P, _P, _P, _P, _P, _P, _P, _P, _P, _P, _P, _P, _P]),
     "cugs_project_backward_adam": (_I, [_L, _I, _I, _P, _P, _P, _P, _P, _P, _P, C.POINTER(Camera), _F, _P,
                                         C.POINTER(AdamFused), _P, _P]),
     "cugs_sh_backward_views": (_I, [_I, _L, _I, _P, _I, _P, C.POINTER(C.c_float), _P, _P]),
diff --git a/cuda-gaussian-splatting_amd/adapter/cugs_hip_torch.cpp b/cuda-gaussian-splatting_amd/adapter/cugs_hip_torch.cpp
--- a/cuda-gaussian-splatting_amd/adapter/cugs_hip_torch.cpp
+++ b/cuda-gaussian-splatting_amd/adapter/cugs_hip_torch.cpp
@@ -212,9 +212,13 @@
                                            const float background[3], int n_gaussians, const torch::Tensor& packed,
                                            bool unpack, const torch::Tensor& zeroed_accum, const torch::Tensor& tile_order,
                                            const torch::Tensor& depths, const torch::Tensor& dL_ddepth_map,
-                                           const torch::Tensor& dL_dalpha, bool want_abs_grad) {
+                                           const torch::Tensor& dL_dalpha, bool want_abs_grad,
+                                           const torch::Tensor& zero_buf) {
     TORCH_CHECK(dL_dcolor.is_cuda(), "dL_dcolor must be on CUDA");
     const int64_t n = n_gaussians;
+    if (zero_buf.defined())
+        TORCH_CHECK(zero_buf.is_contiguous() && zero_buf.scalar_type() == torch::kFloat32 && zero_buf.numel() % 4 == 0,
+                    "zero_buf must be a contiguous float32 tensor of a multiple of four elements");
     RasterizeBackwardOutput o;
     const bool depth_route = depths.defined() || dL_ddepth_map.defined() || dL_dalpha.defined();
     if (depth_route) {
@@ -240,7 +244,10 @@
     }
     if (want_abs_grad)
         o.dL_dmeans_2d_abs = unpack ? torch::empty({n, 2}, fopt(dL_dcolor)) : o.grad_accum.slice(1, 10, 12);
-    if (n == 0) return o;
+    if (n == 0) {
+        if (zero_buf.defined()) zero_buf.zero_();
+        return o;
+    }
     auto g = dL_dcolor.contiguous(), m = means_2d.contiguous(), c = cov_2d_inv.contiguous(), r = rgb.contiguous();
     auto op = opacities.contiguous(), tr = tile_ranges.contiguous(), gi = gaussian_indices.contiguous();
     auto ft = final_T.contiguous(), nc = n_contrib.contiguous();
@@ -258,6 +265,10 @@
     opts.dL_dalpha = ptr<float>(da);
     opts.dL_ddepths = ptr<float>(o.dL_ddepths);
     opts.dL_dmeans_2d_abs = unpack ? ptr<float>(o.dL_dmeans_2d_abs) : nullptr;
+    if (zero_buf.defined() && zero_buf.numel() > 0) {
+        opts.zero_buf = zero_buf.data_ptr();
+        opts.zero_bytes = static_cast<size_t>(zero_buf.numel()) * sizeof(float);
+    }
     check(cugs_rasterize_backward_opts(img_w, img_h, background, ptr<int32_t>(tr), ptr<int32_t>(gi), ptr<float>(m),
                                        ptr<float>(c), ptr<float>(r), ptr<float>(op), ptr<float>(packed), ptr<float>(g),
                                        ptr<float>(ft), ptr<int32_t>(nc), n, ptr<float>(o.grad_accum),
@@ -275,7 +286,8 @@
                                                const torch::Tensor& scales, const torch::Tensor& opacities,
                                                const torch::Tensor& sh_coeffs, const torch::Tensor& radii,
                                                const cugs_camera& camera, int degree, float scale_modifier,
-                                               const cugs_pose_grad* pose = nullptr) {
+                                               const cugs_pose_grad* pose = nullptr,
+                                               const torch::Tensor& zeroed_sh = {}) {
     TORCH_CHECK(positions.is_cuda(), "positions must be on CUDA");
     const int64_t n = positions.size(0);
     ProjectionBackwardOutput o;
@@ -284,7 +296,11 @@
     o.dL_dscales = torch::empty({n, 3}, fopt(positions));
     o.dL_dopacities = torch::empty({n, 1}, fopt(positions));
     auto sh = f32c(sh_coeffs);
-    o.dL_dsh_coeffs = torch::empty_like(sh);
+    const bool zeroed = zeroed_sh.defined() && !pose;
+    if (zeroed)
+        TORCH_CHECK(zeroed_sh.is_contiguous() && zeroed_sh.scalar_type() == torch::kFloat32 && zeroed_sh.sizes() == sh.sizes(),
+                    "zeroed_sh must be a contiguous float32 tensor of sh_coeffs' shape");
+    o.dL_dsh_coeffs = zeroed ? zeroed_sh : torch::empty_like(sh);
     if (n == 0) return o;
     auto pos = f32c(positions), rot = f32c(rotations), scl = f32c(scales), opa = f32c(opacities), rad = radii.contiguous();
     auto cm = gm.defined() ? gm.contiguous() : gm, cc = gc.defined() ? gc.contiguous() : gc;
@@ -302,7 +318,8 @@
               "cugs_project_backward_pose");
         return o;
     }
-    check(cugs_project_backward(n, static_cast<int>(sh.size(2)), degree, ptr<float>(pos), ptr<float>(rot), ptr<float>(scl),
+    const auto entry = zeroed ? cugs_project_backward_zeroed_sh : cugs_project_backward;
+    check(entry(n, static_cast<int>(sh.size(2)), degree, ptr<float>(pos), ptr<float>(rot), ptr<float>(scl),
                                 ptr<float>(opa), ptr<float>(sh), ptr<int32_t>(rad),
                                 colour_gate ? ptr<uint8_t>(*colour_gate) : nullptr, &camera, scale_modifier,
                                 accum ? ptr<float>(*accum) : nullptr, ptr<float>(cm), ptr<float>(cc), ptr<float>(cr),
@@ -310,7 +327,7 @@
                                 ptr<float>(o.dL_dscales), ptr<float>(o.dL_dopacities), ptr<float>(o.dL_dsh_coeffs),
                                 d_means_out ? ptr<float>(*d_means_out) : nullptr, nullptr,
                                 stream_of(positions)),
-          "cugs_project_backward");
+          zeroed ? "cugs_project_backward_zeroed_sh" : "cugs_project_backward");
     return o;
 }
 }
@@ -506,10 +523,15 @@
     ro.zeroed_accum = torch::Tensor();
     if (zeroed.defined() && ro.accum_used && ro.accum_used->exchange(true)) zeroed = torch::Tensor();
     if (zeroed.defined() && (zeroed.dim() != 2 || zeroed.size(0) != n)) zeroed = torch::Tensor();
+    const bool have_gate = ro.colour_gate.defined() && ro.colour_gate.dim() == 1 && ro.colour_gate.size(0) == n;
+    torch::Tensor d_sh;
+    if (!fused && !want_camera_grad && have_gate && model.sh_coeffs.dim() == 3 && model.sh_coeffs.size(1) == 3 &&
+        model.sh_coeffs.size(2) == 16)
+        d_sh = torch::empty({n, 3, 16}, fopt(dL_dcolor));
     auto rb = rasterize_backward(dL_dcolor, ro.means_2d, ro.cov_2d_inv, ro.rgb, ro.opacities_act, ro.tile_ranges,
                                  ro.gaussian_indices, ro.final_T, ro.n_contrib, camera.width, camera.height,
                                  settings.background, static_cast<int>(n), packed, false, zeroed, ro.tile_order,
-                                 depth_grads ? ro.depths : torch::Tensor(), dL_ddepth_map, dL_dalpha, want_abs_grad);
+                                 depth_grads ? ro.depths : torch::Tensor(), dL_ddepth_map, dL_dalpha, want_abs_grad, d_sh);
     o.dL_dmeans_2d_abs = rb.dL_dmeans_2d_abs;
     o.dL_dmeans_2d = torch::empty({n, 2}, fopt(dL_dcolor));
     cugs_pose_grad pose{};
@@ -589,10 +611,9 @@
               "cugs_project_backward_adam");
         return o;
     }
-    const bool have_gate = ro.colour_gate.defined() && ro.colour_gate.dim() == 1 && ro.colour_gate.size(0) == n;
     auto pb = project_backward_impl(&rb.grad_accum, have_gate ? &ro.colour_gate : nullptr, &o.dL_dmeans_2d, {}, {}, {}, {}, model.positions,
                                     model.rotations, model.scales, model.opacities, model.sh_coeffs, ro.radii, camera, degree,
-                                    settings.scale_modifier, want_camera_grad ? &pose : nullptr);
+                                    settings.scale_modifier, want_camera_grad ? &pose : nullptr, d_sh);
     o.dL_dpositions = pb.dL_dpositions; o.dL_drotations = pb.dL_drotations; o.dL_dscales = pb.dL_dscales;
     o.dL_dopacities = pb.dL_dopacities; o.dL_dsh_coeffs = pb.dL_dsh_coeffs;
     return o;
diff --git a/cuda-gaussian-splatting_amd/adapter/cugs_hip_torch.hpp b/cuda-gaussian-splatting_amd/adapter/cugs_hip_torch.hpp
--- a/cuda-gaussian-splatting_amd/adapter/cugs_hip_torch.hpp
+++ b/cuda-gaussian-splatting_amd/adapter/cugs_hip_torch.hpp
@@ -78,7 +78,8 @@
                                            const torch::Tensor& packed = {}, bool unpack = true,
                                            const torch::Tensor& zeroed_accum = {}, const torch::Tensor& tile_order = {},
                                            const torch::Tensor& depths = {}, const torch::Tensor& dL_ddepth_map = {},
-                                           const torch::Tensor& dL_dalpha = {}, bool want_abs_grad = false);
+                                           const torch::Tensor& dL_dalpha = {}, bool want_abs_grad = false,
+                                           const torch::Tensor& zero_buf = {});
 ProjectionBackwardOutput project_backward(const torch::Tensor& dL_dmeans_2d, const torch::Tensor& dL_dcov_2d_inv,
                                           const torch::Tensor& dL_drgb, const torch::Tensor& dL_dopacity_act,
                                           const torch::Tensor& positions, const torch::Tensor& rotations,
diff --git a/cuda-gaussian-splatting_amd/csrc/project_backward.hip b/cuda-gaussian-splatting_amd/csrc/project_backward.hip
--- a/cuda-gaussian-splatting_amd/csrc/project_backward.hip
+++ b/cuda-gaussian-splatting_amd/csrc/project_backward.hip
@@ -61,6 +61,33 @@
 
 }
 
+static int project_backward_plain(int64_t n, int num_coeffs, int active_degree, const float* positions,
+                                  const float* rotations, const float* scales, const float* opacities,
+                                  const float* sh_coeffs, const int32_t* radii, const uint8_t* colour_gate,
+                                  const cugs_camera* camera_host, float scale_modifier,
+                                  const float* grad_accum, const float* dL_dmeans_2d,
+                                  const float* dL_dcov_2d_inv, const float* dL_drgb,
+                                  const float* dL_dopacity_act, float* dL_dpositions, float* dL_drotations,
+                                  float* dL_dscales, float* dL_dopacities, float* dL_dsh_coeffs,
+                                  float* dL_dmeans_2d_out, float* dL_drgb_gated_out, bool sh_zeroed, void* stream) {
+    CamArgs cam;
+    PBPtrs p;
+    bool aligned;
+    const int r = prepare_plain(n, num_coeffs, active_degree, positions, rotations, scales, opacities, sh_coeffs, radii,
+                                colour_gate, camera_host, scale_modifier, grad_accum, dL_dmeans_2d, dL_dcov_2d_inv, dL_drgb,
+                                dL_dopacity_act, dL_dpositions, dL_drotations, dL_dscales, dL_dopacities, dL_dsh_coeffs,
+                                dL_dmeans_2d_out, dL_drgb_gated_out, cam, p, aligned);
+    if (r != 0) return r == 1 ? 0 : r;
+    p.sh_zeroed = sh_zeroed ? 1 : 0;
+    hipStream_t st = static_cast<hipStream_t>(stream);
+    switch (num_coeffs) {
+        case 1: return launch_pb<1>(n, active_degree, cam, p, aligned, st);
+        case 4: return launch_pb<4>(n, active_degree, cam, p, aligned, st);
+        case 9: return launch_pb<9>(n, active_degree, cam, p, aligned, st);
+        default: return launch_pb<16>(n, active_degree, cam, p, aligned, st);
+    }
+}
+
 extern "C" int cugs_project_backward(int64_t n, int num_coeffs, int active_degree, const float* positions,
                                      const float* rotations, const float* scales, const float* opacities,
                                      const float* sh_coeffs, const int32_t* radii, const uint8_t* colour_gate,
@@ -70,21 +97,25 @@
                                      const float* dL_dopacity_act, float* dL_dpositions, float* dL_drotations,
                                      float* dL_dscales, float* dL_dopacities, float* dL_dsh_coeffs,
                                      float* dL_dmeans_2d_out, float* dL_drgb_gated_out, void* stream) {
-    CamArgs cam;
-    PBPtrs p;
-    bool aligned;
-    const int r = prepare_plain(n, num_coeffs, active_degree, positions, rotations, scales, opacities, sh_coeffs, radii,
-                                colour_gate, camera_host, scale_modifier, grad_accum, dL_dmeans_2d, dL_dcov_2d_inv, dL_drgb,
-                                dL_dopacity_act, dL_dpositions, dL_drotations, dL_dscales, dL_dopacities, dL_dsh_coeffs,
-                                dL_dmeans_2d_out, dL_drgb_gated_out, cam, p, aligned);
-    if (r != 0) return r == 1 ? 0 : r;
-    hipStream_t st = static_cast<hipStream_t>(stream);
-    switch (num_coeffs) {
-        case 1: return launch_pb<1>(n, active_degree, cam, p, aligned, st);
-        case 4: return launch_pb<4>(n, active_degree, cam, p, aligned, st);
-        case 9: return launch_pb<9>(n, active_degree, cam, p, aligned, st);
-        default: return launch_pb<16>(n, active_degree, cam, p, aligned, st);
-    }
+    return project_backward_plain(n, num_coeffs, active_degree, positions, rotations, scales, opacities, sh_coeffs, radii,
+                                  colour_gate, camera_host, scale_modifier, grad_accum, dL_dmeans_2d, dL_dcov_2d_inv, dL_drgb,
+                                  dL_dopacity_act, dL_dpositions, dL_drotations, dL_dscales, dL_dopacities, dL_dsh_coeffs,
+                                  dL_dmeans_2d_out, dL_drgb_gated_out, false, stream);
+}
+
+extern "C" int cugs_project_backward_zeroed_sh(int64_t n, int num_coeffs, int active_degree, const float* positions,
+                                               const float* rotations, const float* scales, const float* opacities,
+                                               const float* sh_coeffs, const int32_t* radii, const uint8_t* colour_gate,
+                                               const cugs_camera* camera_host, float scale_modifier,
+                                               const float* grad_accum, const float* dL_dmeans_2d,
+                                               const float* dL_dcov_2d_inv, const float* dL_drgb,
+                                               const float* dL_dopacity_act, float* dL_dpositions, float* dL_drotations,
+                                               float* dL_dscales, float* dL_dopacities, float* dL_dsh_coeffs,
+                                               float* dL_dmeans_2d_out, float* dL_drgb_gated_out, void* stream) {
+    return project_backward_plain(n, num_coeffs, active_degree, positions, rotations, scales, opacities, sh_coeffs, radii,
+                                  colour_gate, camera_host, scale_modifier, grad_accum, dL_dmeans_2d, dL_dcov_2d_inv, dL_drgb,
+                                  dL_dopacity_act, dL_dpositions, dL_drotations, dL_dscales, dL_dopacities, dL_dsh_coeffs,
+                                  dL_dmeans_2d_out, dL_drgb_gated_out, true, stream);
 }
 
 
diff --git a/cuda-gaussian-splatting_amd/csrc/project_backward_kernels.h b/cuda-gaussian-splatting_amd/csrc/project_backward_kernels.h
--- a/cuda-gaussian-splatting_amd/csrc/project_backward_kernels.h
+++ b/cuda-gaussian-splatting_amd/csrc/project_backward_kernels.h
@@ -66,7 +66,7 @@
 
 constexpr int SH_FACTOR_ROW = 20;
 __device__ __forceinline__ void store_sh_rows_from_factors(float* __restrict__ dst_base, int64_t base, int count, int num_active,
-                                                           const float* s_fac) {
+                                                           const float* s_fac, bool zeroed = false) {
     constexpr int C = 16, ROW4 = 3 * C / 4;
     float4* dst4 = reinterpret_cast<float4*>(dst_base + base * (3 * C));
     const int total4 = count * ROW4;
@@ -77,8 +77,10 @@
             const int r = e4 / ROW4, j = e4 - r * ROW4, ch = j >> 2, k = (j & 3) * 4;
             const float4 y = *reinterpret_cast<const float4*>(s_fac + r * SH_FACTOR_ROW + k);
             const float g = s_fac[r * SH_FACTOR_ROW + 16 + ch];
-            cugs_stnt(dst4 + e4, make_float4(k + 0 < num_active ? g * y.x : 0.0f, k + 1 < num_active ? g * y.y : 0.0f,
-                                             k + 2 < num_active ? g * y.z : 0.0f, k + 3 < num_active ? g * y.w : 0.0f));
+            const float4 v = make_float4(k + 0 < num_active ? g * y.x : 0.0f, k + 1 < num_active ? g * y.y : 0.0f,
+                                         k + 2 < num_active ? g * y.z : 0.0f, k + 3 < num_active ? g * y.w : 0.0f);
+            if (zeroed && v.x == 0.0f && v.y == 0.0f && v.z == 0.0f && v.w == 0.0f) continue;
+            cugs_stnt(dst4 + e4, v);
         }
     }
 }
@@ -335,6 +337,7 @@
     float* d_pos; float* d_rot; float* d_scl; float* d_opa; float* d_sh; float* d_means_out;
     float* d_rgb_gated_out;
     float* w_pos; float* w_rot; float* w_scl; float* w_opa; float* w_sh;
+    int sh_zeroed;
 };
 
 struct PoseArgs {
@@ -447,7 +450,7 @@
             }
             __syncthreads();
             if (ADAM) adam_sh_rows_from_factors<SPARSE>(p.w_sh, adam.m[1], adam.v[1], base, count, num_active, s_sh, adam.lr[1], adam);
-            else store_sh_rows_from_factors(p.d_sh, base, count, num_active, s_sh);
+            else store_sh_rows_from_factors(p.d_sh, base, count, num_active, s_sh, p.sh_zeroed != 0);
         }
     } else if (ADAM || p.d_sh) {
         if constexpr (SPARSE) {
diff --git a/cuda-gaussian-splatting_amd/csrc/raster_backward.hip b/cuda-gaussian-splatting_amd/csrc/raster_backward.hip
--- a/cuda-gaussian-splatting_amd/csrc/raster_backward.hip
+++ b/cuda-gaussian-splatting_amd/csrc/raster_backward.hip
@@ -26,7 +26,8 @@
                                                                 float* __restrict__ grad_accum, int64_t stats_row,
                                                                 const float* __restrict__ depths,
                                                                 const float* __restrict__ dL_ddepth_map,
-                                                                const float* __restrict__ dL_dalpha) {
+                                                                const float* __restrict__ dL_dalpha,
+                                                                float4* __restrict__ zero_buf, uint32_t zero_vec4) {
     __shared__ float4 s_rec[CUGS_BLOCK * CUGS_REC_F4];
     __shared__ float2 s_contrib[4][CUGS_BWD_HITS][CUGS_BWD_HSTRIDE];
 
@@ -47,6 +48,7 @@
     }
     const int tile_x = (int)(tile % (unsigned)geo.ntx), tile_y = (int)(tile / (unsigned)geo.ntx);
     const int tid = threadIdx.x, wave = tid >> 6, lane = tid & 63;
+    const unsigned fill_wave = (unsigned)__builtin_amdgcn_readfirstlane(wave);
     const int quad_x = tile_x * CUGS_TILE + (wave & 1) * 8, quad_y = tile_y * CUGS_TILE + (wave >> 1) * 8;
     const int px = quad_x + (lane & 7), py = quad_y + (lane >> 3);
     const bool inside = (px < geo.width) && (py < geo.height);
@@ -235,6 +237,12 @@
             }
         }
     }
+    if (zero_buf) {
+        const uint32_t per = (zero_vec4 + gridDim.x - 1) / gridDim.x;
+        const uint32_t lo = blockIdx.x * per, hi = min(zero_vec4, lo + per);
+        const uint32_t t = fill_wave * CUGS_WAVE + __builtin_amdgcn_mbcnt_hi(~0u, __builtin_amdgcn_mbcnt_lo(~0u, 0u));
+        for (uint32_t e = lo + t; e < hi; e += CUGS_BLOCK) cugs_stnt(zero_buf + e, make_float4(0.0f, 0.0f, 0.0f, 0.0f));
+    }
     if (STATS && lane == 0) {
         float* st = grad_accum + (int64_t)stats_row * CUGS_GRAD_STRIDE;
         atomicAdd(&st[0], (float)st_steps); atomicAdd(&st[1], (float)st_contrib); atomicAdd(&st[2], (float)st_lanes);
@@ -300,7 +308,14 @@
     const bool depth_map = o.depths || o.dL_ddepth_map || o.dL_dalpha;
     const bool abs_grad = o.abs_grad != 0;
     if (width < 0 || height < 0 || n < 0 || !background_host) return CUGS_EINVAL;
-    if (n == 0) return 0;
+    if (o.zero_bytes && (!o.zero_buf || (reinterpret_cast<uintptr_t>(o.zero_buf) & 15u) || (o.zero_bytes & 15u) ||
+                       o.zero_bytes / 16 > 0xFFFFFFFFull))
+        return o.zero_buf ? CUGS_EALIGN : CUGS_EINVAL;
+    hipStream_t st = static_cast<hipStream_t>(stream);
+    if (n == 0) {
+        if (o.zero_bytes) CUGS_RETURN_IF_HIP(hipMemsetAsync(o.zero_buf, 0, o.zero_bytes, st));
+        return 0;
+    }
     if (!grad_accum) return CUGS_EINVAL;
     if ((reinterpret_cast<uintptr_t>(grad_accum) & 63u) != 0) return CUGS_EALIGN;
     const int n_soa = (dL_drgb != nullptr) + (dL_dopacity_act != nullptr) + (dL_dmeans_2d != nullptr) +
@@ -312,7 +327,6 @@
     if (n_soa == 4 && !packed && !cov_2d_inv) return CUGS_EINVAL;
     if (packed && !cugs_aligned16(packed)) return CUGS_EALIGN;
     if (o.tile_order && !cugs_aligned16(o.tile_order)) return CUGS_EALIGN;
-    hipStream_t st = static_cast<hipStream_t>(stream);
     int64_t rows = n;
 #ifdef CUGS_DEV
     const bool stats = cugs_dev_backward_stats();
@@ -322,7 +336,10 @@
         CUGS_RETURN_IF_HIP(hipMemsetAsync(grad_accum, 0, sizeof(float) * CUGS_GRAD_STRIDE * (size_t)rows, st));
 
     const int ntx = (width + CUGS_TILE - 1) / CUGS_TILE, nty = (height + CUGS_TILE - 1) / CUGS_TILE;
-    if (ntx > 0 && nty > 0 && gaussian_indices) {
+    const bool blend = ntx > 0 && nty > 0 && gaussian_indices;
+    if (!blend && o.zero_bytes)
+        CUGS_RETURN_IF_HIP(hipMemsetAsync(o.zero_buf, 0, o.zero_bytes, st));
+    if (blend) {
         if (!tile_ranges || !dL_dcolor || !final_T || !n_contrib) return CUGS_EINVAL;
         if (!packed && (!means_2d || !cov_2d_inv || !rgb || !opacities_act)) return CUGS_EINVAL;
         if (depth_map && !o.depths) return CUGS_EINVAL;
@@ -336,7 +353,8 @@
 #endif
         const auto launch = [&](auto* kernel) {
             hipLaunchKernelGGL(kernel, dim3(geo.ntiles), dim3(CUGS_BLOCK), 0, st, geo, src, dL_dcolor, final_T, n_contrib,
-                               grad_accum, stats_arg, o.depths, o.dL_ddepth_map, o.dL_dalpha);
+                               grad_accum, stats_arg, o.depths, o.dL_ddepth_map, o.dL_dalpha,
+                               o.zero_bytes ? static_cast<float4*>(o.zero_buf) : nullptr, (uint32_t)(o.zero_bytes / 16));
         };
 #ifdef CUGS_DEV
         if (stats && !depth_map && !abs_grad)
diff --git a/cuda-gaussian-splatting_amd/rasterizer.py b/cuda-gaussian-splatting_amd/rasterizer.py
--- a/cuda-gaussian-splatting_amd/rasterizer.py
+++ b/cuda-gaussian-splatting_amd/rasterizer.py
@@ -70,6 +70,23 @@
         ws[:SORT_CONTROL_BYTES].zero_()
         _workspaces[key] = ws
     return ws
+
+
+class _ShHandover:
+    __slots__ = ("coeffs", "wanted", "pending")
+
+    def __init__(self):
+        self.coeffs = None
+        self.wanted = False
+        self.pending = None
+
+
+_sh_handover: Dict[tuple, _ShHandover] = {}
+SH_ZEROED_COEFFS = 16
+
+
+def _handover(device: torch.device) -> _ShHandover:
+    return _sh_handover.setdefault(_skey(device), _ShHandover())
 
 
 _side_streams = {}
@@ -118,6 +135,7 @@
     _torch_check((active_sh_degree + 1) ** 2 <= num_coeffs,
                  f"Need at least {(active_sh_degree + 1) ** 2} coefficients for degree {active_sh_degree}")
     pos_c, rot_c, scl_c, opa_c, sh_c = map(_f32c, (positions, rotations, scales, opacities, sh_coeffs))
+    _handover(dev).coeffs = (n, num_coeffs) if want_colour_gate else None
     cam = camera.to_abi()
     outs = (_ptr(means_2d), _ptr(depths), _ptr(cov_2d_inv), _ptr(radii), _ptr(tiles_touched), _ptr(opacities_act),
             _ptr(rgb), _ptr(packed), _ptr(colour_gate))
@@ -394,7 +412,8 @@
                        tile_order: Optional[torch.Tensor] = None, depths: Optional[torch.Tensor] = None,
                        dL_ddepth_map: Optional[torch.Tensor] = None,
                        dL_dalpha: Optional[torch.Tensor] = None,
-                       want_abs_grad: bool = False) -> RasterizeBackwardOutput:
+                       want_abs_grad: bool = False, zero_buf: Optional[torch.Tensor] = None,
+                       hand_over: bool = True) -> RasterizeBackwardOutput:
     _torch_check(dL_dcolor.is_cuda, "dL_dcolor must be on CUDA")
     dev = dL_dcolor.device
     n = int(n_gaussians)
@@ -424,12 +443,25 @@
     if n > 0 and tile_order is not None:
         _torch_check(tile_order.is_contiguous() and tile_order.dtype == torch.int32 and
                      tile_order.numel() == 4 * tile_ranges.shape[0], "tile_order must be a contiguous [tiles, 4] int32 tensor")
+    if zero_buf is not None:
+        _torch_check(zero_buf.is_contiguous() and zero_buf.dtype == torch.float32 and zero_buf.numel() % 4 == 0,
+                     "zero_buf must be a contiguous float32 tensor of a multiple of four elements")
+    ho = _handover(dev)
+    if ho.pending is not None:
+        ho.pending, ho.wanted = None, False
+    left = None
+    if (hand_over and zero_buf is None and not unpack and n > 0 and ho.wanted
+            and ho.coeffs == (n, SH_ZEROED_COEFFS)):
+        left = zero_buf = torch.empty((n, 3, SH_ZEROED_COEFFS), **f)
+    if n == 0 and zero_buf is not None:
+        zero_buf.zero_()
     if n > 0:
         bg = (C.c_float * 3)(*[float(b) for b in background])
         z, g_depth, g_alpha = (None if t is None else _f32c(t) for t in (depths, dL_ddepth_map, dL_dalpha))
         opts = _lib.BlendBackwardOpts(1 if zeroed_accum is not None else 0, 1 if want_abs_grad else 0, _ptr(tile_order),
                                       _ptr(z), _ptr(g_depth), _ptr(g_alpha), _ptr(d_z),
-                                      _ptr(d_abs) if unpack else None)
+                                      _ptr(d_abs) if unpack else None,
+                                      _ptr(zero_buf), zero_buf.numel() * 4 if zero_buf is not None else 0)
         check(lib.cugs_rasterize_backward_opts(int(img_w), int(img_h), bg, _ptr(tile_ranges.contiguous()),
                                                _ptr(gaussian_indices.contiguous()), _ptr(means_2d.contiguous()),
                                                _ptr(cov_2d_inv.contiguous()), _ptr(rgb.contiguous()),
@@ -438,6 +470,8 @@
                                                _ptr(n_contrib.contiguous()), n, _ptr(accum), _ptr(d_rgb), _ptr(d_opa),
                                                _ptr(d_means), _ptr(d_cov), C.byref(opts), _stream(dev)),
               "cugs_rasterize_backward_opts")
+    if left is not None:
+        ho.pending = (accum.data_ptr(), n, SH_ZEROED_COEFFS, left)
     return RasterizeBackwardOutput(d_rgb, d_opa, d_means, d_cov, accum, dL_ddepths=d_z, dL_dmeans_2d_abs=d_abs)
 
 
@@ -451,7 +485,8 @@
                      dL_drgb_gated_out: Optional[torch.Tensor] = None,
                      skip_sh_grad: bool = False,
                      geom_flat: Optional[torch.Tensor] = None, want_camera_grad: bool = False,
-                     dL_dview_rows: Optional[torch.Tensor] = None) -> ProjectionBackwardOutput:
+                     dL_dview_rows: Optional[torch.Tensor] = None,
+                     zeroed_sh_out: Optional[torch.Tensor] = None) -> ProjectionBackwardOutput:
     _torch_check(positions.is_cuda, "positions must be on CUDA")
     n = int(positions.shape[0])
     dev = positions.device
@@ -465,7 +500,19 @@
         d_pos, d_rot = torch.empty((n, 3), **f), torch.empty((n, 4), **f)
         d_scl, d_opa = torch.empty((n, 3), **f), torch.empty((n, 1), **f)
     sh_c = _f32c(sh_coeffs)
-    d_sh = None if skip_sh_grad else torch.empty_like(sh_c)
+    zeroed = zeroed_sh_out
+    if zeroed is not None:
+        _torch_check(not skip_sh_grad and not want_camera_grad, "zeroed_sh_out: not with skip_sh_grad or want_camera_grad")
+        _torch_check(zeroed.is_cuda and zeroed.device == dev and zeroed.dtype == torch.float32 and zeroed.is_contiguous()
+                     and zeroed.shape == sh_c.shape, "zeroed_sh_out must be a contiguous float32 tensor of sh_coeffs' shape")
+    elif grad_accum is not None and colour_gate is not None and not skip_sh_grad and not want_camera_grad and n > 0 \
+            and sh_c.dim() == 3 and tuple(sh_c.shape[1:]) == (3, SH_ZEROED_COEFFS):
+        ho = _handover(dev)
+        if ho.pending is not None and ho.pending[:3] == (grad_accum.data_ptr(), n, SH_ZEROED_COEFFS):
+            zeroed, ho.pending = ho.pending[3], None
+        else:
+            ho.wanted = True
+    d_sh = None if skip_sh_grad else (zeroed if zeroed is not None else torch.empty_like(sh_c))
     if n == 0:
         if d_view is not None:
             d_view.zero_()
@@ -481,6 +528,8 @@
     if want_camera_grad:
         pg = _pose_grad(d_view, dL_dview_rows, n, dev)
         check(lib.cugs_project_backward_pose(*args, C.byref(pg), _stream(dev)), "cugs_project_backward_pose")
+    elif zeroed is not None:
+        check(lib.cugs_project_backward_zeroed_sh(*args, _stream(dev)), "cugs_project_backward_zeroed_sh")
     else:
         check(lib.cugs_project_backward(*args, _stream(dev)), "cugs_project_backward")
     return ProjectionBackwardOutput(d_pos, d_rot, d_scl, d_opa, d_sh, dL_dviewmat=d_view)
@@ -635,13 +684,17 @@
         zeroed = None
     if zeroed is not None:
         zeroed._cugs_consumed = True
+    d_sh = None
+    if (fused_adam is None and dL_drgb_gated_out is None and not want_camera_grad and render_out.colour_gate is not None
+            and model.sh_coeffs.dim() == 3 and tuple(model.sh_coeffs.shape[1:]) == (3, SH_ZEROED_COEFFS)):
+        d_sh = torch.empty((n, 3, SH_ZEROED_COEFFS), **f)
     rb = rasterize_backward(dL_dcolor, render_out.means_2d, render_out.cov_2d_inv, render_out.rgb,
                             render_out.opacities_act, render_out.tile_ranges, render_out.gaussian_indices,
                             render_out.final_T, render_out.n_contrib, camera.width, camera.height,
                             settings.background, n, packed=render_out.packed, unpack=False, zeroed_accum=zeroed,
                             tile_order=getattr(render_out, "tile_order", None),
                             depths=render_out.depths if depth_grads else None, dL_ddepth_map=dL_ddepth_map,
-                            dL_dalpha=dL_dalpha, want_abs_grad=want_abs_grad)
+                            dL_dalpha=dL_dalpha, want_abs_grad=want_abs_grad, zero_buf=d_sh, hand_over=False)
     d_means_2d = torch.empty((n, 2), **f)
     if fused_adam is not None:
         _torch_check(fused_adam.model_ is model, "fused_adam must have been built on this model")
@@ -694,7 +747,7 @@
                           settings.scale_modifier, grad_accum=rb.grad_accum, colour_gate=render_out.colour_gate,
                           dL_dmeans_2d_out=d_means_2d, dL_drgb_gated_out=gated_by_projection,
                           skip_sh_grad=dL_drgb_gated_out is not None, geom_flat=geom_flat,
-                          want_camera_grad=want_camera_grad)
+                          want_camera_grad=want_camera_grad, zeroed_sh_out=d_sh)
     return BackwardOutput(pb.dL_dpositions, pb.dL_drotations, pb.dL_dscales, pb.dL_dopacities,
                           pb.dL_dsh_coeffs, d_means_2d, geom_flat=geom_flat, dL_dviewmat=pb.dL_dviewmat,
                           dL_dmeans_2d_abs=rb.dL_dmeans_2d_abs)
diff --git a/include/cugs_hip.h b/include/cugs_hip.h
--- a/include/cugs_hip.h
+++ b/include/cugs_hip.h
@@ -154,6 +154,8 @@
     const float* dL_dalpha;
     float* dL_ddepths;
     float* dL_dmeans_2d_abs;
+    void* zero_buf;
+    size_t zero_bytes;
 } cugs_blend_backward_opts;
 
 int cugs_rasterize_backward_opts(int width, int height, const float background_host[3],
@@ -175,6 +177,17 @@
                           float* dL_dpositions, float* dL_drotations, float* dL_dscales,
                           float* dL_dopacities, float* dL_dsh_coeffs, float* dL_dmeans_2d_out,
                           float* dL_drgb_gated_out, void* stream);
+
+int cugs_project_backward_zeroed_sh(int64_t n, int num_coeffs, int active_degree,
+                                    const float* positions, const float* rotations, const float* scales,
+                                    const float* opacities, const float* sh_coeffs, const int32_t* radii,
+                                    const uint8_t* colour_gate, const cugs_camera* camera_host,
+                                    float scale_modifier, const float* grad_accum,
+                                    const float* dL_dmeans_2d, const float* dL_dcov_2d_inv,
+                                    const float* dL_drgb, const float* dL_dopacity_act,
+                                    float* dL_dpositions, float* dL_drotations, float* dL_dscales,
+                                    float* dL_dopacities, float* dL_dsh_coeffs, float* dL_dmeans_2d_out,
+                                    float* dL_drgb_gated_out, void* stream);
 
 typedef struct cugs_adam_fused {
     float* m[5];
```

Result: no change. 2740, median of 6 (+0.6%).
